# szcompressor/sz

Hardware: AMD Instinct MI355X
Metric: compression GB/s (input), 512^3 float32 ABS 1e-4 (higher is better)
Workload: dtype f32

## Files before the change

### sz_amd/csrc/szh_segenc.h

```cpp
#pragma once

namespace szh_se {
constexpr int NR = 4;
constexpr int INNER = 7;
constexpr int PF = 8;

struct col_t { int b0, b1, s0, s1, o0, o1, rows; };
struct seg_t {
    int bkbeg, bkend, kbeg, kend;
    int nE, E, L;
    int ka, nvec, pitch, kshift;
    int nblk, nruns;
    int lg_nvec;
};
SZH_HD int seg_pitch(int width) { int p = (width + 1) & ~1; if (((p >> 1) & 1) == 0) p += 2; return p; }
SZH_HD col_t make_col(const szh_geom3 &G, int col)
{
    col_t c;
    c.b0 = col / G.g1.num; c.b1 = col - c.b0 * G.g1.num;
    c.s0 = szh_blk_size(G.g0, c.b0); c.s1 = szh_blk_size(G.g1, c.b1); c.o0 = szh_blk_start(G.g0, c.b0); c.o1 = szh_blk_start(G.g1, c.b1);
    c.rows = c.s0 * c.s1;
    return c;
}
SZH_HD seg_t make_seg(const szh_geom3 &G, int rows, int segi, int segb, int VW)
{
    seg_t s;
    s.bkbeg = segi * segb; s.bkend = s.bkbeg + segb < G.g2.num ? s.bkbeg + segb : G.g2.num;
    s.kbeg = szh_blk_start(G.g2, s.bkbeg); s.kend = s.bkend < G.g2.num ? szh_blk_start(G.g2, s.bkend) : G.g2.count;
    s.E = G.g2.early; s.L = G.g2.late;
    int nE = G.g2.split - s.bkbeg; if (nE < 0) nE = 0; if (nE > s.bkend - s.bkbeg) nE = s.bkend - s.bkbeg;
    s.nE = nE;
    s.ka = s.kbeg / VW * VW;
    const int kb = (s.kend + VW - 1) / VW * VW;
    s.nvec = (kb - s.ka) / VW;
    s.pitch = seg_pitch(kb - s.ka); s.kshift = s.kbeg - s.ka;
    s.nblk = s.bkend - s.bkbeg; s.nruns = s.nblk * rows;
    s.lg_nvec = 0; while ((1 << s.lg_nvec) < s.nvec) ++s.lg_nvec;
    return s;
}
inline size_t seg_tile_bytes(const szh_geom3 &G, int segb, int VW)
{
    const size_t rows = (size_t)G.g0.early * G.g1.early;
    const int width = segb * G.g2.early + 2 * VW;
    return (rows * (size_t)seg_pitch(width) * 2 + 15) & ~(size_t)15;
}
inline size_t seg_pieces_per_thread(const szh_geom3 &G, int segb, int VW)
{
    const size_t rows = (size_t)G.g0.early * G.g1.early;
    const size_t nvec = ((size_t)segb * G.g2.early + 2 * VW) / VW + 1;
    size_t p2 = 1; while (p2 < nvec) p2 <<= 1;
    return (rows * p2 + 255) / 256;
}
inline size_t seg_window_words(const szh_geom3 &G, unsigned maxlen, int nrmax = NR) { return (size_t)256 * nrmax * (size_t)G.g2.early * maxlen / 32 + 8; }
}

#ifdef SZH_HIPSIM
static inline bool any_lane(bool p) { return __ballot(p ? 1 : 0) != 0ull; }
#else
__device__ __forceinline__ bool any_lane(bool p) { return __builtin_amdgcn_ballot_w64(p) != 0ull; }
#endif
__device__ __forceinline__ unsigned magic_of(unsigned d) { return d > 1u ? 0xffffffffu / d + 1u : 0u; }
__device__ __forceinline__ unsigned div_by(unsigned x, unsigned d, unsigned m) { return d > 1u ? (unsigned)(((u64)x * m) >> 32) : x; }

#define SZH_COL_HBINS 256
__global__ __launch_bounds__(256) void k_col_hist(szh_geom3 G, const uint16_t *__restrict__ codes, unsigned nbins, int rshift, int vw, unsigned *__restrict__ col_hist)
{
    SZH_DYN_SMEM(smem);
    unsigned *sh = reinterpret_cast<unsigned *>(smem);
    const unsigned R = 1u << rshift;
    for (unsigned i = threadIdx.x; i < (nbins << rshift); i += 256) sh[i] = 0;
    __syncthreads();
    const szh_se::col_t c = szh_se::make_col(G, (int)blockIdx.x);
    const int nvec = G.g2.count / vw;
    const int lane = (int)threadIdx.x & 63, wid = (int)threadIdx.x >> 6;
    const unsigned rep = threadIdx.x & (R - 1);
    const unsigned m_s1 = magic_of((unsigned)c.s1);
    for (int x = lane; x < nvec; x += 64) {
        for (int r0 = wid; r0 < c.rows; r0 += 16) {
            uint4 w[4];
#pragma unroll
            for (int q = 0; q < 4; ++q) {
                const int r = r0 + 4 * q;
                w[q] = uint4{0u, 0u, 0u, 0u};
                if (r < c.rows) {
                    const int i = (int)div_by((unsigned)r, (unsigned)c.s1, m_s1), j = r - i * c.s1;
                    const uint16_t *src = codes + (int64_t)(c.o0 + i) * G.d0 + (int64_t)(c.o1 + j) * G.d1 + x * vw;
                    if (vw == 8) w[q] = *reinterpret_cast<const uint4 *>(src);
                    else if (vw == 4) { const uint2 t = *reinterpret_cast<const uint2 *>(src); w[q].x = t.x; w[q].y = t.y; }
                    else w[q].x = src[0];
                }
            }
#pragma unroll
            for (int q = 0; q < 4; ++q) {
                if (r0 + 4 * q < c.rows) {
                    const unsigned wv[4] = {w[q].x, w[q].y, w[q].z, w[q].w};
#pragma unroll
                    for (int e = 0; e < 8; ++e) if (e < vw) { const unsigned cd = (e & 1) ? wv[e >> 1] >> 16 : wv[e >> 1] & 0xffffu; atomicAdd(&sh[(cd << rshift) + rep], 1u); }
                }
            }
        }
    }
    __syncthreads();
    for (unsigned b = threadIdx.x; b < nbins; b += 256) {
        unsigned t = 0;
        for (unsigned q = 0; q < R; ++q) t += sh[(b << rshift) + q];
        col_hist[(size_t)blockIdx.x * nbins + b] = t;
    }
}
__global__ __launch_bounds__(256) void k_hist_reduce(const unsigned *__restrict__ col_hist, unsigned nbins, int64_t ncols, unsigned *__restrict__ hist)
{
    __shared__ unsigned acc[SZH_COL_HBINS];
    for (unsigned b = threadIdx.x; b < nbins; b += 256) acc[b] = 0;
    __syncthreads();
    const unsigned tpb = 256u / nbins > 0u ? 256u / nbins : 1u;
    if (threadIdx.x < tpb * nbins) {
        const unsigned bin = threadIdx.x % nbins, lane_col = threadIdx.x / nbins;
        unsigned t = 0;
        for (int64_t col = (int64_t)blockIdx.x * tpb + lane_col; col < ncols; col += (int64_t)gridDim.x * tpb) t += col_hist[(size_t)col * nbins + bin];
        if (t) atomicAdd(&acc[bin], t);
    }
    __syncthreads();
    for (unsigned b = threadIdx.x; b < nbins; b += 256) if (acc[b]) atomicAdd(&hist[b], acc[b]);
}
__global__ __launch_bounds__(256) void k_col_bits_h(const unsigned *__restrict__ col_hist, const uint8_t *__restrict__ len, unsigned nbins, int64_t ncols, u64 *__restrict__ col_bits, u64 *__restrict__ col_zeros)
{
    __shared__ uint8_t llen[SZH_COL_HBINS];
    for (unsigned i = threadIdx.x; i < nbins; i += 256) llen[i] = len[i];
    __syncthreads();
    const int64_t e = (int64_t)blockIdx.x * 256 + threadIdx.x;
    if (e >= ncols) return;
    const unsigned *h = col_hist + (size_t)e * nbins;
    u64 bits = 0;
    for (unsigned b = 0; b < nbins; ++b) bits += (u64)h[b] * llen[b];
    col_bits[e] = bits; col_zeros[e] = h[0];
}

__global__ __launch_bounds__(256) void k_col_bits(szh_geom3 G, const uint16_t *__restrict__ codes, const uint8_t *__restrict__ len, unsigned nsym, int vw,
                                                  u64 *__restrict__ col_bits, u64 *__restrict__ col_zeros)
{
    SZH_DYN_SMEM(smem);
    __shared__ u64 red[8];
    uint8_t *llen = reinterpret_cast<uint8_t *>(smem);
    const bool tab_lds = nsym <= 16384;
    if (tab_lds) { for (unsigned i = threadIdx.x; i < nsym; i += 256) llen[i] = len[i]; __syncthreads(); }
    const szh_se::col_t c = szh_se::make_col(G, (int)blockIdx.x);
    const int nvec = G.g2.count / vw;
    const int lane = (int)threadIdx.x & 63, wid = (int)threadIdx.x >> 6;
    const unsigned m_s1 = magic_of((unsigned)c.s1);
    u64 bits = 0; unsigned zeros = 0;
    for (int x = lane; x < nvec; x += 64) {
        for (int r0 = wid; r0 < c.rows; r0 += 16) {
            uint4 w[4];
#pragma unroll
            for (int q = 0; q < 4; ++q) {
                const int r = r0 + 4 * q;
                w[q] = uint4{0u, 0u, 0u, 0u};
                if (r < c.rows) {
                    const int i = (int)div_by((unsigned)r, (unsigned)c.s1, m_s1), j = r - i * c.s1;
                    const uint16_t *src = codes + (int64_t)(c.o0 + i) * G.d0 + (int64_t)(c.o1 + j) * G.d1 + x * vw;
                    if (vw == 8) w[q] = *reinterpret_cast<const uint4 *>(src);
                    else if (vw == 4) { const uint2 t = *reinterpret_cast<const uint2 *>(src); w[q].x = t.x; w[q].y = t.y; }
                    else w[q].x = src[0];
                }
            }
#pragma unroll
            for (int q = 0; q < 4; ++q) {
                if (r0 + 4 * q < c.rows) {
                    const unsigned wv[4] = {w[q].x, w[q].y, w[q].z, w[q].w};
#pragma unroll
                    for (int e = 0; e < 8; ++e) if (e < vw) {
                        const unsigned cd = (e & 1) ? wv[e >> 1] >> 16 : wv[e >> 1] & 0xffffu;
                        bits += tab_lds ? llen[cd] : len[cd]; zeros += cd == 0u ? 1u : 0u;
                    }
                }
            }
        }
    }
    bits = wave_sum_u64(bits); const u64 z = wave_sum_u64((u64)zeros);
    if (lane == 0) { red[wid] = bits; red[4 + wid] = z; }
    __syncthreads();
    if (threadIdx.x == 0) { col_bits[blockIdx.x] = red[0] + red[1] + red[2] + red[3]; col_zeros[blockIdx.x] = red[4] + red[5] + red[6] + red[7]; }
}

__global__ __launch_bounds__(256) void k_col_bounds(const u64 *__restrict__ col_bitoff, int64_t nent, const u64 *__restrict__ total_bits, u64 bit0, unsigned *out32)
{
    const int64_t e = (int64_t)blockIdx.x * 256 + threadIdx.x;
    if (e > nent) return;
    const u64 at = bit0 + (e < nent ? col_bitoff[e] : *total_bits);
    out32[at >> 5] = 0u;
    if (e == nent) out32[(at >> 5) + 1] = 0u;
}
#define SZH_COL_SCAN_PER 8
__global__ __launch_bounds__(1024) void k_col_scan(const u64 *__restrict__ col_bits, const u64 *__restrict__ col_zeros, int nent, u64 *__restrict__ col_bitoff, u64 *__restrict__ col_zoff,
                                                   u64 *total_bits, u64 *total_zeros, u64 bit0, unsigned *out32, const u64 *__restrict__ plan = nullptr)
{
    __shared__ u64 shb[16], shz[16];
    if (plan) { if (plan[SZH_PLAN_STATUS] != 0) return; bit0 = plan[SZH_PLAN_BIT0]; }
    const int tid = (int)threadIdx.x, lane = tid & 63, wid = tid >> 6;
    const int lo = tid * SZH_COL_SCAN_PER;
    u64 vb[SZH_COL_SCAN_PER], vz[SZH_COL_SCAN_PER];
#pragma unroll
    for (int q = 0; q < SZH_COL_SCAN_PER; ++q) { const bool in = lo + q < nent; vb[q] = in ? col_bits[lo + q] : 0ull; vz[q] = in ? col_zeros[lo + q] : 0ull; }
    u64 b = 0, z = 0;
#pragma unroll
    for (int q = 0; q < SZH_COL_SCAN_PER; ++q) { b += vb[q]; z += vz[q]; }
    u64 ib = b, iz = z;
    for (int o = 1; o < 64; o <<= 1) { const u64 tb = __shfl_up(ib, o, 64), tz = __shfl_up(iz, o, 64); if (lane >= o) { ib += tb; iz += tz; } }
    if (lane == 63) { shb[wid] = ib; shz[wid] = iz; }
    __syncthreads();
    u64 baseb = 0, basez = 0, totb = 0, totz = 0;
    for (int w = 0; w < 16; ++w) { if (w < wid) { baseb += shb[w]; basez += shz[w]; } totb += shb[w]; totz += shz[w]; }
    u64 rb = baseb + ib - b, rz = basez + iz - z;
#pragma unroll
    for (int q = 0; q < SZH_COL_SCAN_PER; ++q) {
        if (lo + q < nent) { col_bitoff[lo + q] = rb; col_zoff[lo + q] = rz; out32[(bit0 + rb) >> 5] = 0u; }
        rb += vb[q]; rz += vz[q];
    }
    if (tid == 0) { *total_bits = totb; *total_zeros = totz; out32[(bit0 + totb) >> 5] = 0u; out32[((bit0 + totb) >> 5) + 1] = 0u; }
}

__global__ __launch_bounds__(1024) void k_col_zscan(const unsigned *__restrict__ col_zeros, int nent, u64 *__restrict__ col_zoff, u64 *total_zeros)
{
    __shared__ u64 shz[16];
    const int tid = (int)threadIdx.x, lane = tid & 63, wid = tid >> 6;
    const int lo = tid * SZH_COL_SCAN_PER;
    u64 vz[SZH_COL_SCAN_PER], z = 0;
#pragma unroll
    for (int q = 0; q < SZH_COL_SCAN_PER; ++q) { vz[q] = lo + q < nent ? (u64)col_zeros[lo + q] : 0ull; z += vz[q]; }
    u64 iz = z;
    for (int o = 1; o < 64; o <<= 1) { const u64 tz = __shfl_up(iz, o, 64); if (lane >= o) iz += tz; }
    if (lane == 63) shz[wid] = iz;
    __syncthreads();
    u64 basez = 0, totz = 0;
    for (int w = 0; w < 16; ++w) { if (w < wid) basez += shz[w]; totz += shz[w]; }
    u64 rz = basez + iz - z;
#pragma unroll
    for (int q = 0; q < SZH_COL_SCAN_PER; ++q) { if (lo + q < nent) col_zoff[lo + q] = rz; rz += vz[q]; }
    if (tid == 0) *total_zeros = totz;
}

template <class T, bool WIDE>
__global__ __launch_bounds__(256) void k_col_encode(szh_geom3 G, const uint16_t *__restrict__ codes, const u64 *__restrict__ table, unsigned nsym, const szh_se::seg_t *__restrict__ segs, int nseg, int vw, int nrmax,
                                                    size_t tile_bytes, unsigned win_words, const u64 *__restrict__ col_bitoff, const u64 *__restrict__ col_zoff, u64 bit0,
                                                    unsigned *out32, const T *__restrict__ data, T *__restrict__ unpred, const u64 *__restrict__ plan = nullptr)
{
    using namespace szh_se;
    if (plan) { if (plan[SZH_PLAN_STATUS] != 0) return; bit0 = plan[SZH_PLAN_BIT0]; }
    SZH_DYN_SMEM(smem);
    __shared__ u64 sh[2][4];
    __shared__ unsigned rowbase[128];
    u64 *ltab = reinterpret_cast<u64 *>(smem);
    uint16_t *tile = reinterpret_cast<uint16_t *>(smem + ((size_t)nsym + 1) * 8);
    uint16_t *nullrun = reinterpret_cast<uint16_t *>(smem + ((size_t)nsym + 1) * 8 + tile_bytes);
    unsigned *win = reinterpret_cast<unsigned *>(smem + ((size_t)nsym + 1) * 8 + tile_bytes + 16);
    const int tid = (int)threadIdx.x, lane = tid & 63, wid = tid >> 6;
    const col_t c = make_col(G, (int)blockIdx.x);
    for (unsigned i = tid; i < nsym; i += 256) ltab[i] = table[i];
    if (tid == 0) ltab[nsym] = 0;
    if (tid < 8) nullrun[tid] = (uint16_t)nsym;
    for (unsigned w = tid; w < win_words; w += 256) win[w] = 0u;
    const unsigned m_rows = magic_of((unsigned)c.rows);
    if (tid < c.rows) { const int i = tid / c.s1, j = tid - i * c.s1; rowbase[tid] = (unsigned)((int64_t)(c.o0 + i) * G.d0 + (int64_t)(c.o1 + j) * G.d1); }
    __syncthreads();
    uint4 pf[PF];
    auto fetch = [&](const seg_t &s) {
        const int lg = s.lg_nvec, mask = (1 << lg) - 1;
#pragma unroll
        for (int p = 0; p < PF; ++p) {
            const int x = p * 256 + tid, r = x >> lg, cv = x & mask;
            pf[p] = uint4{0u, 0u, 0u, 0u};
            if (r < c.rows && cv < s.nvec) {
                const uint16_t *src = codes + (size_t)rowbase[r] + (unsigned)(s.ka + cv * vw);
                if (vw == 8) pf[p] = *reinterpret_cast<const uint4 *>(src);
                else if (vw == 4) { const uint2 t = *reinterpret_cast<const uint2 *>(src); pf[p].x = t.x; pf[p].y = t.y; }
                else pf[p].x = src[0];
// ... 279 lines not shown
```

### sz_amd/csrc/szhip.hip

```cpp
#include <hip/hip_runtime.h>
#include <algorithm>
#include <array>
#include <cmath>
#include <cstdio>
#include <cstdlib>
#include <cstring>
#include <atomic>
#include <chrono>
#include <ctime>
#include <condition_variable>
#include <deque>
#include <functional>
#include <memory>
#include <mutex>
#include <thread>
#include <vector>
#include "../../include/szhip.h"
#include "szhost.h"
#include "szhip_kernels.h"
#include "szh_quality.h"
#include "szh_rangebatch.h"

namespace {

struct DevBuf { void *p = nullptr; size_t cap = 0; };

double now_ms()
{
    timespec ts; clock_gettime(CLOCK_MONOTONIC, &ts);
    return ts.tv_sec * 1e3 + ts.tv_nsec * 1e-6;
}

}

static std::atomic<int> g_compress_calls{0};
static std::atomic<int> g_fed_active{0};
static std::atomic<long long> g_last_meeting_us{-(1ll << 60)};
static long long mono_us() { timespec ts; clock_gettime(CLOCK_MONOTONIC, &ts); return (long long)ts.tv_sec * 1000000ll + ts.tv_nsec / 1000; }
struct compress_call_guard {
    compress_call_guard()
    {
        if (g_compress_calls.fetch_add(1) > 0) g_last_meeting_us.store(mono_us());
        const long long t0 = mono_us();
        while (g_fed_active.load() != 0 && mono_us() - t0 < 200000) std::this_thread::yield();
    }
    ~compress_call_guard() { g_compress_calls.fetch_sub(1); }
};
struct fed_call_guard {
    bool on = false;
    bool try_raise()
    {
        if (mono_us() - g_last_meeting_us.load() < 100000) return false;
        int expected = 0;
        if (!g_fed_active.compare_exchange_strong(expected, 1)) return false;
        if (g_compress_calls.load() > 1) { g_fed_active.store(0); return false; }
        on = true;
        return true;
    }
    ~fed_call_guard() { if (on) g_fed_active.store(0); }
};
struct szhip_chain_pool {
    std::thread th[4];
    std::mutex m; std::condition_variable cv;
    std::atomic<int> phase{0};
    std::atomic<uint64_t> seq{0};
    std::atomic<int> stage1{0}, stage2{0};
    int n = 0;
    std::function<void(int)> chain, section;
    static void pause() {
#if defined(__x86_64__)
        __builtin_ia32_pause();
#endif
    }
    void run(int e)
    {
        uint64_t seen = 0;
        for (;;) {
            { std::unique_lock<std::mutex> lk(m); cv.wait(lk, [&] { return phase.load() != 0; }); }
            if (phase.load() == 2) return;
            while (phase.load(std::memory_order_acquire) == 1 && seq.load(std::memory_order_acquire) == seen) pause();
            const uint64_t s = seq.load(std::memory_order_acquire);
            if (s != seen) {
                seen = s;
                if (e < n) { chain(e); stage1.fetch_add(1, std::memory_order_release); section(e); }
                stage2.fetch_add(1, std::memory_order_release);
            }
        }
    }
    void start() { for (int e = 0; e < 4; ++e) th[e] = std::thread([this, e] { run(e); }); }
    void arm() { { std::lock_guard<std::mutex> lk(m); if (phase.load() == 0) phase.store(1); } cv.notify_all(); }
    void disarm() { std::lock_guard<std::mutex> lk(m); if (phase.load() == 1) phase.store(0); }
    void submit(int ncoef, std::function<void(int)> c, std::function<void(int)> sec)
    {
        n = ncoef; chain = std::move(c); section = std::move(sec);
        stage1.store(0); stage2.store(0);
        arm();
        seq.fetch_add(1, std::memory_order_release);
    }
    void wait_chains() { while (stage1.load(std::memory_order_acquire) < n) pause(); }
    void wait_all() { while (stage2.load(std::memory_order_acquire) < 4) std::this_thread::yield(); }
    ~szhip_chain_pool()
    {
        { std::lock_guard<std::mutex> lk(m); phase.store(2); }
        cv.notify_all();
        for (auto &t : th) if (t.joinable()) t.join();
    }
};

constexpr int SZH_STAGE_T = 4;
struct szhip_ctx {
    int device = 0;
    int cus = 256;
    hipStream_t stream = nullptr;
    hipStream_t stream2 = nullptr;
    hipEvent_t ev_in = nullptr, ev_fit = nullptr, ev_feed = nullptr, ev_sec = nullptr;
    int settle_probes = 0, settle_rejected = 0;
    hipStream_t stream3 = nullptr;
    hipEvent_t ev_perm = nullptr;
    hipEvent_t ev[6] = {nullptr, nullptr, nullptr, nullptr, nullptr, nullptr};
    char err[512] = {0};
    unsigned epoch = 0;
    bool hdec_sync_rounds = false, hdec_unconverged = false;
    bool gate = false;
    unsigned long long *hdec_res = nullptr;
    DevBuf lor_bits, reg_flags, reg_rank, coef_compact, in, out, codes_nat, codes_blk, coef, blk_lor, faceI, faceJ, rb_down, rb_right, rb_vals, pt_flags, feed_word, progress, order, small, hist, col_zeros, col_zeros64,
        seg_bits, seg_zeros, seg_bitoff, seg_zoff, seg_hist, seg_tab, col_off, partial, samples, unpred, stream_buf, chunk_bits, chunk_off, code_tab, len_tab, dec_tab,
        starts, ends, counts, offs, dirty, zcnt, zpos, pwr_log, pwr_signs, pwr_small, coef_dec, msst_ptab, msst_cells, msst_rec, msst_pe, book_tree, book_rec, book_stage,
        batch_rec, batch_blob,
        in2, quality;
    void *pinned = nullptr; size_t pinned_cap = 0;
    void *pinned2 = nullptr; size_t pinned2_cap = 0;
    void *stage_buf[SZH_STAGE_T][2] = {};
    hipEvent_t stage_ev[SZH_STAGE_T][2] = {};
    void *pinned3 = nullptr; size_t pinned3_cap = 0;
    int streams_independent = -1;
    void *coh = nullptr; size_t coh_cap = 0;
    int order_nI = -1, order_nJ = -1;
    bool wave_timeout = false, ticket_atomic = false;
    bool coef_late = false, no_chain_overlap = false;
    bool book_declined = false, no_dev_book = false;
    unsigned long long *book_pin = nullptr;
    std::vector<int> chain_codes; std::vector<unsigned char> chain_unpred;
    unsigned char *sec_pin[4] = {nullptr, nullptr, nullptr, nullptr}; size_t sec_pin_cap[4] = {0, 0, 0, 0};
    szhip_chain_pool *chain_pool = nullptr;
};

namespace {

#include "szhip_rt.inc"
#include "szhip_steps.inc"
#include "szhip_sz21.inc"
#include "szhip_sz14.inc"
#include "szhip_pwr.inc"
#include "szhip_omp.inc"
#include "szhip_ompbatch.inc"
#include "szhip_rangebatch.inc"
#include "szhip_quality.inc"

}

static void drain(szhip_ctx *ctx)
{
    if (ctx->stream3) hipStreamSynchronize(ctx->stream3);
    hipStreamSynchronize(ctx->stream2);
    hipStreamSynchronize(ctx->stream);
}
static int drained_on_failure(szhip_ctx *ctx, int rc) { if (rc != SZHIP_OK) drain(ctx); return rc; }
static int synced_on_failure(szhip_ctx *ctx, int rc) { if (rc != SZHIP_OK) hipStreamSynchronize(ctx->stream); return rc; }

template <class F>
static int with_ticket_fallback(szhip_ctx *ctx, F &&run)
{
    ctx->wave_timeout = false; ctx->hdec_unconverged = false; ctx->coef_late = false; ctx->book_declined = false;
    auto again = [&]() { drain(ctx); return run(); };
    int rc = run();
    if (rc == SZHIP_ERR_INTERNAL && ctx->book_declined && !ctx->no_dev_book) {
        ctx->no_dev_book = true; ctx->wave_timeout = false; rc = again(); ctx->no_dev_book = false;
    }
    if (rc == SZHIP_OK && !ctx->no_chain_overlap && tune_int("SZ_HIP_TEST_CHAIN_FALLBACK", 0)) { ctx->coef_late = true; rc = SZHIP_ERR_INTERNAL; }
    if (rc == SZHIP_ERR_INTERNAL && ctx->coef_late && !ctx->no_chain_overlap) {
        ctx->no_chain_overlap = true; ctx->wave_timeout = false; rc = again();
    }
    if (rc == SZHIP_ERR_INTERNAL && ctx->hdec_unconverged && !ctx->hdec_sync_rounds) {
        ctx->hdec_sync_rounds = true; ctx->wave_timeout = false; rc = again(); ctx->hdec_sync_rounds = false;
    }
    if (rc == SZHIP_OK && !ctx->ticket_atomic && tune_int("SZ_HIP_TEST_TICKET_FALLBACK", 0)) { ctx->wave_timeout = true; rc = SZHIP_ERR_INTERNAL; }
    if (rc == SZHIP_ERR_INTERNAL && ctx->wave_timeout && !ctx->ticket_atomic) {
        ctx->ticket_atomic = true; rc = again();
    }
    return rc;
}

template <class F>
static int guarded_compress(szhip_ctx *ctx, unsigned char **out, size_t *out_size, F &&run)
{
    const compress_call_guard in_flight;
    unsigned char *const out0 = *out; const size_t cap0 = *out_size;
    return drained_on_failure(ctx, with_ticket_fallback(ctx, [&]() { *out = out0; *out_size = cap0; return run(); }));
}

static bool dims_3d_2d(size_t r0, size_t r1, size_t r2)
{
    return !((r0 != 0 && r0 < 2) || r1 < 2 || r2 < 2 || r0 > 0x7fffffff || r1 > 0x7fffffff || r2 > 0x7fffffff);
}
static bool dims_3d_2d_1d(size_t r0, size_t r1, size_t r2)
{
    return !((r0 != 0 && r0 < 2) || (r1 < 2 && !(r0 == 0 && r1 == 0)) || r2 < 2 || r0 > 0x7fffffff || r1 > 0x7fffffff || r2 > 0x7fffffff);
}

extern "C" {


static int create_ctx(szhip_ctx **out, int device)
{
    if (!out) return SZHIP_ERR_ARG;
    int count = 0;
    hipError_t e = hipGetDeviceCount(&count);
    if (e != hipSuccess || count <= 0) {
        fprintf(stderr, "szhip: no HIP device available (%s); this library has no CPU fallback\n", hipGetErrorString(e));
        return SZHIP_ERR_NODEVICE;
    }
    if (device < 0 || device >= count) return SZHIP_ERR_ARG;
    szhip_ctx *ctx = new szhip_ctx();
    ctx->device = device;
    { int c = 0; if (hipDeviceGetAttribute(&c, hipDeviceAttributeMultiprocessorCount, device) == hipSuccess && c > 0) ctx->cus = c; }
    if (hipSetDevice(device) != hipSuccess || hipStreamCreateWithFlags(&ctx->stream, hipStreamNonBlocking) != hipSuccess) {
        delete ctx; return SZHIP_ERR_NODEVICE;
    }
    for (int i = 0; i < 6; ++i) if (hipEventCreate(&ctx->ev[i]) != hipSuccess) { delete ctx; return SZHIP_ERR_NODEVICE; }
    if (hipStreamCreateWithFlags(&ctx->stream2, hipStreamNonBlocking) != hipSuccess || hipEventCreateWithFlags(&ctx->ev_in, hipEventDisableTiming) != hipSuccess ||
        hipEventCreateWithFlags(&ctx->ev_fit, hipEventDisableTiming) != hipSuccess ||
        hipEventCreateWithFlags(&ctx->ev_feed, hipEventDisableTiming) != hipSuccess ||
        hipEventCreateWithFlags(&ctx->ev_sec, hipEventDisableTiming) != hipSuccess) { delete ctx; return SZHIP_ERR_NODEVICE; }
    *out = ctx;
    return SZHIP_OK;
}

int szhip_create(szhip_ctx **out, int device)
{
    const int rc = create_ctx(out, device);
    if (rc == SZHIP_OK) settle_streams(*out, nullptr, 0);
    return rc;
}

void szhip_destroy(szhip_ctx *ctx)
{
    if (!ctx) return;
    hipSetDevice(ctx->device);
    hipStreamSynchronize(ctx->stream);
    delete ctx->chain_pool; ctx->chain_pool = nullptr;
    DevBuf *bufs[] = {&ctx->lor_bits, &ctx->reg_flags, &ctx->reg_rank, &ctx->coef_compact, &ctx->in, &ctx->out, &ctx->codes_nat, &ctx->codes_blk, &ctx->coef, &ctx->blk_lor, &ctx->faceI, &ctx->faceJ, &ctx->rb_down, &ctx->rb_right, &ctx->rb_vals, &ctx->pt_flags, &ctx->feed_word, &ctx->progress,
                      &ctx->order, &ctx->small, &ctx->hist, &ctx->col_zeros, &ctx->col_zeros64, &ctx->seg_bits, &ctx->seg_zeros, &ctx->seg_bitoff, &ctx->seg_zoff, &ctx->seg_hist, &ctx->seg_tab, &ctx->col_off, &ctx->partial,
                      &ctx->samples, &ctx->unpred, &ctx->stream_buf, &ctx->chunk_bits, &ctx->chunk_off, &ctx->code_tab,
                      &ctx->len_tab, &ctx->dec_tab, &ctx->starts, &ctx->ends, &ctx->counts, &ctx->offs, &ctx->dirty, &ctx->zcnt, &ctx->zpos,
                      &ctx->pwr_log, &ctx->pwr_signs, &ctx->pwr_small, &ctx->coef_dec, &ctx->msst_ptab, &ctx->msst_cells, &ctx->msst_rec, &ctx->msst_pe, &ctx->book_tree, &ctx->book_rec, &ctx->book_stage, &ctx->batch_rec, &ctx->batch_blob, &ctx->in2, &ctx->quality};
    for (DevBuf *b : bufs) if (b->p) hipFree(b->p);
    if (ctx->pinned) hipHostFree(ctx->pinned);
    if (ctx->pinned2) hipHostFree(ctx->pinned2);
    if (ctx->pinned3) hipHostFree(ctx->pinned3);
    if (ctx->coh) hipHostFree(ctx->coh);
    if (ctx->hdec_res) hipHostFree(ctx->hdec_res);
    if (ctx->book_pin) hipHostFree(ctx->book_pin);
    for (int w = 0; w < SZH_STAGE_T; ++w) for (int k = 0; k < 2; ++k) { if (ctx->stage_buf[w][k]) hipHostFree(ctx->stage_buf[w][k]); if (ctx->stage_ev[w][k]) hipEventDestroy(ctx->stage_ev[w][k]); }
    for (int i = 0; i < 6; ++i) if (ctx->ev[i]) hipEventDestroy(ctx->ev[i]);
    if (ctx->ev_in) hipEventDestroy(ctx->ev_in);
    if (ctx->ev_fit) hipEventDestroy(ctx->ev_fit);
    if (ctx->ev_feed) hipEventDestroy(ctx->ev_feed);
    if (ctx->ev_sec) hipEventDestroy(ctx->ev_sec);
    for (int e = 0; e < 4; ++e) if (ctx->sec_pin[e]) hipHostFree(ctx->sec_pin[e]);
    if (ctx->stream2) hipStreamDestroy(ctx->stream2);
    if (ctx->stream3) hipStreamDestroy(ctx->stream3);
    if (ctx->ev_perm) hipEventDestroy(ctx->ev_perm);
    if (ctx->stream) hipStreamDestroy(ctx->stream);
    delete ctx;
}

const char *szhip_last_error(szhip_ctx *ctx) { return ctx ? ctx->err : "no context"; }

struct szhip_pool_job {
    int dtype; const void *data; int on_dev; size_t r0, r1, r2; double eb; szhip_params prm; const unsigned char *meta; size_t meta_len;
    int out_on_device; unsigned char *out; size_t out_size; szhip_stats stats; int rc; bool done;
};
struct szhip_pool {
    std::vector<szhip_ctx *> ctx;
    std::vector<std::thread> workers;
    std::mutex mu;
    std::condition_variable cv_work, cv_done;
    std::deque<int> queue;
    std::vector<szhip_pool_job> jobs;
    std::vector<bool> used;
    bool stop = false;
};
static void szhip_pool_worker(szhip_pool *p, int lane)
{
    for (;;) {
        int t;
        {
            std::unique_lock<std::mutex> lk(p->mu);
            p->cv_work.wait(lk, [&] { return p->stop || !p->queue.empty(); });
            if (p->queue.empty()) return;
            t = p->queue.front(); p->queue.pop_front();
        }
        szhip_pool_job &j = p->jobs[t];
        j.rc = szhip_compress(p->ctx[lane], j.dtype, j.data, j.on_dev, j.r0, j.r1, j.r2, j.eb, &j.prm, j.meta, j.meta_len, j.out_on_device,
                              &j.out, &j.out_size, &j.stats);
        { std::lock_guard<std::mutex> lk(p->mu); j.done = true; }
        p->cv_done.notify_all();
    }
}
int szhip_pool_create(szhip_pool **out, int device, int lanes)
{
    if (!out || lanes < 1 || lanes > 16) return SZHIP_ERR_ARG;
    szhip_pool *p = new szhip_pool();
    for (int i = 0; i < lanes; ++i) {
        szhip_ctx *c = nullptr;
        const int rc = create_ctx(&c, device);
        if (rc != SZHIP_OK) { for (szhip_ctx *x : p->ctx) szhip_destroy(x); delete p; return rc; }
        c->gate = lanes > 1;
        { std::vector<hipStream_t> mains; for (szhip_ctx *x : p->ctx) { mains.push_back(x->stream); mains.push_back(x->stream2); } settle_streams(c, mains.data(), (int)mains.size(), lanes == 1); }
        p->ctx.push_back(c);
    }
    p->jobs.resize(64); p->used.assign(64, false);
    for (int i = 0; i < lanes; ++i) p->workers.emplace_back(szhip_pool_worker, p, i);
    *out = p;
    return SZHIP_OK;
}
void szhip_pool_destroy(szhip_pool *p)
{
    if (!p) return;
    { std::lock_guard<std::mutex> lk(p->mu); p->stop = true; }
    p->cv_work.notify_all();
    for (auto &w : p->workers) if (w.joinable()) w.join();
    for (szhip_ctx *c : p->ctx) szhip_destroy(c);
    delete p;
}
int szhip_pool_submit(szhip_pool *p, int dtype, const void *data, int data_on_device, size_t r0, size_t r1, size_t r2, double eb,
                      const szhip_params *params, const unsigned char *meta, size_t meta_len, int out_on_device,
                      unsigned char *out_buf, size_t out_cap, int *ticket)
{
    if (!p || !data || !params || !meta || !ticket) return SZHIP_ERR_ARG;
    std::lock_guard<std::mutex> lk(p->mu);
    int t = -1;
    for (size_t i = 0; i < p->used.size(); ++i) if (!p->used[i]) { t = (int)i; break; }
    if (t < 0) return SZHIP_ERR_ARG;
    szhip_pool_job &j = p->jobs[t];
    j = szhip_pool_job();
    j.dtype = dtype; j.data = data; j.on_dev = data_on_device; j.r0 = r0; j.r1 = r1; j.r2 = r2; j.eb = eb; j.prm = *params;
    j.meta = meta; j.meta_len = meta_len; j.out_on_device = out_on_device; j.out = out_on_device == 2 ? out_buf : nullptr;
    j.out_size = out_on_device == 2 ? out_cap : 0; j.rc = SZHIP_ERR_INTERNAL; j.done = false;
    p->used[t] = true;
    p->queue.push_back(t);
    *ticket = t;
    p->cv_work.notify_one();
    return SZHIP_OK;
}
int szhip_pool_wait(szhip_pool *p, int ticket, unsigned char **out, size_t *out_size, szhip_stats *stats)
{
    if (!p || ticket < 0 || ticket >= (int)p->jobs.size()) return SZHIP_ERR_ARG;
    std::unique_lock<std::mutex> lk(p->mu);
    if (!p->used[ticket]) return SZHIP_ERR_ARG;
    p->cv_done.wait(lk, [&] { return p->jobs[ticket].done; });
    szhip_pool_job &j = p->jobs[ticket];
    if (out) *out = j.out;
    if (out_size) *out_size = j.out_size;
    if (stats) *stats = j.stats;
    p->used[ticket] = false;
    return j.rc;
}


int szhip_stage_input(szhip_ctx *ctx, const void *host_data, size_t bytes, void **device_ptr)
{
    if (!ctx || !host_data || !device_ptr) return SZHIP_ERR_ARG;
    if (hipSetDevice(ctx->device) != hipSuccess) return SZHIP_ERR_NODEVICE;
    TRY(ensure(ctx, ctx->in, bytes));
    TRY(staged_copy(ctx, ctx->in.p, host_data, bytes, true));
    *device_ptr = ctx->in.p;
    return SZHIP_OK;
}

int szhip_stage_input_batch(szhip_ctx *ctx, const void *const *host_data, int count, size_t bytes, const void **device_ptrs)
{
    if (!ctx || !host_data || !device_ptrs || count < 1 || bytes == 0) return SZHIP_ERR_ARG;
    for (int i = 0; i < count; ++i) if (!host_data[i]) return SZHIP_ERR_ARG;
    if (hipSetDevice(ctx->device) != hipSuccess) return SZHIP_ERR_NODEVICE;
    std::vector<const void *> d;
    TRY(synced_on_failure(ctx, batch_stage(ctx, ctx->in, count, bytes, ctx->stream, [&](int i) { return host_data[i]; }, d)));
    if (hipStreamSynchronize(ctx->stream) != hipSuccess) return SZHIP_ERR_NODEVICE;
    for (int i = 0; i < count; ++i) device_ptrs[i] = d[i];
    return SZHIP_OK;
}
int szhip_stage_input_batch_lens(szhip_ctx *ctx, const void *const *host_data, int count, const size_t *bytes, const void **device_ptrs)
{
    if (!ctx || !host_data || !device_ptrs || !bytes || count < 1) return SZHIP_ERR_ARG;
    for (int i = 0; i < count; ++i) if (!host_data[i] || bytes[i] == 0) return SZHIP_ERR_ARG;
    if (hipSetDevice(ctx->device) != hipSuccess) return SZHIP_ERR_NODEVICE;
    std::vector<const void *> d;
    TRY(synced_on_failure(ctx, batch_stage(ctx, ctx->in, count, 0, ctx->stream, [&](int i) { return host_data[i]; }, d, nullptr, bytes)));
    if (hipStreamSynchronize(ctx->stream) != hipSuccess) return SZHIP_ERR_NODEVICE;
    for (int i = 0; i < count; ++i) device_ptrs[i] = d[i];
    return SZHIP_OK;
}

static int check_alignment_set_device(szhip_ctx *ctx, int dtype, const void *p)
{
    if (((uintptr_t)p & (dtype == SZHIP_F32 ? 3u : 7u)) != 0) {
        snprintf(ctx->err, sizeof(ctx->err), "pointer %p is not aligned to its %d-byte elements", p, dtype == SZHIP_F32 ? 4 : 8);
        return SZHIP_ERR_ARG;
    }
    return hipSetDevice(ctx->device) != hipSuccess ? SZHIP_ERR_NODEVICE : SZHIP_OK;
}
#define BY_DTYPE(dtype, fn, ...) ((dtype) == SZHIP_F32 ? fn<float>(__VA_ARGS__) : fn<double>(__VA_ARGS__))

int szhip_minmax(szhip_ctx *ctx, int dtype, const void *data, int on_dev, size_t n, double *vmin, double *vmax)
{
    if (!ctx || !data || !n || !vmin || !vmax) return SZHIP_ERR_ARG;
    TRY(check_alignment_set_device(ctx, dtype, data));
    return BY_DTYPE(dtype, minmax_impl, ctx, data, on_dev, n, vmin, vmax);
}

static int batch_pointers(szhip_ctx *ctx, int dtype, const void *const *p, int count, size_t n)
{
    if (!ctx || !p || count < 1 || n == 0 || (dtype != SZHIP_F32 && dtype != SZHIP_F64)) return SZHIP_ERR_ARG;
    for (int i = 0; i < count; ++i) {
        if (!p[i]) { snprintf(ctx->err, sizeof(ctx->err), "array %d of the batch: a null pointer", i); return SZHIP_ERR_ARG; }
        if (((uintptr_t)p[i] & (dtype == SZHIP_F32 ? 3u : 7u)) != 0) {
            snprintf(ctx->err, sizeof(ctx->err), "array %d of the batch: pointer %p is not aligned to its %d-byte elements", i, p[i], dtype == SZHIP_F32 ? 4 : 8);
            return SZHIP_ERR_ARG;
        }
    }
    return SZHIP_OK;
}

int szhip_minmax_batch(szhip_ctx *ctx, int dtype, const void *const *data, int count, int data_on_device, size_t n, double *vmin, double *vmax, szhip_stats *stats)
{
    if (!vmin || !vmax) return SZHIP_ERR_ARG;
    TRY(batch_pointers(ctx, dtype, data, count, n));
    if (hipSetDevice(ctx->device) != hipSuccess) return SZHIP_ERR_NODEVICE;
    return synced_on_failure(ctx, BY_DTYPE(dtype, minmax_batch_impl, ctx, data, count, data_on_device, 1, 1, n, n, n, nullptr, vmin, vmax, stats));
}
static int check_view(szhip_ctx *ctx, size_t r0, size_t r1, size_t r2, size_t pitch0, size_t pitch1);
int szhip_minmax_batch_view(szhip_ctx *ctx, int dtype, const void *const *data, int count, int data_on_device, size_t r0, size_t r1, size_t r2, size_t pitch0, size_t pitch1,
                            double *vmin, double *vmax, szhip_stats *stats)
{
    if (!vmin || !vmax) return SZHIP_ERR_ARG;
    if (r0 < 1 || r1 < 1 || r2 < 1 || r0 > 0x7fffffff || r1 > 0x7fffffff || r2 > 0x7fffffff) return SZHIP_ERR_ARG;
    TRY(batch_pointers(ctx, dtype, data, count, 1));
    TRY(check_view(ctx, r0, r1, r2, pitch0, pitch1));
    if ((double)r0 * (double)r1 * (double)r2 >= 4294967296.0) { snprintf(ctx->err, sizeof(ctx->err), "szhip_minmax_batch_view: sub-boxes of 2^32 values or more"); return SZHIP_ERR_UNSUP; }
    if (hipSetDevice(ctx->device) != hipSuccess) return SZHIP_ERR_NODEVICE;
    if (pitch1 == r2 && pitch0 == r1 * r2) { const size_t n = r0 * r1 * r2; r0 = r1 = 1; r2 = pitch0 = pitch1 = n; }
    return synced_on_failure(ctx, BY_DTYPE(dtype, minmax_batch_impl, ctx, data, count, data_on_device, r0, r1, r2, pitch0, pitch1, nullptr, vmin, vmax, stats));
}

int szhip_compress(szhip_ctx *ctx, int dtype, const void *data, int data_on_device, size_t r0, size_t r1, size_t r2, double eb,
                   const szhip_params *params, const unsigned char *meta, size_t meta_len, int out_on_device,
                   unsigned char **out, size_t *out_size, szhip_stats *stats)
{
    if (!ctx || !data || !params || !meta || !out || !out_size) return SZHIP_ERR_ARG;
    if (!dims_3d_2d(r0, r1, r2)) return SZHIP_ERR_ARG;
    if (!(eb > 0)) return SZHIP_ERR_ARG;
    TRY(check_alignment_set_device(ctx, dtype, data));
    return guarded_compress(ctx, out, out_size, [&]() {
               return BY_DTYPE(dtype, compress_impl, ctx, data, data_on_device, r0, r1, r2, eb, params, meta, meta_len, out_on_device, out, out_size, stats); });
}

int szhip_compress_sz14(szhip_ctx *ctx, int dtype, const void *data, int data_on_device, size_t r0, size_t r1, size_t r2, double eb,
                        double value_range, double median, const szhip_params *params, const unsigned char *meta, size_t meta_len,
                        int out_on_device, unsigned char **out, size_t *out_size, szhip_stats *stats)
{
    if (!ctx || !data || !params || !meta || !out || !out_size) return SZHIP_ERR_ARG;
    if (!dims_3d_2d_1d(r0, r1, r2)) return SZHIP_ERR_ARG;
    if (!(eb > 0)) return SZHIP_ERR_ARG;
    TRY(check_alignment_set_device(ctx, dtype, data));
    return guarded_compress(ctx, out, out_size, [&]() {
               return BY_DTYPE(dtype, compress14_impl, ctx, data, data_on_device, r0, r1, r2, eb, value_range, median, params, meta, meta_len, nullptr, out_on_device, out, out_size, stats); });
}

int szhip_decompress_sz14(szhip_ctx *ctx, int dtype, const unsigned char *stream, int stream_on_device, size_t stream_len, size_t body_off,
                          size_t r0, size_t r1, size_t r2, void *out, int out_on_device, szhip_stats *stats)
{
    if (!ctx || !stream || !out || body_off >= stream_len) return SZHIP_ERR_ARG;
    if (!dims_3d_2d_1d(r0, r1, r2)) return SZHIP_ERR_ARG;
    TRY(check_alignment_set_device(ctx, dtype, out));
    return drained_on_failure(ctx, with_ticket_fallback(ctx, [&]() {
               return BY_DTYPE(dtype, decompress14_impl, ctx, stream, stream_on_device, stream_len, body_off, 0, r0, r1, r2, out, out_on_device, stats); }));
}

int szhip_compress_omp(szhip_ctx *ctx, int dtype, const void *data, int data_on_device, size_t r0, size_t r1, size_t r2, double eb, int thread_num,
                       const szhip_params *params, const unsigned char *meta, size_t meta_len, int out_on_device, unsigned char **out, size_t *out_size,
                       szhip_stats *stats)
{
    if (!ctx || !data || !params || !meta || !out || !out_size) return SZHIP_ERR_ARG;
    if (r0 < 1 || r1 < 1 || r2 < 1 || r0 > 0x7fffffff || r1 > 0x7fffffff || r2 > 0x7fffffff || thread_num < 1) return SZHIP_ERR_ARG;
    if (!(eb > 0)) return SZHIP_ERR_ARG;
    TRY(check_alignment_set_device(ctx, dtype, data));
    return synced_on_failure(ctx,
               BY_DTYPE(dtype, compress_omp_impl, ctx, data, data_on_device, r0, r1, r2, r1 * r2, r2, eb, thread_num, params, meta, meta_len, out_on_device, out, out_size, stats));
}

int szhip_decompress_omp(szhip_ctx *ctx, int dtype, const unsigned char *stream, int stream_on_device, size_t stream_len, size_t body_off,
                         size_t r0, size_t r1, size_t r2, void *out, int out_on_device, szhip_stats *stats)
{
    if (!ctx || !stream || !out || body_off >= stream_len) return SZHIP_ERR_ARG;
    if (r0 < 1 || r1 < 1 || r2 < 1 || r0 > 0x7fffffff || r1 > 0x7fffffff || r2 > 0x7fffffff) return SZHIP_ERR_ARG;
    TRY(check_alignment_set_device(ctx, dtype, out));
    return synced_on_failure(ctx,
               BY_DTYPE(dtype, decompress_omp_impl, ctx, stream, stream_on_device, stream_len, body_off, r0, r1, r2, out, out_on_device, 0, 0, stats));
}

static int batch_args(szhip_ctx *ctx, int dtype, const szhip_batch_item *items, int count, size_t r0, size_t r1, size_t r2, bool compress)
// ... 462 lines not shown
```

### sz_amd/csrc/szhip_kernels.h

```cpp
#pragma once
#include <hip/hip_runtime.h>
#include "szh_core.h"
#include "szh_pencil.h"
#include "szh_bufio.h"

typedef unsigned long long u64;

#ifdef SZH_HIPSIM
#define SZH_DYN_SMEM(name) char *name = hipsim_dyn_smem()
#else
#define SZH_DYN_SMEM(name) extern __shared__ __attribute__((aligned(16))) char name[]
#endif

__device__ __forceinline__ u64 ord_enc(float v)
{
    unsigned u = __float_as_uint(v);
    u = (u & 0x80000000u) ? ~u : (u | 0x80000000u);
    return (u64)u;
}
__device__ __forceinline__ u64 ord_enc(double v)
{
    u64 u = (u64)__double_as_longlong(v);
    u = (u & 0x8000000000000000ull) ? ~u : (u | 0x8000000000000000ull);
    return u;
// ... 129 lines not shown
    __device__ static szh_u64 ld_sys_u64(const szh_u64 *p) { return __hip_atomic_load(const_cast<szh_u64 *>(p), __ATOMIC_RELAXED, __HIP_MEMORY_SCOPE_SYSTEM); }
    __device__ static float ld_coef(const float *p) { return __uint_as_float(__hip_atomic_load(reinterpret_cast<unsigned *>(const_cast<float *>(p)), __ATOMIC_RELAXED, __HIP_MEMORY_SCOPE_SYSTEM)); }
    __device__ static double ld_coef(const double *p) { return __longlong_as_double((long long)__hip_atomic_load(reinterpret_cast<szh_u64 *>(const_cast<double *>(p)), __ATOMIC_RELAXED, __HIP_MEMORY_SCOPE_SYSTEM)); }
    __device__ static void backoff(int n) { for (int i = 0; i < n; ++i) __builtin_amdgcn_s_sleep(2); }
    template <class E, int N> __device__ static void ld16(const E *p, E (&v)[N])
    {
        static_assert(sizeof(E) * N == 16, "16-byte vector");
        const uint4 w = *reinterpret_cast<const uint4 *>(p);
        __builtin_memcpy(v, &w, 16);
    }
    template <class E, int N> __device__ static void st16(E *p, const E (&v)[N])
    {
        static_assert(sizeof(E) * N == 16, "16-byte vector");
        uint4 w; __builtin_memcpy(&w, v, 16);
        *reinterpret_cast<uint4 *>(p) = w;
    }
    __device__ static void nap() { __builtin_amdgcn_s_sleep(40); }
};

template <class T> struct szh_tile_shape;
#ifndef SZH_TPI_F32
#define SZH_TPI_F32 2
#define SZH_TPJ_F32 2
#endif
template <> struct szh_tile_shape<float> { static constexpr int TPI = SZH_TPI_F32, TPJ = SZH_TPJ_F32, RL = 64; };
#ifndef SZH_TPI_F64
#define SZH_TPI_F64 3
#define SZH_TPJ_F64 3
#define SZH_RL_F64 32
#endif
template <> struct szh_tile_shape<double> { static constexpr int TPI = SZH_TPI_F64, TPJ = SZH_TPJ_F64, RL = SZH_RL_F64; };

template <class T, bool DEC, bool MS = false>
__global__ __launch_bounds__((szh_tile_shape<T>::TPI * szh_tile_shape<T>::TPJ + 2) * 64) void k_pencil(szh_qargs<T> a)
{
    using S = szh_tile_shape<T>;
    using B = GpuBackend<S::TPI, S::TPJ, S::RL>;
    constexpr int NP = S::TPI * S::TPJ, NV = S::TPI + S::TPJ, NT = (NP + 2) * 64;
    __shared__ uint16_t cring[NP * (SZH_XC + 1) * 64];
    __shared__ T faces[(NP + NV) * (S::RL + 2) * SZH_FROWS + SZH_FTRASH];
    __shared__ unsigned cstep[NP + NV];
    __shared__ unsigned spubJ[NP], spubI[NP];
    __shared__ int scratch[128];
#ifdef SZH_LDS_PAD
    __shared__ int lds_pad[SZH_LDS_PAD / 4];
    if (a.backoff == -12345) lds_pad[threadIdx.x] = 1;
#endif
    __shared__ unsigned tk_s;
    (void)NT;
#ifdef SZH_HIPSIM
    const int w = (int)(threadIdx.x >> 6);
#else
    const int w = __builtin_amdgcn_readfirstlane((int)(threadIdx.x >> 6));
    {
        const int d = w < NP ? (w / S::TPJ + w % S::TPJ) : -1;
        if (d < 0) __builtin_amdgcn_s_setprio(3);
        else if (d == 0) __builtin_amdgcn_s_setprio(3); else if (d == 1) __builtin_amdgcn_s_setprio(2);
        else if (d <= 3) __builtin_amdgcn_s_setprio(1); else __builtin_amdgcn_s_setprio(0);
    }
#endif
    const szh_tile_lds<T> L{cring, faces, (NP + NV) * (S::RL + 2) * SZH_FROWS, cstep, spubJ, spubI, scratch};
    const unsigned ntiles = (unsigned)(((a.nI + S::TPI - 1) / S::TPI) * ((a.nJ + S::TPJ - 1) / S::TPJ));
    for (unsigned it = 0;; ++it) {
        if (it) __syncthreads();
        if (threadIdx.x < NP + NV) cstep[threadIdx.x] = 0;
        if (threadIdx.x < NP) { spubJ[threadIdx.x] = 0; spubI[threadIdx.x] = 0; }
        if (threadIdx.x == 0) {
            const unsigned t = (a.ticket_mode && !a.persist) ? blockIdx.x : atomicAdd(a.ticket, 1u);
            tk_s = t >= ntiles ? 0xffffffffu
                 : (a.ticket_mode == 2 || a.persist) ? szh_pencil_order_at((a.nI + S::TPI - 1) / S::TPI, (a.nJ + S::TPJ - 1) / S::TPJ, t) : a.order[t];
        }
        __syncthreads();
#ifdef SZH_HIPSIM
        const unsigned ij = tk_s;
#else
        const unsigned ij = (unsigned)__builtin_amdgcn_readfirstlane((int)tk_s);
#endif
        if (ij == 0xffffffffu) break;
        const int TI = (int)(ij >> 16), TJ = (int)(ij & 0xffffu);
        if (w < NP) {
            const int I = TI * S::TPI + w / S::TPJ, J = TJ * S::TPJ + w % S::TPJ;
            if (I < a.nI && J < a.nJ) szh_pencil_run<T, DEC, B, MS>(a, I, J, L);
        } else if (w == NP) szh_tile_store<T, B>(a, TI, TJ, L);
        else szh_tile_fill<T, B>(a, TI, TJ, L);
        if (!a.persist) break;
    }
}

template <class T> struct GlobAcc {
    const T *p; int64_t d0, d1;
    __device__ T operator()(int i, int j, int k) const { return p[i * d0 + j * d1 + k]; }
    __device__ T operator()(int j, int k) const { return p[j * d1 + k]; }
};

template <class T>
__global__ __launch_bounds__(256) void k_fit_select(szh_geom3 G, const T *__restrict__ data, T *coef, uint8_t *blk_lor,
                                                    T noise, int use_mean, T mean, u64 *minmax)
{
    __shared__ u64 red[8];
    const int lane = threadIdx.x & 63, wid = threadIdx.x >> 6;
    const int64_t b = (int64_t)blockIdx.x * 256 + threadIdx.x;
    u64 lmin = ~0ull, lmax = 0ull;
    if (b < G.nblocks) {
        const int nb2 = G.g2.num, nb1 = G.g1.num;
        const int b2 = (int)(b % nb2);
        const int64_t c = b / nb2;
        const int b1 = (int)(c % nb1), b0 = (int)(c / nb1);
        const int s0 = szh_blk_size(G.g0, b0), s1 = szh_blk_size(G.g1, b1), s2 = szh_blk_size(G.g2, b2);
        const GlobAcc<T> A{data + (int64_t)szh_blk_start(G.g0, b0) * G.d0 + (int64_t)szh_blk_start(G.g1, b1) * G.d1 + szh_blk_start(G.g2, b2),
                           G.d0, G.d1};
        T c4[4];
        auto range = [&](T v) { const u64 oe = ord_enc(v); const bool num = v == v; lmin = num && oe < lmin ? oe : lmin; lmax = num && oe > lmax ? oe : lmax; };
        int reg;
        if (G.ndim == 2) {
            c4[0] = 0;
            szh_fit_block_2d<T>(A, s1, s2, c4 + 1, range);
            reg = szh_select_block_2d<T>(A, s1, s2, c4 + 1, noise);
        } else {
            szh_fit_block<T>(A, s0, s1, s2, c4, range);
            reg = szh_select_block<T>(A, s0, s1, s2, c4, noise, use_mean, mean);
        }
        for (int e = 0; e < 4; ++e) coef[(int64_t)e * G.nblocks + b] = c4[e];
        blk_lor[b] = reg ? 0 : 1;
    }
    lmin = wave_min_u64(lmin); lmax = wave_max_u64(lmax);
    if (lane == 0) { red[wid] = lmin; red[4 + wid] = lmax; }
    __syncthreads();
    if (threadIdx.x == 0) {
        u64 mn = red[0], mx = red[4];
        for (int w = 1; w < 4; ++w) { mn = red[w] < mn ? red[w] : mn; mx = red[4 + w] > mx ? red[4 + w] : mx; }
        atomicMin(&minmax[0], mn); atomicMax(&minmax[1], mx);
    }
}

template <class T>
__global__ __launch_bounds__(256) void k_minmax(const T *__restrict__ data, int64_t n, u64 *minmax)
{
    __shared__ u64 red[8];
    u64 lmin = ~0ull, lmax = 0ull;
    for (int64_t i = (int64_t)blockIdx.x * 256 + threadIdx.x; i < n; i += (int64_t)gridDim.x * 256) {
        const T v = data[i]; const u64 e = ord_enc(v); const bool num = v == v;
        lmin = num && e < lmin ? e : lmin; lmax = num && e > lmax ? e : lmax;
    }
    lmin = wave_min_u64(lmin); lmax = wave_max_u64(lmax);
    if ((threadIdx.x & 63) == 0) { red[threadIdx.x >> 6] = lmin; red[4 + (threadIdx.x >> 6)] = lmax; }
    __syncthreads();
    if (threadIdx.x == 0) {
        u64 mn = red[0], mx = red[4];
        for (int w = 1; w < 4; ++w) { mn = red[w] < mn ? red[w] : mn; mx = red[4 + w] > mx ? red[4 + w] : mx; }
        atomicMin(&minmax[0], mn); atomicMax(&minmax[1], mx);
    }
}

template <class T>
__global__ __launch_bounds__(256) void k_gather_mean(const T *__restrict__ data, szh_meanwalk w, int64_t count, T *out)
{
    const int64_t m = (int64_t)blockIdx.x * 256 + threadIdx.x;
    if (m < count) out[m] = data[szh_meanwalk_pos(w, m)];
}

#define SZH_LDS_RADIUS_BINS 4096
template <class T, bool FREQ>
__device__ __forceinline__ void sample_body(szh_geom3 G, const T *__restrict__ data, int64_t nrows, int sd, double ebD, T mean,
                                            unsigned max_radius, unsigned *radius_hist, unsigned *freq_hist, u64 *within)
{
    __shared__ unsigned sh_r[SZH_LDS_RADIUS_BINS];
    __shared__ unsigned sh_f[FREQ ? 8192 : 1];
    for (int i = threadIdx.x; i < SZH_LDS_RADIUS_BINS; i += 256) sh_r[i] = 0;
    if (FREQ) for (int i = threadIdx.x; i < 8192; i += 256) sh_f[i] = 0;
    __syncthreads();
    const int64_t rpp = G.g1.count - 1, r2 = G.g2.count;
    const bool two_d = G.ndim == 2;
    unsigned w = 0;
    for (int64_t ridx = (int64_t)blockIdx.x * 256 + threadIdx.x; ridx < nrows; ridx += (int64_t)gridDim.x * 256) {
        const int64_t n1 = two_d ? 0 : ridx / rpp + 1, n2 = two_d ? ridx + 1 : ridx - (n1 - 1) * rpp + 1;
        const int64_t c0 = two_d ? szh_sample_col0_2d(n2, sd) : sd - ((n1 + n2) % sd);
        const int64_t origin = n1 * G.d0 + n2 * r2;
        for (int64_t m = 0;; ++m) {
            const int64_t col = c0 + m * sd;
            if (m > 0 && col >= r2) break;
            const int64_t pos = origin + col;
            if (pos >= G.n) break;
            unsigned ri; int fi, we;
            szh_sample_point<T>(data, pos, r2, two_d ? 0 : G.d0, ebD, mean, max_radius, &ri, &fi, &we);
            if (ri < SZH_LDS_RADIUS_BINS) atomicAdd(&sh_r[ri], 1u); else atomicAdd(&radius_hist[ri], 1u);
            if (FREQ) atomicAdd(&sh_f[fi], 1u);
            w += (unsigned)we;
        }
    }
    w = wave_sum_u32(w);
    if ((threadIdx.x & 63) == 0 && w) atomicAdd(within, (u64)w);
    __syncthreads();
    for (int i = threadIdx.x; i < SZH_LDS_RADIUS_BINS; i += 256) if (sh_r[i]) atomicAdd(&radius_hist[i], sh_r[i]);
    if (FREQ) for (int i = threadIdx.x; i < 8192; i += 256) if (sh_f[i]) atomicAdd(&freq_hist[i], sh_f[i]);
}
template <class T, bool FREQ>
__global__ __launch_bounds__(256) void k_sample(szh_geom3 G, const T *__restrict__ data, int64_t nrows, int sd, double ebD, T mean,
                                                unsigned max_radius, unsigned *radius_hist, unsigned *freq_hist, u64 *within)
{
    sample_body<T, FREQ>(G, data, nrows, sd, ebD, mean, max_radius, radius_hist, freq_hist, within);
}
template <class T, bool FREQ>
__global__ void k_sample_walk(szh_geom3 G, const T *__restrict__ data, int sd, double ebD, T mean, unsigned max_radius, unsigned *radius_hist,
                              unsigned *freq_hist, u64 *within)
{
    if (threadIdx.x != 0 || blockIdx.x != 0) return;
    const int64_t r3 = G.g2.count, r2 = G.g1.count, r23 = r2 * r3, len = G.n;
    int64_t oc = sd - 2, n1 = 1, n2 = 1, pos = r23 + r3 + oc;
    u64 w = 0;
    while (pos < len) {
        unsigned ri; int fi, we;
        szh_sample_point<T>(data, pos, r3, r23, ebD, mean, max_radius, &ri, &fi, &we);
        atomicAdd(&radius_hist[ri], 1u);
        if (FREQ) atomicAdd(&freq_hist[fi], 1u);
        w += (unsigned)we;
        oc += sd;
        if (oc >= r3) {
            n2++;
            if (n2 == r2) { n1++; n2 = 1; pos += r3; }
            const int64_t oc2 = (n1 + n2) % sd;
            pos += (r3 + sd - oc) + (sd - oc2);
            oc = sd - oc2;
            if (oc == 0) oc++;
        } else pos += sd;
    }
    if (w) atomicAdd(within, w);
}

template <class T>
__device__ __forceinline__ void sample_view_body(const unsigned tid, szh_geom3 G, const T *data, int64_t p0, int64_t p1, int64_t nrows, int sd, double ebD,
                                                 unsigned max_radius, unsigned *radius_hist, u64 *within)
{
    __shared__ unsigned sh_r[SZH_LDS_RADIUS_BINS];
    for (int i = tid; i < SZH_LDS_RADIUS_BINS; i += 256) sh_r[i] = 0;
    __syncthreads();
    const int64_t rpp = G.g1.count - 1, r2 = G.g2.count;
    unsigned w = 0;
    for (int64_t ridx = (int64_t)blockIdx.x * 256 + tid; ridx < nrows; ridx += (int64_t)gridDim.x * 256) {
        const int64_t n1 = ridx / rpp + 1, n2 = ridx - (n1 - 1) * rpp + 1;
        const int64_t c0 = sd - ((n1 + n2) % sd);
        const int64_t origin = n1 * G.d0 + n2 * r2;
        for (int64_t m = 0;; ++m) {
            const int64_t col = c0 + m * sd;
            if (m > 0 && col >= r2) break;
            const int64_t pos = origin + col;
            if (pos >= G.n) break;
            unsigned ri; int fi, we;
            if (col < r2) szh_sample_point<T>(data, n1 * p0 + n2 * p1 + col, p1, p0, ebD, (T)0, max_radius, &ri, &fi, &we);
            else szh_sample_point_view<T>(data, pos, r2, G.d0, p0, p1, ebD, max_radius, &ri, &we);
            if (ri < SZH_LDS_RADIUS_BINS) atomicAdd(&sh_r[ri], 1u); else atomicAdd(&radius_hist[ri], 1u);
            w += (unsigned)we;
        }
    }
    w = wave_sum_u32(w);
    if ((tid & 63) == 0 && w) atomicAdd(within, (u64)w);
    __syncthreads();
    for (int i = tid; i < SZH_LDS_RADIUS_BINS; i += 256) if (sh_r[i]) atomicAdd(&radius_hist[i], sh_r[i]);
}
template <class T>
__global__ __launch_bounds__(256) void k_sample_view(szh_geom3 G, const T *__restrict__ data, int64_t p0, int64_t p1, int64_t nrows, int sd, double ebD,
                                                     unsigned max_radius, unsigned *radius_hist, u64 *within)
{
    __shared__ unsigned sh_r[SZH_LDS_RADIUS_BINS];
    for (int i = threadIdx.x; i < SZH_LDS_RADIUS_BINS; i += 256) sh_r[i] = 0;
    __syncthreads();
    const int64_t rpp = G.g1.count - 1, r2 = G.g2.count;
    unsigned w = 0;
    for (int64_t ridx = (int64_t)blockIdx.x * 256 + threadIdx.x; ridx < nrows; ridx += (int64_t)gridDim.x * 256) {
        const int64_t n1 = ridx / rpp + 1, n2 = ridx - (n1 - 1) * rpp + 1;
        const int64_t c0 = sd - ((n1 + n2) % sd);
        const int64_t origin = n1 * G.d0 + n2 * r2;
        for (int64_t m = 0;; ++m) {
            const int64_t col = c0 + m * sd;
            if (m > 0 && col >= r2) break;
            const int64_t pos = origin + col;
            if (pos >= G.n) break;
            unsigned ri; int fi, we;
            if (col < r2) szh_sample_point<T>(data, n1 * p0 + n2 * p1 + col, p1, p0, ebD, (T)0, max_radius, &ri, &fi, &we);
            else szh_sample_point_view<T>(data, pos, r2, G.d0, p0, p1, ebD, max_radius, &ri, &we);
            if (ri < SZH_LDS_RADIUS_BINS) atomicAdd(&sh_r[ri], 1u); else atomicAdd(&radius_hist[ri], 1u);
            w += (unsigned)we;
        }
    }
    w = wave_sum_u32(w);
    if ((threadIdx.x & 63) == 0 && w) atomicAdd(within, (u64)w);
    __syncthreads();
    for (int i = threadIdx.x; i < SZH_LDS_RADIUS_BINS; i += 256) if (sh_r[i]) atomicAdd(&radius_hist[i], sh_r[i]);
}
template <class T>
__global__ void k_sample_walk_view(szh_geom3 G, const T *__restrict__ data, int64_t p0, int64_t p1, int sd, double ebD, unsigned max_radius,
                                   unsigned *radius_hist, u64 *within)
{
    if (threadIdx.x != 0 || blockIdx.x != 0) return;
    const int64_t r3 = G.g2.count, r2 = G.g1.count, r23 = r2 * r3, len = G.n;
    int64_t oc = sd - 2, n1 = 1, n2 = 1, pos = r23 + r3 + oc;
    u64 w = 0;
    while (pos < len) {
        unsigned ri; int we;
        szh_sample_point_view<T>(data, pos, r3, r23, p0, p1, ebD, max_radius, &ri, &we);
        atomicAdd(&radius_hist[ri], 1u);
        w += (unsigned)we;
        oc += sd;
        if (oc >= r3) {
            n2++;
            if (n2 == r2) { n1++; n2 = 1; pos += r3; }
            const int64_t oc2 = (n1 + n2) % sd;
            pos += (r3 + sd - oc) + (sd - oc2);
            oc = sd - oc2;
            if (oc == 0) oc++;
        } else pos += sd;
    }
// ... 1123 lines not shown
```

### sz_amd/csrc/szhip_rt.inc

```

#define HIPCHK(call)                                                                                   \
    do {                                                                                               \
        hipError_t e_ = (call);                                                                        \
        if (e_ != hipSuccess) {                                                                        \
            snprintf(ctx->err, sizeof(ctx->err), "%s failed: %s (%s:%d)", #call, hipGetErrorString(e_), __FILE__, __LINE__); \
            fprintf(stderr, "szhip: %s\n", ctx->err);                                                  \
            return SZHIP_ERR_NODEVICE;                                                                 \
        }                                                                                              \
    } while (0)

#define FAIL(code, ...)                                                                                \
    do {                                                                                               \
        snprintf(ctx->err, sizeof(ctx->err), __VA_ARGS__);                                             \
        fprintf(stderr, "szhip: %s\n", ctx->err);                                                      \
        return (code);                                                                                 \
    } while (0)
#define FAIL_PUBLISHED(code, ...)                                                                      \
    do {                                                                                               \
        if (!out_on_device && out && *out) { free(*out); *out = nullptr; }                              \
        if (out_size) *out_size = 0;                                                                   \
        FAIL(code, __VA_ARGS__);                                                                       \
    } while (0)

int ensure(szhip_ctx *ctx, DevBuf &b, size_t bytes, bool zero_new = false)
{
    if (bytes == 0) bytes = 16;
    if (b.cap >= bytes) return SZHIP_OK;
    if (b.p) { HIPCHK(hipStreamSynchronize(ctx->stream)); HIPCHK(hipFree(b.p)); b.p = nullptr; b.cap = 0; }
    size_t cap = bytes + bytes / 8 + 256;
    HIPCHK(hipMalloc(&b.p, cap));
    b.cap = cap;
    if (zero_new) HIPCHK(hipMemsetAsync(b.p, 0, cap, ctx->stream));
    return SZHIP_OK;
}

#define TRY(x) do { int rc_ = (x); if (rc_ != SZHIP_OK) return rc_; } while (0)

int ensure_host(szhip_ctx *ctx, void *&p, size_t &have, size_t bytes, hipStream_t user, unsigned flags = hipHostMallocDefault)
{
    if (have >= bytes) return SZHIP_OK;
    if (p) { HIPCHK(hipStreamSynchronize(user)); HIPCHK(hipHostFree(p)); p = nullptr; have = 0; }
    size_t cap = bytes + bytes / 4 + 4096;
    HIPCHK(hipHostMalloc(&p, cap, flags));
    have = cap;
    return SZHIP_OK;
}
int ensure_pinned(szhip_ctx *ctx, size_t bytes) { return ensure_host(ctx, ctx->pinned, ctx->pinned_cap, bytes, ctx->stream); }
int ensure_pinned2(szhip_ctx *ctx, size_t bytes) { return ensure_host(ctx, ctx->pinned2, ctx->pinned2_cap, bytes, ctx->stream2); }
int ensure_pinned3(szhip_ctx *ctx, size_t bytes) { return ensure_host(ctx, ctx->pinned3, ctx->pinned3_cap, bytes, ctx->stream); }
int ensure_coherent(szhip_ctx *ctx, size_t bytes)
{
    const size_t had = ctx->coh_cap;
    TRY(ensure_host(ctx, ctx->coh, ctx->coh_cap, bytes, ctx->stream, hipHostMallocCoherent | hipHostMallocMapped));
    if (ctx->coh_cap != had) memset(ctx->coh, 0, ctx->coh_cap);
    return SZHIP_OK;
}

enum { SM_MINMAX = 0, SM_WITHIN = 2, SM_MEANCNT = 3, SM_TOTAL_UNPRED = 4, SM_TOTAL_BITS = 5, SM_TICKET = 6, SM_ERR = 7,
       SM_CHANGED = 8, SM_MEANSUM = 9, SM_TOTAL_SYM = 10, SM_NREG = 11, SM_SCRATCH = 12, SM_COUNT = 16 };

int probe_streams(szhip_ctx *ctx)
{
    if (ctx->streams_independent >= 0) return SZHIP_OK;
    TRY(ensure_coherent(ctx, 256));
    TRY(ensure(ctx, ctx->small, SM_COUNT * 8));
    volatile unsigned long long *flag = (volatile unsigned long long *)((char *)ctx->coh + 128);
    unsigned long long *src = (unsigned long long *)((char *)ctx->coh + 192);
    *flag = 0; *src = 1;
    HIPCHK(hipStreamSynchronize(ctx->stream)); HIPCHK(hipStreamSynchronize(ctx->stream2));
    u64 *sm = (u64 *)ctx->small.p;
    hipLaunchKernelGGL(k_probe_wait, dim3(1), dim3(1), 0, ctx->stream, (const unsigned long long *)flag, (unsigned long long *)(sm + SM_SCRATCH));
    HIPCHK(hipGetLastError());
    HIPCHK(hipMemcpyAsync(sm + SM_SCRATCH + 1, src, 8, hipMemcpyHostToDevice, ctx->stream2));
    const double t0 = now_ms();
    HIPCHK(hipStreamSynchronize(ctx->stream2));
    const double waited = now_ms() - t0;
    *flag = 1;
    HIPCHK(hipStreamSynchronize(ctx->stream));
    ctx->streams_independent = waited < 2.0 ? 1 : 0;
    return SZHIP_OK;
}

static int probe_pair(szhip_ctx *ctx, hipStream_t a, hipStream_t b, int *shared)
{
    TRY(ensure_coherent(ctx, 256));
    TRY(ensure(ctx, ctx->small, SM_COUNT * 8));
    volatile unsigned long long *flag = (volatile unsigned long long *)((char *)ctx->coh + 128);
    *flag = 0;
    HIPCHK(hipStreamSynchronize(a)); HIPCHK(hipStreamSynchronize(b));
    u64 *sm = (u64 *)ctx->small.p;
    hipLaunchKernelGGL(k_probe_wait, dim3(1), dim3(1), 0, a, (const unsigned long long *)flag, (unsigned long long *)(sm + SM_SCRATCH));
    HIPCHK(hipGetLastError());
    hipLaunchKernelGGL(k_probe_touch, dim3(1), dim3(1), 0, b, (unsigned long long *)(sm + SM_SCRATCH + 1));
    HIPCHK(hipGetLastError());
    const double t0 = now_ms();
    HIPCHK(hipStreamSynchronize(b));
    const double waited = now_ms() - t0;
    *flag = 1;
    HIPCHK(hipStreamSynchronize(a));
    *shared = waited < 2.0 ? 0 : 1;
    return SZHIP_OK;
}

static void settle_one(szhip_ctx *ctx, hipStream_t *victim, const std::vector<hipStream_t> &against, std::vector<hipStream_t> &rejected, int *probes)
{
    for (int attempt = 0; attempt < 6; ++attempt) {
        bool clash = false;
        for (hipStream_t a : against) {
            if (a == *victim) continue;
            int shared = 0;
            ++*probes;
            if (probe_pair(ctx, a, *victim, &shared) != SZHIP_OK) return;
            if (shared) { clash = true; break; }
        }
        if (!clash) return;
        hipStream_t fresh = nullptr;
        if (hipStreamCreateWithFlags(&fresh, hipStreamNonBlocking) != hipSuccess) return;
        rejected.push_back(*victim);
        *victim = fresh;
    }
}
static void settle_streams(szhip_ctx *ctx, const hipStream_t *mains, int n_mains, bool third = true)
{
#ifdef SZH_SYNC_LAUNCH
    (void)ctx; (void)mains; (void)n_mains; (void)third;
#else
    std::vector<hipStream_t> rejected, against(mains, mains + n_mains);
    int probes = 0;
    if (n_mains) settle_one(ctx, &ctx->stream, against, rejected, &probes);
    against.push_back(ctx->stream);
    settle_one(ctx, &ctx->stream2, against, rejected, &probes);
    if (third && !ctx->stream3 && hipStreamCreateWithFlags(&ctx->stream3, hipStreamNonBlocking) != hipSuccess) ctx->stream3 = nullptr;
    if (third && ctx->stream3) { against.push_back(ctx->stream2); settle_one(ctx, &ctx->stream3, against, rejected, &probes); }
    ctx->settle_probes = probes; ctx->settle_rejected = (int)rejected.size();
    for (hipStream_t r : rejected) hipStreamDestroy(r);
#endif
}

int tune_int(const char *name, int def);
constexpr size_t SZH_STAGE_CHUNK = 8u << 20;
struct host_view { size_t r1, row, pitch0, pitch1; };
static void host_view_move(const host_view &v, char *base, char *buf, size_t off, size_t len, bool gather)
{
    size_t rw = off / v.row, col = off - rw * v.row;
    while (len) {
        const size_t k = rw / v.r1, i = rw - k * v.r1, take = std::min(len, v.row - col);
        char *p = base + k * v.pitch0 + i * v.pitch1 + col;
        if (gather) memcpy(buf, p, take); else memcpy(p, buf, take);
        buf += take; len -= take; col = 0; ++rw;
    }
}
int staged_copy(szhip_ctx *ctx, void *dst, const void *src, size_t bytes, bool to_device, const host_view *hv = nullptr)
{
    hipStream_t st = ctx->stream;
    const size_t chunk = std::min(SZH_STAGE_CHUNK, (size_t)std::max(1, tune_int("SZ_HIP_STAGE_CHUNK_KB", (int)(SZH_STAGE_CHUNK >> 10))) << 10);
    if (bytes < 4 * chunk && hv) {
        TRY(ensure_pinned3(ctx, bytes));
        HIPCHK(hipStreamSynchronize(st));
        if (to_device) host_view_move(*hv, (char *)const_cast<void *>(src), (char *)ctx->pinned3, 0, bytes, true);
        HIPCHK(hipMemcpyAsync(to_device ? dst : ctx->pinned3, to_device ? ctx->pinned3 : src, bytes, to_device ? hipMemcpyHostToDevice : hipMemcpyDeviceToHost, st));
        HIPCHK(hipStreamSynchronize(st));
        if (!to_device) host_view_move(*hv, (char *)dst, (char *)ctx->pinned3, 0, bytes, false);
        return SZHIP_OK;
    }
    if (bytes < 4 * chunk) {
        HIPCHK(hipMemcpyAsync(dst, src, bytes, to_device ? hipMemcpyHostToDevice : hipMemcpyDeviceToHost, st));
        HIPCHK(hipStreamSynchronize(st));
        return SZHIP_OK;
    }
    constexpr int nthr = SZH_STAGE_T;
    for (int w = 0; w < nthr; ++w)
        for (int k = 0; k < 2; ++k)
            if (!ctx->stage_buf[w][k]) {
                HIPCHK(hipHostMalloc(&ctx->stage_buf[w][k], SZH_STAGE_CHUNK, hipHostMallocDefault));
                HIPCHK(hipEventCreateWithFlags(&ctx->stage_ev[w][k], hipEventDisableTiming));
            }
    HIPCHK(hipStreamSynchronize(st));
    const size_t nchunks = (bytes + chunk - 1) / chunk;
    std::atomic<int> failed(0);
    const int device = ctx->device;
    auto host_in = [&](void *buf, size_t off, size_t len) {
        if (hv) host_view_move(*hv, (char *)const_cast<void *>(src), (char *)buf, off, len, true); else memcpy(buf, (const char *)src + off, len);
    };
    auto host_out = [&](const void *buf, size_t off, size_t len) {
        if (hv) host_view_move(*hv, (char *)dst, (char *)const_cast<void *>(buf), off, len, false); else memcpy((char *)dst + off, buf, len);
    };
    auto worker = [&](int w) {
        if (hipSetDevice(device) != hipSuccess) { failed = 1; return; }
        size_t pend_off[2] = {0, 0}, pend_len[2] = {0, 0};
        bool pend[2] = {false, false};
        int k = 0;
        for (size_t c = (size_t)w; c < nchunks && !failed; c += (size_t)nthr, k ^= 1) {
            const size_t off = c * chunk, len = std::min(chunk, bytes - off);
            if (to_device) {
                if (pend[k] && hipEventSynchronize(ctx->stage_ev[w][k]) != hipSuccess) { failed = 1; return; }
                host_in(ctx->stage_buf[w][k], off, len);
                if (hipMemcpyAsync((char *)dst + off, ctx->stage_buf[w][k], len, hipMemcpyHostToDevice, st) != hipSuccess ||
                    hipEventRecord(ctx->stage_ev[w][k], st) != hipSuccess) { failed = 1; return; }
                pend[k] = true;
            } else {
                if (pend[k]) {
                    if (hipEventSynchronize(ctx->stage_ev[w][k]) != hipSuccess) { failed = 1; return; }
                    host_out(ctx->stage_buf[w][k], pend_off[k], pend_len[k]);
                }
                if (hipMemcpyAsync(ctx->stage_buf[w][k], (const char *)src + off, len, hipMemcpyDeviceToHost, st) != hipSuccess ||
                    hipEventRecord(ctx->stage_ev[w][k], st) != hipSuccess) { failed = 1; return; }
                pend[k] = true; pend_off[k] = off; pend_len[k] = len;
            }
        }
        for (int q = 0; q < 2; ++q, k ^= 1) {
            if (!pend[k]) continue;
            if (hipEventSynchronize(ctx->stage_ev[w][k]) != hipSuccess) { failed = 1; return; }
// ... 204 lines not shown
```

### sz_amd/csrc/szhip_sz21.inc

```
static bool book_declines(unsigned rec_status, unsigned long long plan_status, int test_switch) { return rec_status != 0 || plan_status != 0 || test_switch != 0; }

struct sz21_plan {
    bool use_beam = false;
    bool segenc = false;
    bool seghist = false;
    bool dev_book = false;
    bool sliced = false;
    int slices_req = 1;
    int se_vw = 1, se_segb = 0, se_nseg = 0, se_nrmax = szh_se::NR; size_t se_tile = 0;
    int sh_rshift = 0;
    bool revise(unsigned enc_maxlen) { if (!segenc || enc_maxlen <= 32) return false; segenc = false; seghist = false; return true; }
};
template <class T>
sz21_plan sz21_make_plan(const szhip_ctx *ctx, const szh_geom3 &G, unsigned intervals, size_t reg_count, bool beam_ok, bool overlap, bool feed, size_t meta_len)
{
    sz21_plan P;
    const int64_t n = G.n;
    P.use_beam = !overlap && beam_ok;
    const int segenc_sw = tune_int("SZ_HIP_SEGENC", 1);
    P.segenc = G.ndim == 3 && segenc_sw != 0 && (!feed || segenc_sw == 2);
    P.se_vw = (G.g2.count % 8) == 0 ? 8 : ((G.g2.count % 4) == 0 ? 4 : 1);
    if (P.segenc) {
        bool ok = intervals < 65536 && (double)n < 4.0e9;
        if ((int64_t)G.g0.late * G.g1.late * G.g2.late < 32) ok = false;
        const size_t fixed = ((size_t)intervals + 1) * 8 + 16 + szh_se::seg_window_words(G, 32) * 4 + 64;
        const size_t lds_cap = (size_t)63 * 1024, want = (size_t)std::max(4, tune_int("SZ_HIP_SEG_TILE_KB", 14)) * 1024;
        if (ok && fixed + szh_se::seg_tile_bytes(G, 1, P.se_vw) > lds_cap) ok = false;
        if (ok) {
            const size_t budget = std::min(lds_cap - fixed, std::max(want, szh_se::seg_tile_bytes(G, 1, P.se_vw)));
            int sb = 1;
            while (sb < G.g2.num && szh_se::seg_tile_bytes(G, sb + 1, P.se_vw) <= budget && szh_se::seg_pieces_per_thread(G, sb + 1, P.se_vw) <= (size_t)szh_se::PF) ++sb;
            sb = (G.g2.num + (G.g2.num + sb - 1) / sb - 1) / ((G.g2.num + sb - 1) / sb);
            if (const int f = tune_int("SZ_HIP_SEG_SEGB", 0)) sb = std::max(1, std::min(f, sb));
            P.se_segb = sb;
            P.se_nseg = (G.g2.num + sb - 1) / sb;
            P.se_tile = szh_se::seg_tile_bytes(G, sb, P.se_vw);
            const int rows_typ = (2 * G.g0.split > G.g0.num ? G.g0.early : G.g0.late) * (2 * G.g1.split > G.g1.num ? G.g1.early : G.g1.late);
            const int runs_typ = std::max(1, sb * rows_typ), rounds_typ = (runs_typ + 256 * szh_se::NR - 1) / (256 * szh_se::NR);
            P.se_nrmax = std::max(1, std::min(szh_se::NR, (runs_typ + 256 * rounds_typ - 1) / (256 * rounds_typ)));
            if ((double)G.g0.num * G.g1.num >= 2.0e9) ok = false;
        }
        P.segenc = ok;
    }
    P.seghist = P.segenc && intervals <= SZH_COL_HBINS && tune_int("SZ_HIP_SEGHIST", 1) != 0;
    if (P.seghist) P.sh_rshift = hist_rshift(intervals, 4096);
    P.dev_book = P.segenc && reg_count == 0 && !ctx->no_dev_book && tune_int("SZ_HIP_DEV_BOOK", 0) != 0 && G.g0.num * G.g1.num <= 1024 * SZH_COL_SCAN_PER &&
                 tune_int("SZ_HIP_SEG_SCAN1", 1) != 0 && meta_len + 8 + 4 + sizeof(T) + 1 + sizeof(T) <= 3072;
    P.slices_req = tune_int("SZ_HIP_SLICES", ctx->gate ? tune_int("SZ_HIP_SLICES_POOL", 2) : 4);
    P.sliced = P.use_beam && P.slices_req > 1 && !P.seghist;
    return P;
}

template <class T>
struct sz21_call : call_base {
    static constexpr int is_double = sizeof(T) == 8;
    static constexpr int64_t LINE = 128 / (int64_t)sizeof(T);
    const szhip_params *const prm; const unsigned char *meta; const size_t meta_len; const int out_on_device; unsigned char **const out; size_t *const out_size;
    const double eb_in; const T eb;
    const bool two_d;
    const szh_geom3 G; const int ncoef, ncols; const int64_t n, nb;
    const int tp_on = tune_int("SZ_HIP_TIMING", 0); double tp_t[32]; const char *tp_n[32]; int tp_k = 0;
    const T *d_in = nullptr; u64 *sm = nullptr; T *d_coef = nullptr; uint8_t *d_lor = nullptr; uint16_t *d_nat = nullptr, *d_blk = nullptr; unsigned *d_hist = nullptr, *h_hist = nullptr;
    T noise = 0; bool fit_tile = false; int ft_nseg = 0;
    size_t ind_bytes = 0; unsigned char *ind_bits = nullptr; u64 *nreg_h = nullptr, *minmax_h = nullptr;
    unsigned intervals = 0; int use_mean = 0; T mean = 0; size_t reg_count = 0;
    std::vector<unsigned char> meta_own;
    sz21_plan P;
    unsigned *tile_done = nullptr; size_t beam_words = 0;
    int perm_segb = 1, perm_nseg = 1; size_t perm_lds = 0;
    std::vector<szh_se::seg_t> se_segs; std::vector<u64> tab_code; std::vector<uint8_t> tab_len;
    unsigned enc_maxlen = 0; bool enc32 = false; size_t lds_e32 = 0;
    unsigned char *hdr = nullptr; size_t pre_len = 0, sections_total = 0, hdr_len = 0, unpred_bytes = 0, total_len = 0; u64 total_bits = 0, total_unpred = 0;
    u64 h_small[SM_COUNT];
    szhost_coeffs cf;
    size_t sec_len[4] = {0, 0, 0, 0};
    std::vector<std::thread> section_threads;
    std::atomic<int> section_failed{0};
    std::vector<unsigned char> all_reg_keep;
    std::vector<uint32_t> blk_of_rank;
    size_t chain_done[4] = {0, 0, 0, 0};
    size_t chain_avail = 0;
    double chain_t0[4] = {0, 0, 0, 0}, chain_t1[4] = {0, 0, 0, 0};
    bool overlap = false, feed = false, two_pieces = false;
    fed_call_guard fed_guard;
    T *hcoef = nullptr;
    bool pool_busy = false;
    bool cf_own = false;
    sz21_call(szhip_ctx *c, size_t r0, size_t r1, size_t r2, double eb_, const szhip_params *p, const unsigned char *m, size_t ml, int ood, unsigned char **o, size_t *os)
        : call_base(c), prm(p), meta(m), meta_len(ml), out_on_device(ood), out(o), out_size(os), eb_in(eb_), eb((T)eb_), two_d(r0 == 0),
          G(r0 == 0 ? szh_make_geom2((int)r1, (int)r2) : szh_make_geom3((int)r0, (int)r1, (int)r2)), ncoef(r0 == 0 ? 3 : 4), ncols(G.g0.num * G.g1.num), n(G.n), nb(G.nblocks)
    {
        memset(&cf, 0, sizeof(cf));
        S.n_elements = (uint64_t)n; S.n_blocks = (uint64_t)nb;
    }
    ~sz21_call() {
        join_sections();
        if (ctx->chain_pool) ctx->chain_pool->disarm();
        if (cf_own) for (int e = 0; e < 4; ++e) { cf.codes[e] = nullptr; cf.unpred[e] = nullptr; }
        szhost_coeffs_free(&cf);
    }
    void join_sections() {
        for (auto &x : section_threads) if (x.joinable()) x.join();
        if (pool_busy && ctx->chain_pool) { ctx->chain_pool->wait_all(); pool_busy = false; }
    }
    void TP(const char *nm) { if (tp_on && tp_k < 32) { tp_t[tp_k] = now_ms() - t_begin; tp_n[tp_k++] = nm; } }
    void print_trace() const { if (tp_on) { for (int i = 0; i < tp_k; ++i) fprintf(stderr, "%s %.2f | ", tp_n[i], tp_t[i]); fprintf(stderr, "\n"); } }
    bool is_lorenzo(int64_t bb) const { return (ind_bits[bb >> 3] >> (7 - (bb & 7))) & 1; }
    size_t count_lorenzo(int64_t bb, int64_t b_end) const {
        size_t ones = 0;
        for (; bb < b_end && (bb & 7); ++bb) ones += is_lorenzo(bb);
        for (; bb + 64 <= b_end; bb += 64) { uint64_t w8; memcpy(&w8, ind_bits + (bb >> 3), 8); ones += (size_t)__builtin_popcountll(w8); }
        for (; bb < b_end; ++bb) ones += is_lorenzo(bb);
        return ones;
    }
    size_t chains_done() const {
        size_t p = reg_count;
        for (int e = 0; e < ncoef; ++e) { const size_t d = __atomic_load_n(&chain_done[e], __ATOMIC_ACQUIRE); if (d < p) p = d; }
        return p;
    }
    int launch_fit(hipStream_t s_, int um, T mn) {
        if (fit_tile) hipLaunchKernelGGL((k_fit_tile<T>), dim3((unsigned)((int64_t)ncols * ft_nseg)), dim3(64), 0, s_, G, d_in, d_coef, d_lor, noise, um, mn, sm + SM_MINMAX, ft_nseg);
        else hipLaunchKernelGGL((k_fit_select<T>), dim3((unsigned)((nb + 255) / 256)), dim3(256), 0, s_, G, d_in, d_coef, d_lor, noise, um, mn, sm + SM_MINMAX);
        HIPCHK(hipGetLastError());
        return SZHIP_OK;
    }
    int launch_pack_lor(hipStream_t s_) {
        hipLaunchKernelGGL(k_pack_lor, dim3((unsigned)((ind_bytes + 255) / 256)), dim3(256), 0, s_, (const uint8_t *)d_lor, nb, (uint8_t *)ctx->lor_bits.p, sm + SM_NREG);
        HIPCHK(hipGetLastError());
        HIPCHK(hipMemcpyAsync(ind_bits, ctx->lor_bits.p, ind_bytes, hipMemcpyDeviceToHost, s_));
        HIPCHK(hipMemcpyAsync(nreg_h, sm + SM_NREG, 8, hipMemcpyDeviceToHost, s_));
        return SZHIP_OK;
    }
    int stage_and_fit(const void *data, int data_on_device) {
        TRY(stage_input(ctx, data, data_on_device, (size_t)n, &d_in));
        TRY(clear_small(ctx, &sm));
        static const u64 minmax_init[2] = {~0ull, 0ull};
        HIPCHK(hipMemcpyAsync(sm + SM_MINMAX, minmax_init, 16, hipMemcpyHostToDevice, st));
        TRY(ensure(ctx, ctx->coef, (size_t)nb * 4 * sizeof(T)));
        TRY(ensure(ctx, ctx->blk_lor, (size_t)nb));
        d_coef = (T *)ctx->coef.p;
        d_lor = (uint8_t *)ctx->blk_lor.p;
        HIPCHK(hipEventRecord(ctx->ev[0], st));
        TP("ev0");
        HIPCHK(hipEventRecord(ctx->ev_in, st));
        HIPCHK(hipStreamWaitEvent(ctx->stream2, ctx->ev_in, 0));
        noise = (T)((double)eb * (two_d ? 0.81 : 1.22));
        fit_tile = !two_d && szh_ft::applies<T>(G, d_in) && tune_int("SZ_HIP_FIT_TILE", 0) != 0;
        ft_nseg = (G.g2.num + szh_ft::shape<T>::SEGB - 1) / szh_ft::shape<T>::SEGB;
        TRY(launch_fit(ctx->stream2, 0, (T)0));
        ind_bytes = ((size_t)nb + 7) / 8;
        TRY(ensure(ctx, ctx->lor_bits, ind_bytes + 8));
        TRY(ensure_pinned2(ctx, ind_bytes + 32));
        ind_bits = (unsigned char *)ctx->pinned2 + 32;
        nreg_h = (u64 *)ctx->pinned2;
        minmax_h = (u64 *)ctx->pinned2 + 2;
        TRY(launch_pack_lor(ctx->stream2));
        HIPCHK(hipMemcpyAsync(minmax_h, sm + SM_MINMAX, 16, hipMemcpyDeviceToHost, ctx->stream2));
        HIPCHK(hipEventRecord(ctx->ev_fit, ctx->stream2));
        return SZHIP_OK;
    }
    int choose_intervals() {
        intervals = prm->quantization_intervals;
        const unsigned max_radius = prm->max_quant_intervals / 2;
        if (intervals == 0) {
            const int64_t md = (int64_t)(int)std::sqrt((double)n);
            const szh_meanwalk w = two_d ? szh_make_meanwalk(n, INT64_MAX / 2, INT64_MAX / 2, md) : szh_make_meanwalk(n, G.d0, G.g2.count, md);
            int64_t M = 0, M_hi = n / std::max<int64_t>(md - 2, 1) + 2;
            while (szh_meanwalk_pos(w, M_hi) < n) M_hi *= 2;
            while (M < M_hi) { int64_t mid = (M + M_hi) / 2; if (szh_meanwalk_pos(w, mid) >= n) M_hi = mid; else M = mid + 1; }
            TRY(ensure(ctx, ctx->samples, (size_t)M * sizeof(T)));
            TRY(ensure_pinned(ctx, std::max<size_t>((size_t)M * sizeof(T), (size_t)(max_radius + 8192) * 4 + 64)));
            hipLaunchKernelGGL((k_gather_mean<T>), dim3((unsigned)((M + 255) / 256)), dim3(256), 0, st, d_in, w, M, (T *)ctx->samples.p);
            HIPCHK(hipGetLastError());
            HIPCHK(hipMemcpyAsync(ctx->pinned, ctx->samples.p, (size_t)M * sizeof(T), hipMemcpyDeviceToHost, st));
            TP("mean enqueued");
            HIPCHK(hipStreamSynchronize(st));
            TP("mean on host");
            double h0 = now_ms();
            const double smean = szhost_seq_mean(is_double, ctx->pinned, (size_t)M);
            host_ms += now_ms() - h0;
            TRY(ensure(ctx, ctx->hist, (size_t)(max_radius + 8192) * 4 + 64));
            unsigned *d_rh = (unsigned *)ctx->hist.p, *d_fh = d_rh + max_radius;
            HIPCHK(hipMemsetAsync(d_rh, 0, (size_t)(max_radius + 8192) * 4, st));
            const int64_t nrows = szh_sample_row_limit(G, prm->sample_distance);
            if (!two_d && (G.g0.count <= 1 || G.g1.count <= 1)) {
                hipLaunchKernelGGL((k_sample_walk<T, true>), dim3(1), dim3(64), 0, st, G, d_in, prm->sample_distance, (double)eb, (T)smean, max_radius, d_rh, d_fh, sm + SM_WITHIN);
                HIPCHK(hipGetLastError());
            } else if (nrows > 0) {
                int grid = (int)std::min<int64_t>((nrows + 255) / 256, 1024);
                hipLaunchKernelGGL((k_sample<T, true>), dim3(grid), dim3(256), 0, st, G, d_in, nrows, prm->sample_distance, (double)eb, (T)smean, max_radius, d_rh, d_fh, sm + SM_WITHIN);
                HIPCHK(hipGetLastError());
            }
            unsigned *s_hist = (unsigned *)ctx->pinned;
            u64 within = 0;
            HIPCHK(hipMemcpyAsync(s_hist, d_rh, (size_t)(max_radius + 8192) * 4, hipMemcpyDeviceToHost, st));
            HIPCHK(hipMemcpyAsync(&within, sm + SM_WITHIN, 8, hipMemcpyDeviceToHost, st));
            TP("sample enqueued");
            HIPCHK(hipStreamSynchronize(st));
            TP("sample on host");
            h0 = now_ms();
            u64 sample_count = 0;
            for (unsigned i = 0; i < max_radius; ++i) sample_count += s_hist[i];
            szhost_decision dec;
            szhost_decide(is_double, s_hist, max_radius, s_hist + max_radius, sample_count, within, prm->pred_threshold, (double)eb, smean, &dec);
            host_ms += now_ms() - h0;
            intervals = dec.intervals; use_mean = two_d ? 0 : dec.use_mean;
            if (use_mean) {
                T *d_sum = (T *)(sm + SM_MEANSUM);
                hipLaunchKernelGGL((k_mean_seq<T>), dim3(1), dim3(64), 0, st, d_in, n, (T)dec.dense_pos, eb, d_sum, sm + SM_MEANCNT);
                HIPCHK(hipGetLastError());
                T hsum = 0; u64 hcnt = 0;
                HIPCHK(hipMemcpyAsync(&hsum, d_sum, sizeof(T), hipMemcpyDeviceToHost, st));
                HIPCHK(hipMemcpyAsync(&hcnt, sm + SM_MEANCNT, 8, hipMemcpyDeviceToHost, st));
                HIPCHK(hipStreamSynchronize(st));
                if (hcnt > 0) mean = hsum / (T)hcnt;
            }
        }
        if (intervals > 65536 || intervals < 4) FAIL(SZHIP_ERR_UNSUP, "quantization interval count %u outside [4,65536]", intervals);
        S.intervals = intervals; S.use_mean = use_mean;
        return SZHIP_OK;
    }
    int join_fit() {
        HIPCHK(hipStreamWaitEvent(st, ctx->ev_fit, 0));
        if (use_mean) {
            TRY(launch_fit(st, use_mean, mean));
            HIPCHK(hipMemsetAsync(sm + SM_NREG, 0, 8, st));
            TRY(launch_pack_lor(st));
            HIPCHK(hipStreamSynchronize(st));
        } else HIPCHK(hipEventSynchronize(ctx->ev_fit));
        TP("fit joined");
        reg_count = (size_t)*nreg_h;
        S.n_reg_blocks = reg_count;
        if (reg_count == 0 && ctx->chain_pool) ctx->chain_pool->disarm();
        meta_own.assign(meta, meta + meta_len);
        if (prm->flags & SZHIP_RANGE_FROM_DATA) {
            if (meta_len < 4 + 20 + 2 * sizeof(T)) FAIL(SZHIP_ERR_ARG, "parameter bytes too short for a range field");
            const T lo = (T)ord_dec<T>(minmax_h[0]), hi = (T)ord_dec<T>(minmax_h[1]);
            const T range = hi - lo, top = lo + range;
            unsigned char *q = meta_own.data() + 4 + 20;
            if (is_double) { szhost_put_f64be(q, (double)lo); szhost_put_f64be(q + 8, (double)top); }
            else { szhost_put_f32be(q, (float)lo); szhost_put_f32be(q + 4, (float)top); }
            S.vmin = (double)lo; S.vmax = (double)hi;
            if ((double)range <= eb_in) {
                HIPCHK(hipStreamSynchronize(ctx->stream2)); HIPCHK(hipStreamSynchronize(st));
                *out = nullptr; *out_size = 0;
                S.ms_total = now_ms() - t_begin;
                return SZHIP_CONSTANT;
            }
        }
        meta = meta_own.data();
        return SZHIP_OK;
    }
    void make_section(int e) {
        std::vector<uint32_t> h32(65536, 0);
        for (size_t i = 0; i < reg_count; ++i) h32[(size_t)cf.codes[e][i]]++;
        const huff_ptr ch(szhost_huff_build(131072, h32.data(), nullptr, 65536));
        if (!ch) { section_failed = 1; return; }
        const size_t tb = szhost_huff_tree_size(ch.get());
        const size_t enc_cap = (size_t)((ch->total_bits + 7) / 8) + 16;
        if (sizeof(T) + 12 + tb + 8 + enc_cap + 4 + cf.unpred_count[e] * sizeof(T) > ctx->sec_pin_cap[e]) { section_failed = 1; return; }
        unsigned char *const sec0 = ctx->sec_pin[e];
        unsigned char *q = sec0;
        if (is_double) szhost_put_f64be(q, cf.prec[e]); else szhost_put_f32be(q, (float)cf.prec[e]);
        q += sizeof(T);
        szhost_put_u32be(q, 32768); q += 4;
        szhost_put_u32be(q, (uint32_t)tb); q += 4;
        szhost_put_u32be(q, (uint32_t)ch->n_nodes); q += 4;
        szhost_huff_tree_write(ch.get(), q); q += tb;
        const size_t enc = szhost_huff_encode_i32(ch.get(), cf.codes[e], reg_count, q + 8);
        szhost_put_u64be(q, enc); q += 8 + enc;
        szhost_put_u32be(q, (uint32_t)cf.unpred_count[e]); q += 4;
        memcpy(q, cf.unpred[e], cf.unpred_count[e] * sizeof(T)); q += cf.unpred_count[e] * sizeof(T);
        sec_len[e] = (size_t)(q - sec0);
    }
    int prepare_chains() {
        for (int e = 0; e < ncoef; ++e) {
            const size_t bound = sizeof(T) + 12 + (13 * 2 * std::min<size_t>(reg_count, 65536) + 16) + 8 + (8 * reg_count + 16) + 4 + reg_count * sizeof(T) + 64;
            if (ctx->sec_pin_cap[e] < bound) {
                HIPCHK(hipStreamSynchronize(ctx->stream2)); HIPCHK(hipStreamSynchronize(st));
                if (ctx->sec_pin[e]) { HIPCHK(hipHostFree(ctx->sec_pin[e])); ctx->sec_pin[e] = nullptr; ctx->sec_pin_cap[e] = 0; }
                HIPCHK(hipHostMalloc((void **)&ctx->sec_pin[e], bound + bound / 8, hipHostMallocDefault));
                ctx->sec_pin_cap[e] = bound + bound / 8;
            }
        }
        TRY(ensure(ctx, ctx->reg_flags, (size_t)nb * 8));
        TRY(ensure(ctx, ctx->reg_rank, (size_t)nb * 8));
        TRY(ensure(ctx, ctx->coef_compact, reg_count * 4 * sizeof(T)));
        hipLaunchKernelGGL(k_reg_flags, dim3((unsigned)((nb + 255) / 256)), dim3(256), 0, st, (const uint8_t *)d_lor, nb, (u64 *)ctx->reg_flags.p);
        TRY(scan_u64(ctx, (const u64 *)ctx->reg_flags.p, nb, (u64 *)ctx->reg_rank.p, sm + SM_SCRATCH));
        hipLaunchKernelGGL((k_move_coef<T, 0>), dim3((unsigned)((nb + 255) / 256)), dim3(256), 0, st, (const uint8_t *)d_lor, (const u64 *)ctx->reg_rank.p, nb, (int64_t)reg_count, d_coef, (T *)ctx->coef_compact.p);
        HIPCHK(hipGetLastError());
#ifndef SZH_SYNC_LAUNCH
        overlap = !beam_applies<T>(G, d_in, reg_count) && !two_d && !ctx->gate && !ctx->no_chain_overlap && g_compress_calls.load() <= 1;
        if (overlap) { TRY(probe_streams(ctx)); overlap = ctx->streams_independent == 1; }
#endif
        feed = beam_applies<T>(G, d_in, reg_count) && !ctx->gate && !ctx->no_chain_overlap && g_compress_calls.load() <= 1 && tune_int("SZ_HIP_BEAM_FEED", 1) &&
               G.g0.num >= 2 && reg_count >= (size_t)tune_int("SZ_HIP_FEED_MIN_REG", 65536);
#ifndef SZH_SYNC_LAUNCH
        feed = feed && (G.d0 % 128) == 0;
        if (feed) { TRY(probe_streams(ctx)); feed = ctx->streams_independent == 1; }
#endif
        if (feed) feed = fed_guard.try_raise();
        TRY(ensure_pinned3(ctx, reg_count * 4 * sizeof(T) + (overlap ? ((size_t)nb + 64) * 4 * sizeof(T) + 256 : 0)));
        hcoef = (T *)ctx->pinned3;
        return SZHIP_OK;
    }
    int run_chains() {
        chain_avail = reg_count;
        struct AvailAll {
            size_t *p; size_t v;
            ~AvailAll() { __atomic_store_n(p, v, __ATOMIC_RELEASE); }
        } avail_all{&chain_avail, reg_count};
        const size_t first_piece = (size_t)std::max(1, tune_int("SZ_HIP_CHAIN_EARLY_PIECE", 32768));
        two_pieces = feed && reg_count >= 4 * first_piece;
        if (two_pieces) {
            for (int e = 0; e < 4; ++e)
                HIPCHK(hipMemcpyAsync(hcoef + (size_t)e * reg_count, (const T *)ctx->coef_compact.p + (size_t)e * reg_count, first_piece * sizeof(T), hipMemcpyDeviceToHost, st));
            HIPCHK(hipEventRecord(ctx->ev_sec, st));
            for (int e = 0; e < 4; ++e)
                HIPCHK(hipMemcpyAsync(hcoef + (size_t)e * reg_count + first_piece, (const T *)ctx->coef_compact.p + (size_t)e * reg_count + first_piece, (reg_count - first_piece) * sizeof(T), hipMemcpyDeviceToHost, st));
            chain_avail = 0;
            HIPCHK(hipEventSynchronize(ctx->ev_sec));
            __atomic_store_n(&chain_avail, first_piece, __ATOMIC_RELEASE);
        } else {
            HIPCHK(hipMemcpyAsync(hcoef, ctx->coef_compact.p, reg_count * 4 * sizeof(T), hipMemcpyDeviceToHost, st));
            HIPCHK(hipStreamSynchronize(st));
        }
        TP("coef on host");
        double h0 = now_ms();
        all_reg_keep.assign(reg_count, 0);
        TP("chain begin");
        const unsigned char *const ind = all_reg_keep.data();
        T *const chain_in = hcoef + (two_d ? reg_count : 0);
        szhost_coeff_chain_begin(is_double, ind, reg_count, (double)eb, G.g0.late, G.g1.late, G.g2.late, ncoef, &cf);
        if (ctx->chain_codes.size() < reg_count * 4) ctx->chain_codes.resize(reg_count * 4 + reg_count / 4);
        if (ctx->chain_unpred.size() < reg_count * 4 * sizeof(T)) ctx->chain_unpred.resize((reg_count * 4 + reg_count / 4) * sizeof(T));
        for (int e = 0; e < 4; ++e) {
            free(cf.codes[e]); free(cf.unpred[e]);
            cf.codes[e] = ctx->chain_codes.data() + (size_t)e * reg_count;
            cf.unpred[e] = ctx->chain_unpred.data() + (size_t)e * reg_count * sizeof(T);
        }
        cf_own = true;
        if (overlap) {
            blk_of_rank.resize(reg_count);
            size_t r = 0;
            for (int64_t bb = 0; bb < nb && r < reg_count; ++bb) if (!is_lorenzo(bb)) blk_of_rank[r++] = (uint32_t)bb;
            if (r != reg_count) FAIL(SZHIP_ERR_INTERNAL, "indicator bits and regression-block count disagree");
            for (int e = 0; e < 4; ++e) chain_done[e] = 0;
            for (int e = 0; e < ncoef; ++e)
                section_threads.emplace_back([this, e, chain_in, ind] {
                    szhost_coeff_chain_one_p(is_double, chain_in, ind, reg_count, use_mean, e, &cf, &chain_done[e]);
                    make_section(e);
                });
        } else {
            if (!ctx->chain_pool) { ctx->chain_pool = new szhip_chain_pool(); ctx->chain_pool->start(); }
            pool_busy = true;
            for (int e = 0; e < 4; ++e) chain_done[e] = feed && e >= ncoef ? reg_count : 0;
            const size_t *const avail_ptr = two_pieces ? &chain_avail : nullptr;
            ctx->chain_pool->submit(ncoef, [this, chain_in, ind, avail_ptr](int e) {
                    chain_t0[e] = now_ms() - t_begin;
                    szhost_coeff_chain_one_pa(is_double, chain_in, ind, reg_count, use_mean, e, &cf, feed ? &chain_done[e] : nullptr, avail_ptr);
                    chain_t1[e] = now_ms() - t_begin;
                }, [this](int e) { make_section(e); });
            if (two_pieces) {
                HIPCHK(hipStreamSynchronize(st));
                __atomic_store_n(&chain_avail, reg_count, __ATOMIC_RELEASE);
            }
            if (!feed) ctx->chain_pool->wait_chains();
        }
        if (!feed) host_ms += now_ms() - h0;
        TP("chain done");
        if (tp_on) fprintf(stderr, "chain threads: %.2f-%.2f %.2f-%.2f %.2f-%.2f %.2f-%.2f | ", chain_t0[0], chain_t1[0], chain_t0[1], chain_t1[1], chain_t0[2], chain_t1[2], chain_t0[3], chain_t1[3]);
        if (!overlap && !feed) {
            HIPCHK(hipMemcpyAsync(ctx->coef_compact.p, hcoef, reg_count * 4 * sizeof(T), hipMemcpyHostToDevice, st));
            hipLaunchKernelGGL((k_move_coef<T, 1>), dim3((unsigned)((nb + 255) / 256)), dim3(256), 0, st, (const uint8_t *)d_lor, (const u64 *)ctx->reg_rank.p, nb, (int64_t)reg_count, d_coef, (T *)ctx->coef_compact.p);
            HIPCHK(hipGetLastError());
        }
        return SZHIP_OK;
    }
    int feed_slices(const szh_qargs<T> &a) {
        const double h1 = now_ms();
        const int NF = std::max(2, std::min(G.g0.num, 12));
        const int64_t per_row = (int64_t)G.g1.num * G.g2.num;
        size_t r_lo = 0; int b0_lo = 0;
        for (int sl = 0; sl < NF; ++sl) {
            const int b0_hi = sl == NF - 1 ? G.g0.num : std::max(b0_lo, (int)((int64_t)G.g0.num * (sl + 1) / NF));
            if (b0_hi == b0_lo && sl != NF - 1) continue;
            size_t r_hi = reg_count;
            if (b0_hi < G.g0.num) r_hi = r_lo + ((size_t)(b0_hi - b0_lo) * per_row - count_lorenzo(b0_lo * per_row, b0_hi * per_row));
            unsigned idle = 0;
            while (chains_done() < r_hi) {
                szhip_chain_pool::pause();
                if (++idle > (1u << 28)) FAIL(SZHIP_ERR_INTERNAL, "coefficient chain made no progress");
            }
            const int planes_end = b0_hi >= G.g0.num ? G.g0.count : szh_blk_start(G.g0, b0_hi);
            TRY((feed_beam_slice<T>(ctx, G, a, ctx->stream2, hcoef, reg_count, r_lo, r_hi, b0_lo, b0_hi, planes_end, (const u64 *)ctx->reg_rank.p, nb)));
            r_lo = r_hi; b0_lo = b0_hi;
        }
        host_ms += now_ms() - h1;
        S.chain_overlapped = 2;
        return SZHIP_OK;
    }
    int ship_coefs(unsigned epoch, szh_u64 *coh_prog, T *dec, int64_t nbp) {
        const double h1 = now_ms();
        const szh_u64 tag = (szh_u64)(epoch & 0xffffffu) << 40;
        T *const full = (T *)(((uintptr_t)(hcoef + reg_count * 4) + 127) & ~(uintptr_t)127);
        const size_t chunk = std::max<size_t>(2048, reg_count / 32);
        size_t shipped = 0; int64_t sent = 0;
        int idle = 0;
        while (sent < nb) {
            const size_t p = chains_done();
            if (p > shipped && (p - shipped >= chunk || p == reg_count)) {
                for (int e = 0; e < ncoef; ++e)
                    for (size_t r = shipped; r < p; ++r) full[(size_t)e * nbp + blk_of_rank[r]] = hcoef[(size_t)e * reg_count + r];
                shipped = p;
                const int64_t fin = p == reg_count ? nb : (int64_t)blk_of_rank[p];
                const int64_t upto = fin == nb ? nb : fin / LINE * LINE;
                if (upto > sent) {
                    for (int e = 0; e < ncoef; ++e)
                        HIPCHK(hipMemcpyAsync(dec + (size_t)e * nbp + sent, full + (size_t)e * nbp + sent, (size_t)(upto - sent) * sizeof(T), hipMemcpyHostToDevice, ctx->stream2));
                    HIPCHK(hipStreamSynchronize(ctx->stream2));
                    __atomic_store_n(coh_prog, tag | (szh_u64)upto, __ATOMIC_RELEASE);
                    sent = upto;
                }
                idle = 0;
            } else if (++idle > 200000) FAIL(SZHIP_ERR_INTERNAL, "coefficient chain made no progress");
            else std::this_thread::sleep_for(std::chrono::microseconds(10));
        }
        host_ms += now_ms() - h1;
        S.chain_overlapped = 1;
        TP("coefficients shipped");
        return SZHIP_OK;
    }
    int launch_sweep() {
        TRY(ensure(ctx, ctx->codes_nat, (size_t)n * 2 + 64));
        TRY(ensure(ctx, ctx->codes_blk, (size_t)n * 2 + 64));
        d_nat = (uint16_t *)ctx->codes_nat.p; d_blk = (uint16_t *)ctx->codes_blk.p;
        int nI, nJ, ntiles;
        using TS = szh_tile_shape<T>;
        TRY(prepare_pencil(ctx, G, szh_gran<T>::NW, TS::TPI, TS::TPJ, &nI, &nJ, &ntiles));
        const szh_bm::grid_t bgrid = szh_bm::make_grid(G);
        beam_words = (size_t)bgrid.nKB * bgrid.nJG * szh_bm::WPG;
        if (P.sliced) {
            TRY(ensure_coherent(ctx, 512 + beam_words * 4));
            tile_done = (unsigned *)((char *)ctx->coh + 512);
            if (!ctx->stream3) HIPCHK(hipStreamCreateWithFlags(&ctx->stream3, hipStreamNonBlocking));
            if (!ctx->ev_perm) HIPCHK(hipEventCreateWithFlags(&ctx->ev_perm, hipEventDisableTiming));
        }
        szh_qargs<T> a; memset(&a, 0, sizeof(a));
        a.tile_done = tile_done; a.pub_lines = 32;
        a.G = G; a.data = d_in; a.out = nullptr; a.codes = d_nat; a.blk_lor = d_lor; a.coef = d_coef; a.coef_stride = nb;
        a.eb = eb; a.recip = 1 / eb; a.mean = mean; a.cap = (int)intervals; a.radius = (int)intervals / 2; a.use_mean = use_mean;
        a.faceI = (szh_u64 *)ctx->faceI.p; a.faceJ = (szh_u64 *)ctx->faceJ.p; a.epoch = ++ctx->epoch;
        a.nI = nI; a.nJ = nJ; a.order = (const unsigned *)ctx->order.p; a.no_reg = reg_count == 0;
        a.ticket = (unsigned *)(sm + SM_TICKET); a.err = (unsigned *)(sm + SM_ERR); a.ticket_mode = ctx->ticket_atomic ? 0 : tune_int("SZ_HIP_TICKET_MODE", 2);
        a.progress = (szh_u64 *)ctx->progress.p; a.backoff = SZH_FILL_BACKOFF; a.wide = pencil_wide<T>(G, nJ);
        a.coef_progress = nullptr;
        szh_u64 *coh_prog = nullptr;
        T *dec = nullptr;
        const int64_t nbp = (nb + LINE - 1) / LINE * LINE;
        if (overlap) {
            TRY(ensure_coherent(ctx, 256));
            TRY(ensure(ctx, ctx->coef_dec, (size_t)nbp * 4 * sizeof(T)));
            coh_prog = (szh_u64 *)ctx->coh;
            dec = (T *)ctx->coef_dec.p;
            a.coef_progress = coh_prog;
            a.coef = dec; a.coef_stride = nbp;
        }
        HIPCHK(hipEventRecord(ctx->ev[2], st));
        if (P.use_beam) {
#ifdef SZH_SYNC_LAUNCH
            if (feed) {
                TRY(ensure(ctx, ctx->pt_flags, (size_t)G.n + 64)); TRY(ensure(ctx, ctx->rb_vals, (size_t)G.n * sizeof(T) + 64)); TRY(ensure(ctx, ctx->feed_word, 256));
                HIPCHK(hipMemsetAsync(ctx->pt_flags.p, 0, (size_t)G.n, st));
                TRY(feed_slices(a));
                TRY((launch_beam<T, false>(ctx, G, a, st, reg_count, true)));
            } else
#endif
            TRY((launch_beam<T, false>(ctx, G, a, st, reg_count, feed)));
            S.quant_kernel = 2;
#ifndef SZH_SYNC_LAUNCH
            if (feed) TRY(feed_slices(a));
#endif
        } else {
            const unsigned pgrid = pencil_grid(ctx, a, ntiles);
            hipLaunchKernelGGL((k_pencil<T, false>), dim3(pgrid), dim3((TS::TPI * TS::TPJ + 2) * 64), 0, st, a);
            HIPCHK(hipGetLastError());
        }
        HIPCHK(hipEventRecord(ctx->ev[3], st));
        TP("pencil launched");
        S.quant_kernel_launches = 1;
        if (overlap) TRY(ship_coefs(a.epoch, coh_prog, dec, nbp));
        return SZHIP_OK;
    }
    int launch_hist() {
        HIPCHK(hipEventRecord(ctx->ev_in, st));
        HIPCHK(hipStreamWaitEvent(ctx->stream2, ctx->ev_in, 0));
        HIPCHK(hipMemsetAsync(d_hist, 0, (size_t)intervals * 4, ctx->stream2));
        TRY(launch_hist_u16(ctx, ctx->stream2, d_nat, 0, n, intervals, d_hist));
        HIPCHK(hipMemcpyAsync(h_hist, d_hist, (size_t)intervals * 4, hipMemcpyDeviceToHost, ctx->stream2));
        HIPCHK(hipEventRecord(ctx->ev_fit, ctx->stream2));
        return SZHIP_OK;
    }
    int prepare_permute() {
        perm_segb = choose_segb(G, 2, SZH_PERM_TILE_BYTES);
        perm_nseg = (G.g2.num + perm_segb - 1) / perm_segb;
        TRY(ensure(ctx, ctx->zcnt, (size_t)ncols * perm_nseg * 4));
        TRY(ensure(ctx, ctx->zpos, (size_t)ncols * perm_nseg * SZH_ZCAP * 4));
        const size_t tile_el = (tile_bytes(G, perm_segb, 2) + 1) / 2;
        perm_lds = ((tile_el + 1) & ~(size_t)1) * 2 + 16;
        return SZHIP_OK;
    }
    void launch_permute(hipStream_t s_, int col0, int cols) {
        hipLaunchKernelGGL((k_permute<0>), dim3((unsigned)cols, std::min(perm_nseg, std::max(1, tune_int("SZ_HIP_PERM_Y", 1)))), dim3(256), perm_lds, s_, G, (const uint16_t *)d_nat, d_blk,
                           (unsigned *)ctx->col_zeros.p, perm_segb, (unsigned *)ctx->zcnt.p, (unsigned *)ctx->zpos.p, col0);
    }
    int scan_col_zeros(hipStream_t s_) {
        hipLaunchKernelGGL(k_u32_to_u64, dim3((ncols + 255) / 256), dim3(256), 0, s_, (const unsigned *)ctx->col_zeros.p, (int64_t)ncols, (u64 *)ctx->col_zeros64.p);
        return scan_u64(ctx, (const u64 *)ctx->col_zeros64.p, ncols, (u64 *)ctx->col_off.p, sm + SM_TOTAL_UNPRED, s_);
    }
    int permute_all() {
        HIPCHK(hipMemsetAsync(ctx->col_zeros.p, 0, (size_t)ncols * 4, st));
        TRY(prepare_permute());
        launch_permute(st, 0, ncols);
        HIPCHK(hipGetLastError());
        return scan_col_zeros(st);
    }
    int hist_and_order_sliced() {
        const int NS = std::min(P.slices_req, G.g0.num);
        TRY(prepare_permute());
        HIPCHK(hipMemsetAsync(d_hist, 0, (size_t)intervals * 4, ctx->stream2));
        HIPCHK(hipMemsetAsync(ctx->col_zeros.p, 0, (size_t)ncols * 4, ctx->stream3));
        const unsigned tag = (ctx->epoch & 0xfffu) << 20;
        bool sweep_over = false;
        int b0_done = 0;
        int64_t hist_first = 0;
        for (int sl = 0; sl < NS; ++sl) {
            const int b0_hi = sl == NS - 1 ? G.g0.num : std::max(b0_done, (int)((int64_t)G.g0.num * (sl + 1) / NS));
            const int rows_need = b0_hi >= G.g0.num ? G.g0.count : szh_blk_start(G.g0, b0_hi);
            size_t first_late = 0;
            unsigned spins = 0;
            while (!sweep_over && first_late < beam_words) {
                const unsigned wv = __atomic_load_n(&tile_done[first_late], __ATOMIC_ACQUIRE);
                if ((wv & 0xfff00000u) == tag && (int)(wv & 0xfffffu) >= rows_need) { ++first_late; continue; }
                szhip_chain_pool::pause();
                if ((++spins & 127u) == 0) {
                    const hipError_t q = hipEventQuery(ctx->ev[3]);
                    if (q == hipSuccess) { sweep_over = true; break; }
                    if (q != hipErrorNotReady) HIPCHK(q);
                }
            }
            if (b0_hi > b0_done) {
                const int64_t h_lo = hist_first, h_hi = b0_hi >= G.g0.num ? (int64_t)n : ((int64_t)rows_need * G.d0) / 8 * 8;
                hist_first = h_hi;
                if (h_hi > h_lo) TRY(launch_hist_u16(ctx, ctx->stream2, d_nat, h_lo, h_hi, intervals, d_hist));
                if (!P.segenc) launch_permute(ctx->stream3, b0_done * G.g1.num, (b0_hi - b0_done) * G.g1.num);
                HIPCHK(hipGetLastError());
                b0_done = b0_hi;
            }
        }
        HIPCHK(hipMemcpyAsync(h_hist, d_hist, (size_t)intervals * 4, hipMemcpyDeviceToHost, ctx->stream2));
        HIPCHK(hipEventRecord(ctx->ev_fit, ctx->stream2));
        if (!P.segenc) TRY(scan_col_zeros(ctx->stream3));
        HIPCHK(hipEventRecord(ctx->ev_perm, ctx->stream3));
        return SZHIP_OK;
    }
    int hist_and_order() {
        TRY(ensure(ctx, ctx->hist, (size_t)(65536 + 8192) * 4 + 64));
        d_hist = (unsigned *)ctx->hist.p;
        TRY(ensure_pinned(ctx, (size_t)intervals * 4 + 64));
        h_hist = (unsigned *)ctx->pinned;
        if (P.seghist) {
            TRY(ensure(ctx, ctx->seg_hist, (size_t)ncols * intervals * 4));
            HIPCHK(hipMemsetAsync(d_hist, 0, (size_t)intervals * 4, st));
            hipLaunchKernelGGL(k_col_hist, dim3((unsigned)ncols), dim3(256), ((size_t)intervals * 4) << P.sh_rshift, st, G, (const uint16_t *)d_nat, intervals, P.sh_rshift, P.se_vw, (unsigned *)ctx->seg_hist.p);
            hipLaunchKernelGGL(k_hist_reduce, dim3((unsigned)std::min<int64_t>(64, ncols)), dim3(256), 0, st, (const unsigned *)ctx->seg_hist.p, intervals, (int64_t)ncols, d_hist);
            HIPCHK(hipGetLastError());
            if (!P.dev_book) {
                HIPCHK(hipMemcpyAsync(h_hist, d_hist, (size_t)intervals * 4, hipMemcpyDeviceToHost, st));
                HIPCHK(hipEventRecord(ctx->ev_fit, st));
            }
        } else if (!P.sliced) TRY(launch_hist());
        TRY(ensure(ctx, ctx->col_zeros, (size_t)ncols * 4));
        TRY(ensure(ctx, ctx->col_zeros64, (size_t)ncols * 8));
        TRY(ensure(ctx, ctx->col_off, (size_t)ncols * 8));
        if (P.sliced) TRY(hist_and_order_sliced());
        else if (!P.segenc) TRY(permute_all());
        return SZHIP_OK;
    }
    unsigned char *put_front(unsigned char *q) const {
        memcpy(q, meta, meta_len); q += meta_len;
        szhost_put_u64be(q, (uint64_t)n); q += 8;
        szhost_put_u32be(q, (uint32_t)G.block_size); q += 4;
        if (is_double) szhost_put_f64be(q, (double)eb); else szhost_put_f32be(q, (float)eb);
        return q + sizeof(T);
    }
    int upload_segments() {
        se_segs.resize((size_t)P.se_nseg);
        for (int q = 0; q < P.se_nseg; ++q) se_segs[(size_t)q] = szh_se::make_seg(G, 1, q, P.se_segb, P.se_vw);
        TRY(ensure(ctx, ctx->seg_tab, se_segs.size() * sizeof(szh_se::seg_t)));
        HIPCHK(hipMemcpyAsync(ctx->seg_tab.p, se_segs.data(), se_segs.size() * sizeof(szh_se::seg_t), hipMemcpyHostToDevice, st));
        return SZHIP_OK;
    }
    template <class F>
    int pack_columns(unsigned char *d_stream, u64 base_bits, const u64 *d_plan, unsigned maxlen, F &&between) {
        const int64_t nent = (int64_t)ncols;
        TRY(ensure(ctx, ctx->seg_bits, (size_t)nent * 8)); TRY(ensure(ctx, ctx->seg_zeros, (size_t)nent * 8));
        TRY(ensure(ctx, ctx->seg_bitoff, (size_t)nent * 8)); TRY(ensure(ctx, ctx->seg_zoff, (size_t)nent * 8));
        u64 *const bits = (u64 *)ctx->seg_bits.p, *const zeros = (u64 *)ctx->seg_zeros.p, *const bitoff = (u64 *)ctx->seg_bitoff.p, *const zoff = (u64 *)ctx->seg_zoff.p;
        const size_t lb = intervals <= 16384 ? (size_t)intervals : 16;
        if (P.seghist) hipLaunchKernelGGL(k_col_bits_h, dim3((unsigned)((nent + 255) / 256)), dim3(256), 0, st, (const unsigned *)ctx->seg_hist.p, (const uint8_t *)ctx->len_tab.p, intervals, nent, bits, zeros);
        else hipLaunchKernelGGL(k_col_bits, dim3((unsigned)nent), dim3(256), lb, st, G, (const uint16_t *)d_nat, (const uint8_t *)ctx->len_tab.p, intervals, P.se_vw, bits, zeros);
        if (nent <= 1024 * SZH_COL_SCAN_PER && tune_int("SZ_HIP_SEG_SCAN1", 1))
            hipLaunchKernelGGL(k_col_scan, dim3(1), dim3(1024), 0, st, (const u64 *)bits, (const u64 *)zeros, (int)nent, bitoff, zoff, sm + SM_TOTAL_BITS, sm + SM_TOTAL_UNPRED, base_bits, (unsigned *)d_stream, d_plan);
        else {
            TRY(scan_u64(ctx, (const u64 *)bits, nent, bitoff, sm + SM_TOTAL_BITS));
            TRY(scan_u64(ctx, (const u64 *)zeros, nent, zoff, sm + SM_TOTAL_UNPRED));
            hipLaunchKernelGGL(k_col_bounds, dim3((unsigned)((nent + 1 + 255) / 256)), dim3(256), 0, st, (const u64 *)bitoff, nent, (const u64 *)(sm + SM_TOTAL_BITS), base_bits, (unsigned *)d_stream);
        }
        HIPCHK(hipGetLastError());
        TRY(between());
        const unsigned win = (unsigned)szh_se::seg_window_words(G, std::max(1u, maxlen), P.se_nrmax);
        const size_t lds = ((size_t)intervals + 1) * 8 + P.se_tile + 16 + (size_t)win * 4;
        auto encode = [&](auto kernel) {
            hipLaunchKernelGGL(kernel, dim3((unsigned)nent), dim3(256), lds, st, G, (const uint16_t *)d_nat, (const u64 *)ctx->code_tab.p, intervals, (const szh_se::seg_t *)ctx->seg_tab.p, P.se_nseg, P.se_vw,
                               P.se_nrmax, P.se_tile, win, (const u64 *)bitoff, (const u64 *)zoff, base_bits, (unsigned *)d_stream, d_in, (T *)ctx->unpred.p, d_plan);
        };
        if (G.g2.num >= 2 && G.g2.early <= szh_se::INNER && G.g2.late >= szh_se::INNER - 1) encode(k_col_encode<T, true>);
        else encode(k_col_encode<T, false>);
        HIPCHK(hipGetLastError());
        return SZHIP_OK;
    }
    int enqueue_readback() {
        HIPCHK(hipEventRecord(ctx->ev[4], st));
        TP("encode launched");
        HIPCHK(hipMemcpyAsync(h_small, sm, SM_COUNT * 8, hipMemcpyDeviceToHost, st));
        return SZHIP_OK;
    }
    int check_final(bool declined, unsigned book_status, u64 bits, u64 unpred) {
        if ((unsigned)h_small[SM_ERR] == 2) { ctx->coef_late = true; FAIL(SZHIP_ERR_INTERNAL, "wavefront kernel: the regression coefficients did not arrive"); }
        if ((unsigned)h_small[SM_ERR] != 0) { ctx->wave_timeout = true; FAIL(SZHIP_ERR_INTERNAL, "wavefront kernel: halo wait timed out"); }
        if (declined) {
            ctx->book_declined = true;
            snprintf(ctx->err, sizeof(ctx->err), "device code book declined (status %u)", book_status);
            return SZHIP_ERR_INTERNAL;
        }
        if ((bits > 0 && h_small[SM_TOTAL_BITS] != bits) || h_small[SM_TOTAL_UNPRED] != unpred)
            FAIL(SZHIP_ERR_INTERNAL, "entropy stage mismatch (bits %llu vs %llu, unpredictable %llu vs %llu)", (unsigned long long)h_small[SM_TOTAL_BITS],
                 (unsigned long long)bits, (unsigned long long)h_small[SM_TOTAL_UNPRED], (unsigned long long)unpred);
        return SZHIP_OK;
    }
    void finish_stats(size_t len, u64 unpred, int packing, int book_on_device) {
        compress_times(ctx, S, host_ms, t_begin, len);
        S.n_unpred = unpred; S.packing = packing; S.book_on_device = book_on_device;
    }
    int encode_with_device_book() {
        const size_t bk_front = meta_len + 8 + 4 + sizeof(T), bk_mid = 1 + sizeof(T);
        if (!P.seghist) HIPCHK(hipStreamWaitEvent(st, ctx->ev_fit, 0));
        if (!ctx->book_pin) HIPCHK(hipHostMalloc((void **)&ctx->book_pin, 4096, hipHostMallocDefault));
        unsigned char *const blob = (unsigned char *)ctx->book_pin + 256;
        unsigned char *const mid = put_front(blob);
        mid[0] = (unsigned char)use_mean; memcpy(mid + 1, &mean, sizeof(T));
        const size_t plan_fixed = bk_front + 12 + bk_mid + ind_bytes + 8;
        const size_t tree_cap = 1 + (size_t)9 * (2 * SZH_BOOK_CAP - 1);
        const size_t unpred_cap = std::min((size_t)n * sizeof(T), (size_t)n * sizeof(T) / 4 + 65536);
        const bool in_place = out_on_device == 2 && *out && *out_size >= plan_fixed + tree_cap + 64 && ((uintptr_t)*out & 15) == 0 && tune_int("SZ_HIP_OUT_IN_PLACE", 1);
        const size_t stream_cap = in_place ? *out_size : plan_fixed + tree_cap + (size_t)n * sizeof(T) + 65536;
        if (!in_place) TRY(ensure(ctx, ctx->stream_buf, stream_cap));
        unsigned char *d_stream = in_place ? (unsigned char *)*out : (unsigned char *)ctx->stream_buf.p;
        TRY(ensure(ctx, ctx->book_stage, bk_front + bk_mid)); TRY(ensure(ctx, ctx->book_tree, tree_cap)); TRY(ensure(ctx, ctx->book_rec, 32 + SZH_PLAN_COUNT * 8));
        TRY(ensure(ctx, ctx->code_tab, (size_t)intervals * 8)); TRY(ensure(ctx, ctx->len_tab, (size_t)intervals));
        TRY(ensure(ctx, ctx->unpred, unpred_cap + 64));
        szh_book_rec *const d_rec = (szh_book_rec *)ctx->book_rec.p;
        u64 *const d_plan = (u64 *)((char *)ctx->book_rec.p + 32);
        HIPCHK(hipMemcpyAsync(ctx->book_stage.p, blob, bk_front + bk_mid, hipMemcpyHostToDevice, st));
        hipLaunchKernelGGL(k_huff_book, dim3(1), dim3(256), 0, st, (const unsigned *)d_hist, intervals, SZH_BOOK_TAB_SEG, (unsigned char *)ctx->book_tree.p, (unsigned)tree_cap,
                           (u64 *)ctx->code_tab.p, (uint8_t *)ctx->len_tab.p, d_rec, d_plan, (u64)plan_fixed, (unsigned)sizeof(T), (u64)stream_cap, (u64)unpred_cap);
        HIPCHK(hipGetLastError());
        TRY(upload_segments());
        TRY(pack_columns(d_stream, 0, (const u64 *)d_plan, 32u, [&]() -> int {
            hipLaunchKernelGGL(k_book_tail, dim3((unsigned)std::min<size_t>(64, (plan_fixed + tree_cap + 255) / 256)), dim3(256), 0, st, d_stream, (const unsigned char *)ctx->book_stage.p, (unsigned)bk_front,
                               (unsigned)bk_mid, intervals, (const unsigned char *)ctx->lor_bits.p, ind_bytes, (const unsigned char *)ctx->book_tree.p, (const szh_book_rec *)d_rec, (const u64 *)d_plan);
            return SZHIP_OK;
        }));
        hipLaunchKernelGGL((k_book_unpred<T>), dim3((unsigned)std::min<size_t>(256, (unpred_cap / sizeof(T) + 255) / 256)), dim3(256), 0, st, d_stream, (const T *)ctx->unpred.p, (const szh_book_rec *)d_rec, (const u64 *)d_plan);
        HIPCHK(hipGetLastError());
        TRY(enqueue_readback());
        HIPCHK(hipMemcpyAsync(ctx->book_pin, ctx->book_rec.p, 32 + SZH_PLAN_COUNT * 8, hipMemcpyDeviceToHost, st));
        HIPCHK(hipStreamSynchronize(st));
        TP("final sync");
        szh_book_rec rec; memcpy(&rec, ctx->book_pin, sizeof(rec));
        const u64 *const plan = (const u64 *)ctx->book_pin + 4;
        print_trace();
        TRY(check_final(book_declines(rec.status, plan[SZH_PLAN_STATUS], tune_int("SZ_HIP_TEST_BOOK_FALLBACK", 0)), rec.status ? rec.status : (unsigned)plan[SZH_PLAN_STATUS],
                        rec.total_bits, rec.total_unpred));
        const size_t len = (size_t)plan[SZH_PLAN_TOTAL_LEN];
        TRY(deliver_stream(ctx, d_stream, len, out_on_device, out, out_size, in_place, true));
        finish_stats(len, rec.total_unpred, 1, 1);
        return SZHIP_OK;
    }
    int build_host_book() {
        TP("permute launched");
        HIPCHK(hipEventSynchronize(ctx->ev_fit));
        TP("hist on host");
        double h0 = now_ms();
        const huff_ptr hf = host_book(h_hist, intervals, tab_code, tab_len, &enc_maxlen);
        host_ms += now_ms() - h0;
        total_unpred = h_hist[0];
        if (!hf) FAIL(SZHIP_ERR_INTERNAL, "Huffman build failed");
        TP("tree built");
        join_sections();
        TP("sections joined");
        if (section_failed) FAIL(SZHIP_ERR_INTERNAL, "coefficient Huffman build failed");
        for (int e = 0; e < ncoef; ++e) sections_total += sec_len[e];
        h0 = now_ms();
        const size_t tree_bytes = szhost_huff_tree_size(hf.get());
        pre_len = meta_len + 8 + 4 + sizeof(T) + 4 + 4 + 4 + tree_bytes + 1 + sizeof(T) + ind_bytes;
        hdr_len = pre_len + sections_total + 8;
        unpred_bytes = (size_t)total_unpred * sizeof(T);
        total_len = hdr_len + unpred_bytes + (size_t)((hf->total_bits + 7) / 8);
        TRY(ensure_pinned(ctx, pre_len + 8 + 64));
        hdr = (unsigned char *)ctx->pinned;
        memset(hdr, 0, pre_len + 8);
        unsigned char *q = put_front(hdr);
        szhost_put_u32be(q, intervals); q += 4;
        szhost_put_u32be(q, (uint32_t)tree_bytes); q += 4;
        szhost_put_u32be(q, (uint32_t)hf->n_nodes); q += 4;
        szhost_huff_tree_write(hf.get(), q); q += tree_bytes;
        *q++ = (unsigned char)use_mean;
        memcpy(q, &mean, sizeof(T)); q += sizeof(T);
        memcpy(q, ind_bits, ind_bytes); q += ind_bytes;
        const uint64_t tu = total_unpred; memcpy(q, &tu, 8);
        total_bits = hf->total_bits;
        lds_e32 = (size_t)intervals * 8 + ((size_t)SZH_E32_ROUND * enc_maxlen / 32 + 4) * 4 + 16;
        enc32 = enc_maxlen >= 1 && enc_maxlen <= 32 && lds_e32 <= 60 * 1024 && tune_int("SZ_HIP_ENC32", 1);
        if (P.revise(enc_maxlen)) {
            if (P.sliced) HIPCHK(hipStreamWaitEvent(st, ctx->ev_perm, 0));
            TRY(permute_all());
        }
        if (P.segenc) TRY(upload_segments());
        if (P.segenc) for (unsigned s = 0; s < intervals; ++s) tab_code[s] = (tab_code[s] << 32) | tab_len[s] | (s == 0 ? 0x10000u : 0u);
        else if (enc32) for (unsigned s = 0; s < intervals; ++s) tab_code[s] = (tab_code[s] << 8) | tab_len[s];
        host_ms += now_ms() - h0;
        return upload_code_tables(ctx, tab_code, tab_len);
    }
    int copy_header(unsigned char *d_stream) {
        HIPCHK(hipMemcpyAsync(d_stream, hdr, pre_len, hipMemcpyHostToDevice, st));
        HIPCHK(hipMemcpyAsync(d_stream + pre_len + sections_total, hdr + pre_len, 8, hipMemcpyHostToDevice, st));
        if (sections_total) {
            const hipStream_t ssec = ctx->stream3 ? ctx->stream3 : ctx->stream2;
            HIPCHK(hipEventRecord(ctx->ev_feed, st));
            HIPCHK(hipStreamWaitEvent(ssec, ctx->ev_feed, 0));
            size_t off = pre_len;
            for (int e = 0; e < ncoef; ++e) { HIPCHK(hipMemcpyAsync(d_stream + off, ctx->sec_pin[e], sec_len[e], hipMemcpyHostToDevice, ssec)); off += sec_len[e]; }
            HIPCHK(hipEventRecord(ctx->ev_sec, ssec));
        }
        return SZHIP_OK;
    }
    int pack_block_ordered(unsigned char *d_stream) {
        const u64 base_bits = (u64)(hdr_len + unpred_bytes) * 8;
        if (P.sliced) HIPCHK(hipStreamWaitEvent(st, ctx->ev_perm, 0));
        if (total_unpred > 0) {
            TRY(ensure(ctx, ctx->unpred, unpred_bytes));
            HIPCHK(hipEventRecord(ctx->ev_in, st));
            HIPCHK(hipStreamWaitEvent(ctx->stream2, ctx->ev_in, 0));
            hipLaunchKernelGGL((k_unpred<T, 0>), dim3(ncols), dim3(256), 0, ctx->stream2, G, (const uint16_t *)d_blk, (const unsigned *)ctx->col_zeros.p,
                               (const u64 *)ctx->col_off.p, d_in, (T *)ctx->unpred.p, (T *)nullptr, (const unsigned *)ctx->zcnt.p, (const unsigned *)ctx->zpos.p, perm_segb, perm_nseg);
            HIPCHK(hipGetLastError());
            HIPCHK(hipEventRecord(ctx->ev_fit, ctx->stream2));
        }
        if (total_bits > 0) {
            TRY(chunk_bit_offsets(ctx, d_blk, n, intervals, sm, 64));
            if (enc32) {
                const int64_t nrounds = (n + SZH_E32_ROUND - 1) / SZH_E32_ROUND;
                hipLaunchKernelGGL(k_encode32, dim3((unsigned)((nrounds + SZH_E32_PER - 1) / SZH_E32_PER)), dim3(256), lds_e32, st, (const uint16_t *)d_blk, n, (const u64 *)ctx->code_tab.p,
                                   intervals, (const u64 *)ctx->chunk_off.p, base_bits, (unsigned *)d_stream);
                HIPCHK(hipGetLastError());
            } else
                TRY(launch_encode(ctx, d_blk, n, intervals, base_bits, d_stream));
        }
        if (total_unpred > 0) HIPCHK(hipStreamWaitEvent(st, ctx->ev_fit, 0));
        return SZHIP_OK;
    }
    int encode_with_host_book() {
        TRY(build_host_book());
        const bool in_place = out_on_device == 2 && *out && *out_size >= total_len + 64 && ((uintptr_t)*out & 15) == 0 && tune_int("SZ_HIP_OUT_IN_PLACE", 1);
        if (!in_place) TRY(ensure(ctx, ctx->stream_buf, total_len + 64));
        unsigned char *d_stream = in_place ? (unsigned char *)*out : (unsigned char *)ctx->stream_buf.p;
        if (P.segenc) {
            TRY(pack_columns(d_stream, (u64)(hdr_len + unpred_bytes) * 8, (const u64 *)nullptr, enc_maxlen, [&]() -> int {
                TRY(copy_header(d_stream));
                return ensure(ctx, ctx->unpred, unpred_bytes + 64);
            }));
        } else {
            HIPCHK(hipMemsetAsync(d_stream, 0, total_len + 64, st));
            TRY(copy_header(d_stream));
            TRY(pack_block_ordered(d_stream));
        }
        if (total_unpred > 0) HIPCHK(hipMemcpyAsync(d_stream + hdr_len, ctx->unpred.p, unpred_bytes, hipMemcpyDeviceToDevice, st));
        if (sections_total) HIPCHK(hipStreamWaitEvent(st, ctx->ev_sec, 0));
        TRY(enqueue_readback());
        TRY(deliver_stream(ctx, d_stream, total_len, out_on_device, out, out_size, in_place, false));
        TP("final sync");
        print_trace();
        const int rc = check_final(false, 0, total_bits, total_unpred);
        if (rc != SZHIP_OK) {
            if (!out_on_device && *out) { free(*out); *out = nullptr; }
            *out_size = 0;
            return rc;
        }
        finish_stats(total_len, total_unpred, P.segenc ? 1 : 0, 0);
        return SZHIP_OK;
    }
};

template <class T>
int compress_impl(szhip_ctx *ctx, const void *data, int data_on_device, size_t r0, size_t r1, size_t r2, double eb_in, const szhip_params *prm, const unsigned char *meta, size_t meta_len, int out_on_device,
                  unsigned char **out, size_t *out_size, szhip_stats *stats)
{
    sz21_call<T> c(ctx, r0, r1, r2, eb_in, prm, meta, meta_len, out_on_device, out, out_size);
    int rc = c.stage_and_fit(data, data_on_device);
    if (rc == SZHIP_OK) rc = c.choose_intervals();
    if (rc == SZHIP_OK) rc = c.join_fit();
    if (rc == SZHIP_CONSTANT && stats) *stats = c.S;
    if (rc != SZHIP_OK) return rc;
    if (ctx->chain_pool) ctx->chain_pool->arm();
    if (c.reg_count > 0) { TRY(c.prepare_chains()); TRY(c.run_chains()); }
    HIPCHK(hipEventRecord(ctx->ev[1], c.st));
    c.TP("ev1");
    c.P = sz21_make_plan<T>(ctx, c.G, c.intervals, c.reg_count, beam_applies<T>(c.G, c.d_in, c.reg_count), c.overlap, c.feed, meta_len);
    TRY(c.launch_sweep());
    TRY(c.hist_and_order());
    TRY(c.P.dev_book ? c.encode_with_device_book() : c.encode_with_host_book());
    return c.done(stats);
}

#define HDEC_CHECK(ctx) do { if ((ctx)->hdec_res[1] != 0 || (tune_int("SZ_HIP_TEST_HDEC_FALLBACK", 0) && !(ctx)->hdec_sync_rounds)) { (ctx)->hdec_unconverged = true; \
         \
        snprintf((ctx)->err, sizeof((ctx)->err), "Huffman decode: %llu start guesses still moving after two rounds", (ctx)->hdec_res[1]); return SZHIP_ERR_INTERNAL; } } while (0)
int huff_decode_device(szhip_ctx *ctx, u64 *sm, const unsigned char *d_bits, unsigned bytes_before, u64 total_bits, const std::vector<uint32_t> &dtab, int n_nodes,
                       int single_symbol, int64_t n, uint16_t *d_out_codes)
{
    if (!ctx->hdec_res) HIPCHK(hipHostMalloc((void **)&ctx->hdec_res, 64, hipHostMallocDefault));
    ctx->hdec_res[0] = (u64)n; ctx->hdec_res[1] = 0;
    hipStream_t st = ctx->stream;
    if (single_symbol >= 0) {
        hipLaunchKernelGGL(k_fill_u16, dim3((unsigned)((n + 255) / 256)), dim3(256), 0, st, d_out_codes, n, (uint16_t)single_symbol);
        HIPCHK(hipGetLastError());
    } else {
        const int64_t nsub = (int64_t)((total_bits + SZH_SUBSEQ_BITS - 1) / SZH_SUBSEQ_BITS);
        if (nsub == 0) FAIL(SZHIP_ERR_STREAM, "empty Huffman payload");
        const size_t lut_off = (dtab.size() * 4 + 63) / 64 * 64;
        TRY(ensure(ctx, ctx->dec_tab, lut_off + SZH_LUT_BYTES));
        HIPCHK(hipMemcpyAsync(ctx->dec_tab.p, dtab.data(), dtab.size() * 4, hipMemcpyHostToDevice, st));
        hipLaunchKernelGGL(k_hdec_build_lut, dim3(SZH_LUT_SIZE / 256), dim3(256), 0, st, (const unsigned *)ctx->dec_tab.p, (uint4 *)((char *)ctx->dec_tab.p + lut_off));
        TRY(ensure(ctx, ctx->starts, (size_t)nsub * 8)); TRY(ensure(ctx, ctx->ends, (size_t)nsub * 8));
        TRY(ensure(ctx, ctx->counts, (size_t)nsub * 8)); TRY(ensure(ctx, ctx->offs, (size_t)nsub * 8));
        TRY(ensure(ctx, ctx->dirty, (size_t)nsub));
        szh_hdec_args a;
        a.bits = d_bits; a.total_bits = total_bits; a.bytes_before = bytes_before; a.table = (const unsigned *)ctx->dec_tab.p; a.n_nodes = n_nodes;
        a.table_in_lds = (size_t)n_nodes * 8 <= 13 * 1024; a.nsub = nsub;
        a.lut = (const uint4 *)((char *)ctx->dec_tab.p + lut_off);
        a.starts = (u64 *)ctx->starts.p; a.ends = (u64 *)ctx->ends.p; a.counts = (u64 *)ctx->counts.p;
        a.dirty = (unsigned char *)ctx->dirty.p; a.changed = (unsigned *)(sm + SM_CHANGED);
        const size_t lds_tab = a.table_in_lds ? (size_t)n_nodes * 8 : 16;
        const size_t lds_pass = SZH_HDEC_LDS + SZH_LUT_SIZE * 4 + lds_tab, lds_write = SZH_HDEC_LDS + SZH_LUT_SIZE * 16 + lds_tab;
        const unsigned gsub = (unsigned)((nsub + 255) / 256);
        hipLaunchKernelGGL(k_hdec_init, dim3(gsub), dim3(256), 0, st, a);
        const bool optimistic = !ctx->hdec_sync_rounds;
        constexpr int64_t opt_rounds = 3;
        int64_t iter = 0;
        for (;;) {
            a.warmup = iter == 0;
            hipLaunchKernelGGL(k_hdec_pass, dim3(gsub), dim3(256), lds_pass, st, a);
            HIPCHK(hipMemsetAsync(sm + SM_CHANGED, 0, 8, st));
            hipLaunchKernelGGL(k_hdec_update, dim3(gsub), dim3(256), 0, st, a);
            HIPCHK(hipGetLastError());
            if (optimistic) {
                if (iter + 1 < opt_rounds && nsub > 1) { ++iter; continue; }
                HIPCHK(hipMemcpyAsync(&ctx->hdec_res[1], sm + SM_CHANGED, 8, hipMemcpyDeviceToHost, st));
                break;
            }
            unsigned changed = 0;
            HIPCHK(hipMemcpyAsync(&changed, sm + SM_CHANGED, 4, hipMemcpyDeviceToHost, st));
            HIPCHK(hipStreamSynchronize(st));
            if (!changed) break;
            if (++iter > nsub + 2) FAIL(SZHIP_ERR_INTERNAL, "Huffman decode did not converge");
        }
        TRY(scan_u64(ctx, (const u64 *)ctx->counts.p, nsub, (u64 *)ctx->offs.p, sm + SM_TOTAL_SYM));
        HIPCHK(hipMemcpyAsync(&ctx->hdec_res[0], sm + SM_TOTAL_SYM, 8, hipMemcpyDeviceToHost, st));
        hipLaunchKernelGGL(k_hdec_write, dim3(gsub), dim3(256), lds_write, st, a, (const u64 *)ctx->offs.p, d_out_codes, n);
        HIPCHK(hipGetLastError());
    }

    return SZHIP_OK;
}

int check_decoded(szhip_ctx *ctx, int64_t n, u64 listed, u64 zeros_found, const char *what)
{
    HDEC_CHECK(ctx);
    if ((int64_t)ctx->hdec_res[0] < n) FAIL(SZHIP_ERR_STREAM, "Huffman payload holds %llu symbols, need %lld", ctx->hdec_res[0], (long long)n);
    if (zeros_found != listed) FAIL(SZHIP_ERR_STREAM, "stream lists %llu %s values, codes need %llu", (unsigned long long)listed, what, (unsigned long long)zeros_found);
    return SZHIP_OK;
}

template <class T> struct dec_header {
    T eb = 0, mean = 0;
    unsigned intervals = 0; int use_mean = 0;
    dec_table D;
    size_t reg_count = 0, ind_off = 0, unpred_off = 0, pay_off = 0; uint64_t total_unpred = 0;
    std::vector<T> coef;
    bool defer = false;
    std::function<int()> finish; char finish_err[200] = {0};
};

template <class T>
int parse_header(const unsigned char *hs, size_t avail, size_t stream_len, size_t body_off, size_t nb, int want_block_size,
                 dec_header<T> &H, size_t *need, char *err, size_t errlen)
{
    const int ncoef = want_block_size == SZH_BLOCK_SIZE_2D ? 3 : 4;
    const int is_double = sizeof(T) == 8;
#define PFAIL(code, ...) do { snprintf(err, errlen, __VA_ARGS__); return (code); } while (0)
#define NEED(k) do { const size_t end_ = (size_t)(q - hs) + (size_t)(k); if (end_ > stream_len) PFAIL(SZHIP_ERR_STREAM, "truncated stream"); \
                     if (end_ > avail) { *need = std::min(stream_len, end_ + need_more); return 1; } } while (0)
    size_t need_more = 0;
    const unsigned char *q = hs + body_off;
    const int tp_on = tune_int("SZ_HIP_TIMING", 0); const double tp0 = now_ms();
    auto mark = [&](const char *nm) { if (tp_on) fprintf(stderr, "[header %s %.3f] ", nm, now_ms() - tp0); };
    NEED(4 + sizeof(T) + 12);
    const unsigned block_size = szhost_get_u32be(q); q += 4;
    if ((int)block_size != want_block_size) PFAIL(SZHIP_ERR_UNSUP, "block size %u", block_size);
    H.eb = is_double ? (T)szhost_get_f64be(q) : (T)szhost_get_f32be(q); q += sizeof(T);
    H.intervals = szhost_get_u32be(q); q += 4;
    const unsigned tree_size = szhost_get_u32be(q); q += 4;
    const int node_count = (int)szhost_get_u32be(q); q += 4;
    if (H.intervals < 4 || H.intervals > 65536) PFAIL(SZHIP_ERR_STREAM, "bad interval count %u", H.intervals);
    NEED(tree_size);
    if (node_count <= 0 || szhost_huff_serial_size(node_count) > tree_size) PFAIL(SZHIP_ERR_STREAM, "bad Huffman tree size");
    if (!read_tree(q, node_count, H.intervals, H.D)) PFAIL(SZHIP_ERR_STREAM, "bad Huffman tree");
    q += tree_size;
    NEED(1 + sizeof(T));
    H.use_mean = *q++;
    memcpy(&H.mean, q, sizeof(T)); q += sizeof(T);
    const size_t ind_bytes = (nb - 1) / 8 + 1;
    NEED(ind_bytes);
    {
        size_t ones = 0, full = nb / 8;
        for (size_t i = 0; i < full; ++i) ones += (size_t)__builtin_popcount(q[i]);
        for (size_t b = full * 8; b < nb; ++b) ones += (q[b >> 3] >> (7 - (b & 7))) & 1;
// ... 40 lines not shown
            int sec_rc[4] = {0, 0, 0, 0};
            size_t sec_zeros[4] = {0, 0, 0, 0};
            const std::vector<unsigned char> all_reg(reg_count, 0);
            auto decode_section = [&](int e) {
                const huff_ptr ch(szhost_huff_from_bytes(4 * sd[e].crad, sd[e].tree_at, sd[e].cnc));
                if (!ch) { sec_rc[e] = 1; return; }
                std::vector<int> codes(reg_count);
                if (!szhost_huff_decode_i32(ch.get(), sd[e].pay_at, sd[e].enc, reg_count, codes.data())) { sec_rc[e] = 2; return; }
                size_t zeros = 0;
                for (size_t i = 0; i < reg_count; ++i) zeros += codes[i] == 0;
                sec_zeros[e] = zeros;
                if (zeros > sd[e].cu) { sec_rc[e] = 3; return; }
                int *const c1[4] = {codes.data(), nullptr, nullptr, nullptr};
                const int r1[4] = {sd[e].crad, 0, 0, 0}; const double p1[4] = {sd[e].prec, 0, 0, 0}; const unsigned char *const u1[4] = {sd[e].cun, nullptr, nullptr, nullptr};
                szhost_coeff_unchain(is_double, coef_out + (size_t)(e + (ncoef == 3 ? 1 : 0)) * reg_count, all_reg.data(), reg_count, c1, r1, p1, u1, 1);
            };
            if (reg_count >= 16384) {
                std::vector<std::thread> th;
                for (int e = 1; e < ncoef; ++e) th.emplace_back(decode_section, e);
                decode_section(0);
                for (auto &t : th) t.join();
            } else {
                for (int e = 0; e < ncoef; ++e) decode_section(e);
            }
            for (int e = 0; e < ncoef; ++e) {
                if (sec_rc[e] == 1) { snprintf(ferr, 200, "bad coefficient tree"); return SZHIP_ERR_STREAM; }
                if (sec_rc[e] == 2) { snprintf(ferr, 200, "coefficient payload too short"); return SZHIP_ERR_STREAM; }
                if (sec_rc[e] == 3) { snprintf(ferr, 200, "coefficient section lists %u verbatim values, codes need %zu", sd[e].cu, sec_zeros[e]); return SZHIP_ERR_STREAM; }
            }
            return 0;
        };
        if (H.defer && H.reg_count >= (size_t)tune_int("SZ_HIP_DEC_DEFER_MIN", 16384)) H.finish = run_sections;
        else { const int src = run_sections(); if (src) PFAIL(src, "%s", H.finish_err); }
        mark("unchained");
    }
    NEED(8);
    memcpy(&H.total_unpred, q, 8); q += 8;
    H.unpred_off = (size_t)(q - hs);
    if (H.total_unpred > (stream_len - H.unpred_off) / sizeof(T)) PFAIL(SZHIP_ERR_STREAM, "truncated stream");
    H.pay_off = H.unpred_off + (size_t)H.total_unpred * sizeof(T);
    mark("done");
    return 0;
#undef NEED
#undef PFAIL
}

template <class T>
int decompress_impl(szhip_ctx *ctx, const unsigned char *stream_in, int stream_on_device, size_t stream_len, size_t body_off,
                    size_t r0, size_t r1, size_t r2, void *out, int out_on_device, szhip_stats *stats)
{
    const szh_geom3 G = r0 == 0 ? szh_make_geom2((int)r1, (int)r2) : szh_make_geom3((int)r0, (int)r1, (int)r2);
    const int64_t n = G.n, nb = G.nblocks;
    const double t_begin = now_ms();
    double host_ms = 0;
    hipStream_t st = ctx->stream;
    szhip_stats S; memset(&S, 0, sizeof(S));
    S.n_elements = (uint64_t)n; S.n_blocks = (uint64_t)nb;

    std::vector<unsigned char> hcopy;
    const unsigned char *hs = stream_in;
    size_t avail = stream_len;
    TRY(ensure(ctx, ctx->stream_buf, stream_len + 64));
    unsigned char *d_stream = (unsigned char *)ctx->stream_buf.p;
    HIPCHK(hipEventRecord(ctx->ev[0], st));
    bool on_device_copied = false;
    auto copy_on_device = [&]() -> int {
        if (on_device_copied) return SZHIP_OK;
        on_device_copied = true;
        if (stream_in != d_stream) HIPCHK(hipMemcpyAsync(d_stream, stream_in, stream_len, hipMemcpyDeviceToDevice, st));
        HIPCHK(hipMemsetAsync(d_stream + stream_len, 0, 64, st));
        return SZHIP_OK;
    };
    if (stream_on_device) avail = 0;
    else {
        TRY(staged_copy(ctx, d_stream, stream_in, stream_len, true));
        HIPCHK(hipMemsetAsync(d_stream + stream_len, 0, 64, st));
    }

    double h0 = now_ms();
    dec_header<T> H;
    H.defer = true;
    struct Finisher {
        std::thread th; int rc = 0;
        void join() { if (th.joinable()) th.join(); }
        ~Finisher() { join(); }
    } finisher;
    for (size_t want = std::min<size_t>(stream_len, (size_t)256 << 10);;) {
        if (stream_on_device && want > avail) {
            TRY(ensure_pinned(ctx, want));
            HIPCHK(hipMemcpyAsync(ctx->pinned, stream_in, want, hipMemcpyDeviceToHost, st));
            HIPCHK(hipEventRecord(ctx->ev_in, st));
            TRY(copy_on_device());
            HIPCHK(hipEventSynchronize(ctx->ev_in));
            hs = (const unsigned char *)ctx->pinned; avail = want;
        }
        size_t need = 0;
        const int rc = parse_header<T>(hs, avail, stream_len, body_off, (size_t)nb, G.block_size, H, &need, ctx->err, sizeof(ctx->err));
        if (rc == 0) break;
        if (rc < 0) {
            if (on_device_copied) hipStreamSynchronize(st);
            fprintf(stderr, "szhip: %s\n", ctx->err); return rc;
        }
        want = std::min<size_t>(stream_len, std::max<size_t>(need, avail * 2));
    }
    if (stream_on_device) TRY(copy_on_device());
    if (H.finish) finisher.th = std::thread([&] { finisher.rc = H.finish(); });
    if (tune_int("SZ_HIP_TIMING", 0)) fprintf(stderr, "[header on host %.3f ms after the call began]\n", now_ms() - t_begin);
    const T eb = H.eb, mean = H.mean;
    const unsigned intervals = H.intervals;
    const int use_mean = H.use_mean, n_nodes = H.D.n_nodes, single_symbol = H.D.single_symbol;
    const size_t reg_count = H.reg_count, unpred_off = H.unpred_off, pay_off = H.pay_off;
    const uint64_t total_unpred = H.total_unpred;
    std::vector<T> &hcoef = H.coef;
    std::vector<uint32_t> &dtab = H.D.dtab;
    const u64 total_bits = (u64)(stream_len - pay_off) * 8;
    S.intervals = intervals; S.use_mean = use_mean; S.n_reg_blocks = reg_count; S.n_unpred = total_unpred;
    host_ms += now_ms() - h0;

    u64 *sm = nullptr;
    TRY(clear_small(ctx, &sm));
    const size_t nat_elems = (size_t)n;
    const bool dec_beam = beam_applies<T>(G, out_on_device ? (const void *)out : (const void *)nullptr, reg_count);
    TRY(ensure(ctx, ctx->codes_nat, nat_elems * 2 + 64));
    TRY(ensure(ctx, ctx->codes_blk, (size_t)n * 2 + 64));
    uint16_t *d_nat = (uint16_t *)ctx->codes_nat.p, *d_blk = (uint16_t *)ctx->codes_blk.p;

    TRY(huff_decode_device(ctx, sm, d_stream + pay_off, (unsigned)std::min<size_t>(pay_off, 4096), total_bits, dtab, n_nodes, single_symbol, n, d_blk));

    const int ncols = G.g0.num * G.g1.num;
    TRY(ensure(ctx, ctx->col_zeros, (size_t)ncols * 4));
    TRY(ensure(ctx, ctx->col_zeros64, (size_t)ncols * 8));
    TRY(ensure(ctx, ctx->col_off, (size_t)ncols * 8));
    int perm_segb = 1, perm_nseg = 1;
    T *d_out = nullptr;
    TRY(device_out(ctx, out, out_on_device, (size_t)n, &d_out));
    T *d_sweep = d_out;
    const int up_vw = (G.g2.count % 8) == 0 ? 8 : ((G.g2.count % 4) == 0 ? 4 : 1);
    int up_segb = 0, up_nseg = 0; size_t up_lds = 0;
    bool col_unpack = dec_beam && tune_int("SZ_HIP_COL_UNPACK", 1) != 0 && ((uintptr_t)d_blk & 15) == 0 && (double)n < 4.0e9;
    if (col_unpack) {
        const size_t rows_max = (size_t)G.g0.early * G.g1.early, want = (size_t)std::max(4, tune_int("SZ_HIP_UNPACK_TILE_KB", 24)) * 1024;
        int sb = 1;
        while (sb < G.g2.num && (rows_max * (size_t)(sb + 1) * G.g2.early + 16) * 2 <= want) ++sb;
        up_segb = sb; up_nseg = (G.g2.num + sb - 1) / sb;
        up_lds = ((rows_max * (size_t)sb * G.g2.early + 16) * 2 + 15) & ~(size_t)15;
        if (up_lds > 63 * 1024 || rows_max > 128) col_unpack = false;
    }
    std::vector<szh_se::seg_t> up_segs;
    if (col_unpack) {
        hipLaunchKernelGGL(k_col_zeros, dim3((unsigned)ncols), dim3(256), 0, st, G, (const uint16_t *)d_blk, (unsigned *)ctx->col_zeros.p);
        HIPCHK(hipGetLastError());
        up_segs.resize((size_t)up_nseg);
        for (int q = 0; q < up_nseg; ++q) up_segs[(size_t)q] = szh_se::make_seg(G, 1, q, up_segb, up_vw);
        TRY(ensure(ctx, ctx->seg_tab, up_segs.size() * sizeof(szh_se::seg_t)));
        HIPCHK(hipMemcpyAsync(ctx->seg_tab.p, up_segs.data(), up_segs.size() * sizeof(szh_se::seg_t), hipMemcpyHostToDevice, st));
    } else
    {
        HIPCHK(hipMemsetAsync(ctx->col_zeros.p, 0, (size_t)ncols * 4, st));
        const int segb = choose_segb(G, 2, SZH_PERM_TILE_BYTES);
        const int nseg = (G.g2.num + segb - 1) / segb;
        TRY(ensure(ctx, ctx->zcnt, (size_t)ncols * nseg * 4));
        TRY(ensure(ctx, ctx->zpos, (size_t)ncols * nseg * SZH_ZCAP * 4));
        hipLaunchKernelGGL((k_permute<1>), dim3(ncols, std::min(nseg, std::max(1, tune_int("SZ_HIP_PERM_Y", nseg)))), dim3(256), tile_bytes(G, segb, 2), st, G, (const uint16_t *)d_blk, d_nat,
                           (unsigned *)ctx->col_zeros.p, segb, (unsigned *)ctx->zcnt.p, (unsigned *)ctx->zpos.p, 0);
        perm_segb = segb; perm_nseg = nseg;
        HIPCHK(hipGetLastError());
    }
    if (col_unpack && ncols <= 1024 * SZH_COL_SCAN_PER && tune_int("SZ_HIP_SEG_SCAN1", 1)) {
        hipLaunchKernelGGL(k_col_zscan, dim3(1), dim3(1024), 0, st, (const unsigned *)ctx->col_zeros.p, (int)ncols, (u64 *)ctx->col_off.p, sm + SM_TOTAL_UNPRED);
        HIPCHK(hipGetLastError());
    } else {
        hipLaunchKernelGGL(k_u32_to_u64, dim3((ncols + 255) / 256), dim3(256), 0, st, (const unsigned *)ctx->col_zeros.p, (int64_t)ncols,
                           (u64 *)ctx->col_zeros64.p);
        TRY(scan_u64(ctx, (const u64 *)ctx->col_zeros64.p, ncols, (u64 *)ctx->col_off.p, sm + SM_TOTAL_UNPRED));
    }
    ctx->hdec_res[2] = 0;
    HIPCHK(hipMemcpyAsync(&ctx->hdec_res[2], sm + SM_TOTAL_UNPRED, 8, hipMemcpyDeviceToHost, st));
    auto decoder_checks = [&]() { return check_decoded(ctx, n, total_unpred, ctx->hdec_res[2], "unpredictable"); };
    const bool checks_last = col_unpack && tune_int("SZ_HIP_DEC_CHECKS_LAST", 1) != 0;
    if (!checks_last) {
        HIPCHK(hipStreamSynchronize(st));
        TRY(decoder_checks());
    }
    if (col_unpack) {
        TRY(ensure(ctx, ctx->unpred, (size_t)total_unpred * sizeof(T) + 64));
        if (total_unpred > 0) HIPCHK(hipMemcpyAsync(ctx->unpred.p, d_stream + unpred_off, (size_t)total_unpred * sizeof(T), hipMemcpyDeviceToDevice, st));
        hipLaunchKernelGGL((k_col_unpack<T>), dim3((unsigned)ncols), dim3(256), up_lds, st, G, (const uint16_t *)d_blk, d_nat, (const szh_se::seg_t *)ctx->seg_tab.p, up_nseg, up_vw,
                           (const u64 *)ctx->col_off.p, (const T *)ctx->unpred.p, (u64)total_unpred, d_sweep);
        HIPCHK(hipGetLastError());
    } else
    if (total_unpred > 0) {
        TRY(ensure(ctx, ctx->unpred, (size_t)total_unpred * sizeof(T)));
        HIPCHK(hipMemcpyAsync(ctx->unpred.p, d_stream + unpred_off, (size_t)total_unpred * sizeof(T), hipMemcpyDeviceToDevice, st));
        hipLaunchKernelGGL((k_unpred<T, 1>), dim3(ncols), dim3(256), 0, st, G, (const uint16_t *)d_blk, (const unsigned *)ctx->col_zeros.p,
                           (const u64 *)ctx->col_off.p, (const T *)nullptr, (T *)ctx->unpred.p, d_sweep, (const unsigned *)ctx->zcnt.p,
                           (const unsigned *)ctx->zpos.p, perm_segb, perm_nseg);
        HIPCHK(hipGetLastError());
    }
    TRY(ensure(ctx, ctx->coef, (size_t)nb * 4 * sizeof(T)));
    TRY(ensure(ctx, ctx->blk_lor, (size_t)nb));

    hipLaunchKernelGGL(k_unpack_lor, dim3((unsigned)((nb + 255) / 256)), dim3(256), 0, st, (const uint8_t *)(d_stream + H.ind_off), nb,
                       (uint8_t *)ctx->blk_lor.p);
    HIPCHK(hipGetLastError());
    if (reg_count > 0) {
        TRY(ensure(ctx, ctx->reg_flags, (size_t)nb * 8));
        TRY(ensure(ctx, ctx->reg_rank, (size_t)nb * 8));
        TRY(ensure(ctx, ctx->coef_compact, reg_count * 4 * sizeof(T)));
        {
            const double hj = now_ms();
            finisher.join();
            host_ms += now_ms() - hj;
            if (tune_int("SZ_HIP_TIMING", 0)) fprintf(stderr, "[sections joined %.3f ms after the call began, waited %.3f]\n", now_ms() - t_begin, now_ms() - hj);
            if (finisher.rc) { snprintf(ctx->err, sizeof(ctx->err), "%s", H.finish_err); fprintf(stderr, "szhip: %s\n", ctx->err); return finisher.rc; }
        }
        TRY(ensure_pinned3(ctx, hcoef.size() * sizeof(T)));
        memcpy(ctx->pinned3, hcoef.data(), hcoef.size() * sizeof(T));
        HIPCHK(hipMemcpyAsync(ctx->coef_compact.p, ctx->pinned3, hcoef.size() * sizeof(T), hipMemcpyHostToDevice, st));
        hipLaunchKernelGGL(k_reg_flags, dim3((unsigned)((nb + 255) / 256)), dim3(256), 0, st, (const uint8_t *)ctx->blk_lor.p, nb, (u64 *)ctx->reg_flags.p);
        TRY(scan_u64(ctx, (const u64 *)ctx->reg_flags.p, nb, (u64 *)ctx->reg_rank.p, sm + SM_SCRATCH));
        hipLaunchKernelGGL((k_move_coef<T, 1>), dim3((unsigned)((nb + 255) / 256)), dim3(256), 0, st, (const uint8_t *)ctx->blk_lor.p,
                           (const u64 *)ctx->reg_rank.p, nb, (int64_t)reg_count, (T *)ctx->coef.p, (T *)ctx->coef_compact.p);
        HIPCHK(hipGetLastError());
    }
    HIPCHK(hipEventRecord(ctx->ev[1], st));

    int nI, nJ, ntiles;
    using TS = szh_tile_shape<T>;
    TRY(prepare_pencil(ctx, G, szh_gran<T>::NW, TS::TPI, TS::TPJ, &nI, &nJ, &ntiles));
    {
        szh_qargs<T> a; memset(&a, 0, sizeof(a));
        a.G = G; a.data = nullptr; a.out = d_out; a.codes = d_nat; a.blk_lor = (const uint8_t *)ctx->blk_lor.p; a.coef = (const T *)ctx->coef.p; a.coef_stride = nb;
        a.eb = eb; a.recip = 1 / eb; a.mean = mean; a.cap = (int)intervals; a.radius = (int)intervals / 2; a.use_mean = use_mean;
        a.faceI = (szh_u64 *)ctx->faceI.p; a.faceJ = (szh_u64 *)ctx->faceJ.p; a.epoch = ++ctx->epoch;
        a.nI = nI; a.nJ = nJ; a.order = (const unsigned *)ctx->order.p; a.no_reg = reg_count == 0;
        a.ticket = (unsigned *)(sm + SM_TICKET); a.err = (unsigned *)(sm + SM_ERR); a.ticket_mode = ctx->ticket_atomic ? 0 : tune_int("SZ_HIP_TICKET_MODE", 2);
        a.progress = (szh_u64 *)ctx->progress.p; a.backoff = SZH_FILL_BACKOFF; a.wide = pencil_wide<T>(G, nJ);
        HIPCHK(hipEventRecord(ctx->ev[2], st));
        if (dec_beam) {
            TRY((launch_beam<T, true>(ctx, G, a, st, reg_count))); S.quant_kernel = 2;
        }
        else {
        const unsigned pgrid = pencil_grid(ctx, a, ntiles);
        hipLaunchKernelGGL((k_pencil<T, true>), dim3(pgrid), dim3((TS::TPI * TS::TPJ + 2) * 64), 0, st, a);
        HIPCHK(hipGetLastError());
        }
        HIPCHK(hipEventRecord(ctx->ev[3], st));
        S.quant_kernel_launches = 1;
    }
    unsigned kerr = 0;
    HIPCHK(hipMemcpyAsync(&kerr, sm + SM_ERR, 4, hipMemcpyDeviceToHost, st));
    TRY(return_out(ctx, out, out_on_device, d_out, (size_t)n));
    HIPCHK(hipEventRecord(ctx->ev[4], st));
    HIPCHK(hipStreamSynchronize(st));
    if (checks_last) TRY(decoder_checks());
    if (kerr) { ctx->wave_timeout = true; FAIL(SZHIP_ERR_INTERNAL, "wavefront kernel: halo wait timed out"); }
    decompress_times(ctx, S, host_ms, t_begin, (size_t)n * sizeof(T));
    if (stats) *stats = S;
    return SZHIP_OK;
}
```

Measured before the change: 383.8.

## Publish device results to coherent host memory and poll instead of stream syncs

Kernels such as mean gather, sample histogram and code histogram now write their results straight into coherent mapped host memory. A last-block arrival counter then publishes a sequence word with a system-scope release store, and the host spins on that word in place of hipStreamSynchronize plus D2H memcpys. Header assembly is moved later, code and length tables go up in a single pinned copy, and the thread-pool workers spin briefly before falling back to the condition variable. This targets the host-device round-trip latency on the compression critical path, at the cost of CPU spinning, system fences and more complex correctness logic.

```diff
diff --git a/sz_amd/csrc/szh_segenc.h b/sz_amd/csrc/szh_segenc.h
--- a/sz_amd/csrc/szh_segenc.h
+++ b/sz_amd/csrc/szh_segenc.h
@@ -107,7 +107,8 @@
         col_hist[(size_t)blockIdx.x * nbins + b] = t;
     }
 }
-__global__ __launch_bounds__(256) void k_hist_reduce(const unsigned *__restrict__ col_hist, unsigned nbins, int64_t ncols, unsigned *__restrict__ hist)
+__global__ __launch_bounds__(256) void k_hist_reduce(const unsigned *__restrict__ col_hist, unsigned nbins, int64_t ncols, unsigned *hist,
+                                                     unsigned *arrive = nullptr, unsigned *host_hist = nullptr, u64 *word = nullptr, u64 seq = 0)
 {
     __shared__ unsigned acc[SZH_COL_HBINS];
     for (unsigned b = threadIdx.x; b < nbins; b += 256) acc[b] = 0;
@@ -121,6 +122,10 @@
     }
     __syncthreads();
     for (unsigned b = threadIdx.x; b < nbins; b += 256) if (acc[b]) atomicAdd(&hist[b], acc[b]);
+    if (word && szh_publish_last(arrive)) {
+        for (unsigned b = threadIdx.x; b < nbins; b += 256) host_hist[b] = __hip_atomic_load(&hist[b], __ATOMIC_RELAXED, __HIP_MEMORY_SCOPE_AGENT);
+        szh_publish_word(word, seq);
+    }
 }
 __global__ __launch_bounds__(256) void k_col_bits_h(const unsigned *__restrict__ col_hist, const uint8_t *__restrict__ len, unsigned nbins, int64_t ncols, u64 *__restrict__ col_bits, u64 *__restrict__ col_zeros)
 {
diff --git a/sz_amd/csrc/szhip.hip b/sz_amd/csrc/szhip.hip
--- a/sz_amd/csrc/szhip.hip
+++ b/sz_amd/csrc/szhip.hip
@@ -136,6 +136,11 @@
     int streams_independent = -1;
     void *coh = nullptr; size_t coh_cap = 0;
     int order_nI = -1, order_nJ = -1;
+    void *pub = nullptr; size_t pub_cap = 0; unsigned long long pub_seq = 0; unsigned pub_radius = 0; size_t pub_hi_r = 0, pub_hi_f = 0;
+    hipEvent_t ev_pub = nullptr;
+    unsigned long long *pin_words = nullptr;
+    void *tab_pin = nullptr; size_t tab_pin_cap = 0;
+    struct seg_key_t { int d[3], segb, vw; bool operator==(const seg_key_t &o) const { return d[0] == o.d[0] && d[1] == o.d[1] && d[2] == o.d[2] && segb == o.segb && vw == o.vw; } } seg_key = {{0, 0, 0}, 0, 0};
     bool wave_timeout = false, ticket_atomic = false;
     bool coef_late = false, no_chain_overlap = false;
     bool book_declined = false, no_dev_book = false;
@@ -290,21 +295,35 @@
     std::vector<szhip_pool_job> jobs;
     std::vector<bool> used;
     bool stop = false;
+    std::atomic<int> pending{0};
+    std::array<std::atomic<int>, 64> done_word{};
 };
+static void szhip_pool_spin(const std::atomic<int> &word)
+{
+    const int bound_us = tune_int("SZ_HIP_POOL_SPIN_US", 50);
+    if (bound_us <= 0) return;
+    const long long t0 = mono_us();
+    for (unsigned k = 1; word.load(std::memory_order_acquire) == 0; ++k) {
+        szhip_chain_pool::pause();
+        if ((k & 63u) == 0 && mono_us() - t0 >= bound_us) return;
+    }
+}
 static void szhip_pool_worker(szhip_pool *p, int lane)
 {
     for (;;) {
         int t;
+        szhip_pool_spin(p->pending);
         {
             std::unique_lock<std::mutex> lk(p->mu);
             p->cv_work.wait(lk, [&] { return p->stop || !p->queue.empty(); });
             if (p->queue.empty()) return;
             t = p->queue.front(); p->queue.pop_front();
+            p->pending.fetch_sub(1, std::memory_order_relaxed);
         }
         szhip_pool_job &j = p->jobs[t];
         j.rc = szhip_compress(p->ctx[lane], j.dtype, j.data, j.on_dev, j.r0, j.r1, j.r2, j.eb, &j.prm, j.meta, j.meta_len, j.out_on_device,
                               &j.out, &j.out_size, &j.stats);
-        { std::lock_guard<std::mutex> lk(p->mu); j.done = true; }
+        { std::lock_guard<std::mutex> lk(p->mu); j.done = true; p->done_word[(size_t)t].store(1, std::memory_order_release); }
         p->cv_done.notify_all();
     }
 }
@@ -349,7 +368,9 @@
     j.meta = meta; j.meta_len = meta_len; j.out_on_device = out_on_device; j.out = out_on_device == 2 ? out_buf : nullptr;
     j.out_size = out_on_device == 2 ? out_cap : 0; j.rc = SZHIP_ERR_INTERNAL; j.done = false;
     p->used[t] = true;
+    p->done_word[(size_t)t].store(0, std::memory_order_relaxed);
     p->queue.push_back(t);
+    p->pending.fetch_add(1, std::memory_order_release);
     *ticket = t;
     p->cv_work.notify_one();
     return SZHIP_OK;
@@ -357,6 +378,7 @@
 int szhip_pool_wait(szhip_pool *p, int ticket, unsigned char **out, size_t *out_size, szhip_stats *stats)
 {
     if (!p || ticket < 0 || ticket >= (int)p->jobs.size()) return SZHIP_ERR_ARG;
+    szhip_pool_spin(p->done_word[(size_t)ticket]);
     std::unique_lock<std::mutex> lk(p->mu);
     if (!p->used[ticket]) return SZHIP_ERR_ARG;
     p->cv_done.wait(lk, [&] { return p->jobs[ticket].done; });
diff --git a/sz_amd/csrc/szhip_kernels.h b/sz_amd/csrc/szhip_kernels.h
--- a/sz_amd/csrc/szhip_kernels.h
+++ b/sz_amd/csrc/szhip_kernels.h
@@ -305,11 +305,61 @@
     }
 }
 
+__device__ __forceinline__ void szh_fence_system()
+{
+#ifndef SZH_HIPSIM
+    __threadfence_system();
+#endif
+}
+__device__ __forceinline__ bool szh_publish_last(unsigned *arrive)
+{
+    __shared__ unsigned last;
+    szh_fence_system();
+    __syncthreads();
+    if (threadIdx.x == 0) {
+        const unsigned before = atomicAdd(arrive, 1u);
+        last = before + 1u == gridDim.x * gridDim.y ? 1u : 0u;
+        if (last) szh_fence_system();
+    }
+    __syncthreads();
+    return last != 0u;
+}
+__device__ __forceinline__ void szh_publish_word(u64 *word, u64 seq)
+{
+    szh_fence_system();
+    __syncthreads();
+    if (threadIdx.x == 0) __hip_atomic_store(word, seq, __ATOMIC_RELEASE, __HIP_MEMORY_SCOPE_SYSTEM);
+}
+__global__ void k_arm_small(u64 *sm, int count, int minmax_at)
+{
+    const int i = (int)threadIdx.x;
+    if (i < count) sm[i] = i == minmax_at ? ~0ull : 0ull;
+}
+
 template <class T>
-__global__ __launch_bounds__(256) void k_gather_mean(const T *__restrict__ data, szh_meanwalk w, int64_t count, T *out)
+__global__ __launch_bounds__(256) void k_gather_mean(const T *__restrict__ data, szh_meanwalk w, int64_t count, T *out, unsigned *arrive = nullptr, u64 *word = nullptr, u64 seq = 0)
 {
     const int64_t m = (int64_t)blockIdx.x * 256 + threadIdx.x;
     if (m < count) out[m] = data[szh_meanwalk_pos(w, m)];
+    if (word && szh_publish_last(arrive)) szh_publish_word(word, seq);
+}
+__global__ __launch_bounds__(1024) void k_publish_sample(const unsigned *__restrict__ radius_hist, unsigned max_radius, const unsigned *__restrict__ freq_hist, unsigned freq_bins,
+                                                         const u64 *__restrict__ within, unsigned *host_radius, unsigned *host_freq, u64 *hdr, u64 *word, u64 seq)
+{
+    __shared__ u64 sh_sum[16], sh_hr[16], sh_hf[16];
+    const int lane = (int)threadIdx.x & 63, wid = (int)threadIdx.x >> 6;
+    u64 sum = 0, hr = 0, hf = 0;
+    for (unsigned i = threadIdx.x; i < max_radius; i += 1024) { const unsigned v = radius_hist[i]; sum += v; if (v) hr = (u64)i + 1; }
+    for (unsigned i = threadIdx.x; i < freq_bins; i += 1024) if (freq_hist[i]) hf = (u64)i + 1;
+    sum = wave_sum_u64(sum); hr = wave_max_u64(hr); hf = wave_max_u64(hf);
+    if (lane == 0) { sh_sum[wid] = sum; sh_hr[wid] = hr; sh_hf[wid] = hf; }
+    __syncthreads();
+    sum = 0; hr = 0; hf = 0;
+    for (int q = 0; q < 16; ++q) { sum += sh_sum[q]; hr = sh_hr[q] > hr ? sh_hr[q] : hr; hf = sh_hf[q] > hf ? sh_hf[q] : hf; }
+    for (unsigned i = threadIdx.x; i < (unsigned)hr; i += 1024) host_radius[i] = radius_hist[i];
+    for (unsigned i = threadIdx.x; i < (unsigned)hf; i += 1024) host_freq[i] = freq_hist[i];
+    if (threadIdx.x == 0) { hdr[0] = hr; hdr[1] = hf; hdr[2] = sum; hdr[3] = *within; }
+    szh_publish_word(word, seq);
 }
 
 #define SZH_LDS_RADIUS_BINS 4096
diff --git a/sz_amd/csrc/szhip_rt.inc b/sz_amd/csrc/szhip_rt.inc
--- a/sz_amd/csrc/szhip_rt.inc
+++ b/sz_amd/csrc/szhip_rt.inc
@@ -55,9 +55,40 @@
     if (ctx->coh_cap != had) memset(ctx->coh, 0, ctx->coh_cap);
     return SZHIP_OK;
 }
+int tune_int(const char *name, int def);
 
 enum { SM_MINMAX = 0, SM_WITHIN = 2, SM_MEANCNT = 3, SM_TOTAL_UNPRED = 4, SM_TOTAL_BITS = 5, SM_TICKET = 6, SM_ERR = 7,
-       SM_CHANGED = 8, SM_MEANSUM = 9, SM_TOTAL_SYM = 10, SM_NREG = 11, SM_SCRATCH = 12, SM_COUNT = 16 };
+       SM_CHANGED = 8, SM_MEANSUM = 9, SM_TOTAL_SYM = 10, SM_NREG = 11, SM_SCRATCH = 12, SM_ARRIVE = 15, SM_COUNT = 16 };
+
+enum { PUB_MEAN = 0, PUB_SAMPLE = 8, PUB_HIST = 16, PUB_SAMPLE_HDR = 24, PUB_AREAS = 32 };
+int ensure_pub(szhip_ctx *ctx, size_t bytes)
+{
+    if (!ctx->ev_pub) HIPCHK(hipEventCreateWithFlags(&ctx->ev_pub, hipEventDisableTiming));
+    if (!ctx->pin_words) { HIPCHK(hipHostMalloc((void **)&ctx->pin_words, 4096, hipHostMallocDefault)); memset(ctx->pin_words, 0, 4096); }
+    const size_t had = ctx->pub_cap;
+    TRY(ensure_host(ctx, ctx->pub, ctx->pub_cap, PUB_AREAS * 8 + bytes, ctx->stream, hipHostMallocCoherent | hipHostMallocMapped));
+    if (ctx->pub_cap != had) { memset(ctx->pub, 0, ctx->pub_cap); ctx->pub_radius = 0; ctx->pub_hi_r = ctx->pub_hi_f = 0; }
+    return SZHIP_OK;
+}
+int wait_published(szhip_ctx *ctx, const unsigned long long *word, unsigned long long seq, hipEvent_t behind, const char *what)
+{
+    if (tune_int("SZ_HIP_TEST_PUB_LOST", 0)) seq += 1ull << 40;
+    for (unsigned looks = 1;; ++looks) {
+        if (__atomic_load_n(word, __ATOMIC_ACQUIRE) == seq) return SZHIP_OK;
+#ifdef SZH_SYNC_LAUNCH
+        const hipError_t q = hipSuccess;
+        (void)behind;
+#else
+        szhip_chain_pool::pause();
+        if ((looks & 255u) != 0) continue;
+        const hipError_t q = hipEventQuery(behind);
+        if (q == hipErrorNotReady) continue;
+#endif
+        HIPCHK(q);
+        if (__atomic_load_n(word, __ATOMIC_ACQUIRE) == seq) return SZHIP_OK;
+        FAIL(SZHIP_ERR_INTERNAL, "%s: the kernel has ended and its result never came", what);
+    }
+}
 
 int probe_streams(szhip_ctx *ctx)
 {
diff --git a/sz_amd/csrc/szhip_sz21.inc b/sz_amd/csrc/szhip_sz21.inc
--- a/sz_amd/csrc/szhip_sz21.inc
+++ b/sz_amd/csrc/szhip_sz21.inc
@@ -71,7 +71,13 @@
     std::vector<szh_se::seg_t> se_segs; std::vector<u64> tab_code; std::vector<uint8_t> tab_len;
     unsigned enc_maxlen = 0; bool enc32 = false; size_t lds_e32 = 0;
     unsigned char *hdr = nullptr; size_t pre_len = 0, sections_total = 0, hdr_len = 0, unpred_bytes = 0, total_len = 0; u64 total_bits = 0, total_unpred = 0;
-    u64 h_small[SM_COUNT];
+    u64 *h_small = nullptr;
+    enum { PW_MEANSUM = 32, PW_MEANCNT = 33 };
+    huff_ptr hf;
+    const uint8_t *d_len = nullptr;
+    bool sweep_ready = false; szh_qargs<T> qa; int q_ntiles = 0;
+    bool hist_cleared = false;
+    u64 seq_hist = 0;
     szhost_coeffs cf;
     size_t sec_len[4] = {0, 0, 0, 0};
     std::vector<std::thread> section_threads;
@@ -133,13 +139,16 @@
     }
     int stage_and_fit(const void *data, int data_on_device) {
         TRY(stage_input(ctx, data, data_on_device, (size_t)n, &d_in));
-        TRY(clear_small(ctx, &sm));
-        static const u64 minmax_init[2] = {~0ull, 0ull};
-        HIPCHK(hipMemcpyAsync(sm + SM_MINMAX, minmax_init, 16, hipMemcpyHostToDevice, st));
+        TRY(ensure(ctx, ctx->small, SM_COUNT * 8));
+        TRY(ensure_pub(ctx, 0));
+        sm = (u64 *)ctx->small.p;
+        h_small = ctx->pin_words;
         TRY(ensure(ctx, ctx->coef, (size_t)nb * 4 * sizeof(T)));
         TRY(ensure(ctx, ctx->blk_lor, (size_t)nb));
         d_coef = (T *)ctx->coef.p;
         d_lor = (uint8_t *)ctx->blk_lor.p;
+        hipLaunchKernelGGL(k_arm_small, dim3(1), dim3(64), 0, st, sm, (int)SM_COUNT, (int)SM_MINMAX);
+        HIPCHK(hipGetLastError());
         HIPCHK(hipEventRecord(ctx->ev[0], st));
         TP("ev0");
         HIPCHK(hipEventRecord(ctx->ev_in, st));
@@ -168,20 +177,27 @@
             int64_t M = 0, M_hi = n / std::max<int64_t>(md - 2, 1) + 2;
             while (szh_meanwalk_pos(w, M_hi) < n) M_hi *= 2;
             while (M < M_hi) { int64_t mid = (M + M_hi) / 2; if (szh_meanwalk_pos(w, mid) >= n) M_hi = mid; else M = mid + 1; }
-            TRY(ensure(ctx, ctx->samples, (size_t)M * sizeof(T)));
-            TRY(ensure_pinned(ctx, std::max<size_t>((size_t)M * sizeof(T), (size_t)(max_radius + 8192) * 4 + 64)));
-            hipLaunchKernelGGL((k_gather_mean<T>), dim3((unsigned)((M + 255) / 256)), dim3(256), 0, st, d_in, w, M, (T *)ctx->samples.p);
+            TRY(ensure(ctx, ctx->hist, (size_t)(65536 + 8192) * 4 + 64));
+            TRY(ensure_pub(ctx, pub_bytes(max_radius, (size_t)M)));
+            u64 *const pw = (u64 *)ctx->pub;
+            unsigned *const s_hist = (unsigned *)((char *)ctx->pub + pub_sample_off());
+            T *const h_samples = (T *)((char *)ctx->pub + pub_mean_off(max_radius));
+            if (ctx->pub_radius != max_radius) {
+                memset(s_hist, 0, (size_t)(max_radius + 8192) * 4);
+                ctx->pub_radius = max_radius; ctx->pub_hi_r = ctx->pub_hi_f = 0;
+            }
+            const u64 seq_mean = ++ctx->pub_seq;
+            hipLaunchKernelGGL((k_gather_mean<T>), dim3((unsigned)((M + 255) / 256)), dim3(256), 0, st, d_in, w, M, h_samples, (unsigned *)(sm + SM_ARRIVE), pw + PUB_MEAN, seq_mean);
             HIPCHK(hipGetLastError());
-            HIPCHK(hipMemcpyAsync(ctx->pinned, ctx->samples.p, (size_t)M * sizeof(T), hipMemcpyDeviceToHost, st));
+            HIPCHK(hipEventRecord(ctx->ev_pub, st));
+            unsigned *d_rh = (unsigned *)ctx->hist.p, *d_fh = d_rh + max_radius;
+            HIPCHK(hipMemsetAsync(d_rh, 0, (size_t)(max_radius + 8192) * 4, st));
             TP("mean enqueued");
-            HIPCHK(hipStreamSynchronize(st));
+            TRY(wait_published(ctx, pw + PUB_MEAN, seq_mean, ctx->ev_pub, "mean samples"));
             TP("mean on host");
             double h0 = now_ms();
-            const double smean = szhost_seq_mean(is_double, ctx->pinned, (size_t)M);
+            const double smean = szhost_seq_mean(is_double, h_samples, (size_t)M);
             host_ms += now_ms() - h0;
-            TRY(ensure(ctx, ctx->hist, (size_t)(max_radius + 8192) * 4 + 64));
-            unsigned *d_rh = (unsigned *)ctx->hist.p, *d_fh = d_rh + max_radius;
-            HIPCHK(hipMemsetAsync(d_rh, 0, (size_t)(max_radius + 8192) * 4, st));
             const int64_t nrows = szh_sample_row_limit(G, prm->sample_distance);
             if (!two_d && (G.g0.count <= 1 || G.g1.count <= 1)) {
                 hipLaunchKernelGGL((k_sample_walk<T, true>), dim3(1), dim3(64), 0, st, G, d_in, prm->sample_distance, (double)eb, (T)smean, max_radius, d_rh, d_fh, sm + SM_WITHIN);
@@ -191,16 +207,25 @@
                 hipLaunchKernelGGL((k_sample<T, true>), dim3(grid), dim3(256), 0, st, G, d_in, nrows, prm->sample_distance, (double)eb, (T)smean, max_radius, d_rh, d_fh, sm + SM_WITHIN);
                 HIPCHK(hipGetLastError());
             }
-            unsigned *s_hist = (unsigned *)ctx->pinned;
-            u64 within = 0;
-            HIPCHK(hipMemcpyAsync(s_hist, d_rh, (size_t)(max_radius + 8192) * 4, hipMemcpyDeviceToHost, st));
-            HIPCHK(hipMemcpyAsync(&within, sm + SM_WITHIN, 8, hipMemcpyDeviceToHost, st));
+            const u64 seq_sample = ++ctx->pub_seq;
+            ctx->pub_radius = 0;
+            hipLaunchKernelGGL(k_publish_sample, dim3(1), dim3(1024), 0, st, (const unsigned *)d_rh, max_radius, (const unsigned *)d_fh, 8192u, (const u64 *)(sm + SM_WITHIN),
+                               s_hist, s_hist + max_radius, pw + PUB_SAMPLE_HDR, pw + PUB_SAMPLE, seq_sample);
+            HIPCHK(hipGetLastError());
+            HIPCHK(hipEventRecord(ctx->ev_pub, st));
+            HIPCHK(hipMemsetAsync(d_rh, 0, (size_t)SZH_COL_HBINS * 4, st));
+            hist_cleared = true;
             TP("sample enqueued");
-            HIPCHK(hipStreamSynchronize(st));
+            TRY(prepare_sweep());
+            TRY(wait_published(ctx, pw + PUB_SAMPLE, seq_sample, ctx->ev_pub, "sampler's bins"));
             TP("sample on host");
             h0 = now_ms();
-            u64 sample_count = 0;
-            for (unsigned i = 0; i < max_radius; ++i) sample_count += s_hist[i];
+            const size_t hi_r = (size_t)pw[PUB_SAMPLE_HDR], hi_f = (size_t)pw[PUB_SAMPLE_HDR + 1];
+            if (hi_r > max_radius || hi_f > 8192) FAIL(SZHIP_ERR_INTERNAL, "sampler's bins: bounds %zu / %zu", hi_r, hi_f);
+            if (ctx->pub_hi_r > hi_r) memset(s_hist + hi_r, 0, (ctx->pub_hi_r - hi_r) * 4);
+            if (ctx->pub_hi_f > hi_f) memset(s_hist + max_radius + hi_f, 0, (ctx->pub_hi_f - hi_f) * 4);
+            ctx->pub_hi_r = hi_r; ctx->pub_hi_f = hi_f; ctx->pub_radius = max_radius;
+            const u64 sample_count = pw[PUB_SAMPLE_HDR + 2], within = pw[PUB_SAMPLE_HDR + 3];
             szhost_decision dec;
             szhost_decide(is_double, s_hist, max_radius, s_hist + max_radius, sample_count, within, prm->pred_threshold, (double)eb, smean, &dec);
             host_ms += now_ms() - h0;
@@ -209,10 +234,11 @@
                 T *d_sum = (T *)(sm + SM_MEANSUM);
                 hipLaunchKernelGGL((k_mean_seq<T>), dim3(1), dim3(64), 0, st, d_in, n, (T)dec.dense_pos, eb, d_sum, sm + SM_MEANCNT);
                 HIPCHK(hipGetLastError());
-                T hsum = 0; u64 hcnt = 0;
-                HIPCHK(hipMemcpyAsync(&hsum, d_sum, sizeof(T), hipMemcpyDeviceToHost, st));
-                HIPCHK(hipMemcpyAsync(&hcnt, sm + SM_MEANCNT, 8, hipMemcpyDeviceToHost, st));
+                HIPCHK(hipMemcpyAsync(ctx->pin_words + PW_MEANSUM, d_sum, sizeof(T), hipMemcpyDeviceToHost, st));
+                HIPCHK(hipMemcpyAsync(ctx->pin_words + PW_MEANCNT, sm + SM_MEANCNT, 8, hipMemcpyDeviceToHost, st));
                 HIPCHK(hipStreamSynchronize(st));
+                T hsum; memcpy(&hsum, ctx->pin_words + PW_MEANSUM, sizeof(T));
+                const u64 hcnt = ctx->pin_words[PW_MEANCNT];
                 if (hcnt > 0) mean = hsum / (T)hcnt;
             }
         }
@@ -432,30 +458,59 @@
         TP("coefficients shipped");
         return SZHIP_OK;
     }
-    int launch_sweep() {
+    static size_t pub_hist_off() { return (size_t)PUB_AREAS * 8; }
+    static size_t pub_sample_off() { return pub_hist_off() + (size_t)SZH_COL_HBINS * 4; }
+    static size_t pub_mean_off(unsigned max_radius) { return (pub_sample_off() + (size_t)(max_radius + 8192) * 4 + 255) & ~(size_t)255; }
+    static size_t pub_bytes(unsigned max_radius, size_t M) { return pub_mean_off(max_radius) + M * sizeof(T) + 256; }
+    int prepare_sweep() {
+        if (sweep_ready) return SZHIP_OK;
         TRY(ensure(ctx, ctx->codes_nat, (size_t)n * 2 + 64));
         TRY(ensure(ctx, ctx->codes_blk, (size_t)n * 2 + 64));
         d_nat = (uint16_t *)ctx->codes_nat.p; d_blk = (uint16_t *)ctx->codes_blk.p;
-        int nI, nJ, ntiles;
+        int nI, nJ;
         using TS = szh_tile_shape<T>;
-        TRY(prepare_pencil(ctx, G, szh_gran<T>::NW, TS::TPI, TS::TPJ, &nI, &nJ, &ntiles));
+        TRY(prepare_pencil(ctx, G, szh_gran<T>::NW, TS::TPI, TS::TPJ, &nI, &nJ, &q_ntiles));
         const szh_bm::grid_t bgrid = szh_bm::make_grid(G);
         beam_words = (size_t)bgrid.nKB * bgrid.nJG * szh_bm::WPG;
+        if (beam_applies<T>(G, d_in, 0)) {
+            TRY(ensure(ctx, ctx->rb_down, szh_bm::kface_words<T>(G) * sizeof(u64) + 64, true));
+            TRY(ensure(ctx, ctx->rb_right, szh_bm::jface_words<T>(G) * sizeof(u64) + 64, true));
+        }
+        TRY(ensure(ctx, ctx->hist, (size_t)(65536 + 8192) * 4 + 64));
+        TRY(ensure(ctx, ctx->col_zeros, (size_t)ncols * 4));
+        TRY(ensure(ctx, ctx->col_zeros64, (size_t)ncols * 8));
+        TRY(ensure(ctx, ctx->col_off, (size_t)ncols * 8));
+        if (G.ndim == 3) {
+            TRY(ensure(ctx, ctx->seg_bits, (size_t)ncols * 8)); TRY(ensure(ctx, ctx->seg_zeros, (size_t)ncols * 8));
+            TRY(ensure(ctx, ctx->seg_bitoff, (size_t)ncols * 8)); TRY(ensure(ctx, ctx->seg_zoff, (size_t)ncols * 8));
+        }
+        szh_qargs<T> &a = qa; memset(&a, 0, sizeof(a));
+        a.pub_lines = 32;
+        a.G = G; a.data = d_in; a.out = nullptr; a.codes = d_nat; a.blk_lor = d_lor; a.coef = d_coef; a.coef_stride = nb;
+        a.eb = eb; a.recip = 1 / eb;
+        a.faceI = (szh_u64 *)ctx->faceI.p; a.faceJ = (szh_u64 *)ctx->faceJ.p;
+        a.nI = nI; a.nJ = nJ; a.order = (const unsigned *)ctx->order.p;
+        a.ticket = (unsigned *)(sm + SM_TICKET); a.err = (unsigned *)(sm + SM_ERR);
+        a.progress = (szh_u64 *)ctx->progress.p; a.backoff = SZH_FILL_BACKOFF; a.wide = pencil_wide<T>(G, nJ);
+        a.coef_progress = nullptr;
+        sweep_ready = true;
+        return SZHIP_OK;
+    }
+    int launch_sweep() {
+        TRY(prepare_sweep());
+        using TS = szh_tile_shape<T>;
+        const int ntiles = q_ntiles;
         if (P.sliced) {
             TRY(ensure_coherent(ctx, 512 + beam_words * 4));
             tile_done = (unsigned *)((char *)ctx->coh + 512);
             if (!ctx->stream3) HIPCHK(hipStreamCreateWithFlags(&ctx->stream3, hipStreamNonBlocking));
             if (!ctx->ev_perm) HIPCHK(hipEventCreateWithFlags(&ctx->ev_perm, hipEventDisableTiming));
         }
-        szh_qargs<T> a; memset(&a, 0, sizeof(a));
-        a.tile_done = tile_done; a.pub_lines = 32;
-        a.G = G; a.data = d_in; a.out = nullptr; a.codes = d_nat; a.blk_lor = d_lor; a.coef = d_coef; a.coef_stride = nb;
-        a.eb = eb; a.recip = 1 / eb; a.mean = mean; a.cap = (int)intervals; a.radius = (int)intervals / 2; a.use_mean = use_mean;
-        a.faceI = (szh_u64 *)ctx->faceI.p; a.faceJ = (szh_u64 *)ctx->faceJ.p; a.epoch = ++ctx->epoch;
-        a.nI = nI; a.nJ = nJ; a.order = (const unsigned *)ctx->order.p; a.no_reg = reg_count == 0;
-        a.ticket = (unsigned *)(sm + SM_TICKET); a.err = (unsigned *)(sm + SM_ERR); a.ticket_mode = ctx->ticket_atomic ? 0 : tune_int("SZ_HIP_TICKET_MODE", 2);
-        a.progress = (szh_u64 *)ctx->progress.p; a.backoff = SZH_FILL_BACKOFF; a.wide = pencil_wide<T>(G, nJ);
-        a.coef_progress = nullptr;
+        szh_qargs<T> a = qa;
+        a.tile_done = tile_done;
+        a.mean = mean; a.cap = (int)intervals; a.radius = (int)intervals / 2; a.use_mean = use_mean;
+        a.epoch = ++ctx->epoch; a.no_reg = reg_count == 0;
+        a.ticket_mode = ctx->ticket_atomic ? 0 : tune_int("SZ_HIP_TICKET_MODE", 2);
         szh_u64 *coh_prog = nullptr;
         T *dec = nullptr;
         const int64_t nbp = (nb + LINE - 1) / LINE * LINE;
@@ -572,13 +627,19 @@
         h_hist = (unsigned *)ctx->pinned;
         if (P.seghist) {
             TRY(ensure(ctx, ctx->seg_hist, (size_t)ncols * intervals * 4));
-            HIPCHK(hipMemsetAsync(d_hist, 0, (size_t)intervals * 4, st));
+            if (!hist_cleared) HIPCHK(hipMemsetAsync(d_hist, 0, (size_t)intervals * 4, st));
             hipLaunchKernelGGL(k_col_hist, dim3((unsigned)ncols), dim3(256), ((size_t)intervals * 4) << P.sh_rshift, st, G, (const uint16_t *)d_nat, intervals, P.sh_rshift, P.se_vw, (unsigned *)ctx->seg_hist.p);
-            hipLaunchKernelGGL(k_hist_reduce, dim3((unsigned)std::min<int64_t>(64, ncols)), dim3(256), 0, st, (const unsigned *)ctx->seg_hist.p, intervals, (int64_t)ncols, d_hist);
-            HIPCHK(hipGetLastError());
             if (!P.dev_book) {
-                HIPCHK(hipMemcpyAsync(h_hist, d_hist, (size_t)intervals * 4, hipMemcpyDeviceToHost, st));
-                HIPCHK(hipEventRecord(ctx->ev_fit, st));
+                TRY(ensure_pub(ctx, pub_bytes(prm->max_quant_intervals / 2, 0)));
+                h_hist = (unsigned *)((char *)ctx->pub + pub_hist_off());
+                seq_hist = ++ctx->pub_seq;
+                hipLaunchKernelGGL(k_hist_reduce, dim3((unsigned)std::min<int64_t>(64, ncols)), dim3(256), 0, st, (const unsigned *)ctx->seg_hist.p, intervals, (int64_t)ncols, d_hist,
+                                   (unsigned *)(sm + SM_ARRIVE) + 1, h_hist, (u64 *)ctx->pub + PUB_HIST, seq_hist);
+                HIPCHK(hipGetLastError());
+                HIPCHK(hipEventRecord(ctx->ev_pub, st));
+            } else {
+                hipLaunchKernelGGL(k_hist_reduce, dim3((unsigned)std::min<int64_t>(64, ncols)), dim3(256), 0, st, (const unsigned *)ctx->seg_hist.p, intervals, (int64_t)ncols, d_hist);
+                HIPCHK(hipGetLastError());
             }
         } else if (!P.sliced) TRY(launch_hist());
         TRY(ensure(ctx, ctx->col_zeros, (size_t)ncols * 4));
@@ -596,10 +657,14 @@
         return q + sizeof(T);
     }
     int upload_segments() {
+        const szhip_ctx::seg_key_t key = {{G.g0.count, G.g1.count, G.g2.count}, P.se_segb, P.se_vw};
+        if (ctx->seg_key == key) return SZHIP_OK;
+        ctx->seg_key.segb = 0;
         se_segs.resize((size_t)P.se_nseg);
         for (int q = 0; q < P.se_nseg; ++q) se_segs[(size_t)q] = szh_se::make_seg(G, 1, q, P.se_segb, P.se_vw);
         TRY(ensure(ctx, ctx->seg_tab, se_segs.size() * sizeof(szh_se::seg_t)));
         HIPCHK(hipMemcpyAsync(ctx->seg_tab.p, se_segs.data(), se_segs.size() * sizeof(szh_se::seg_t), hipMemcpyHostToDevice, st));
+        ctx->seg_key = key;
         return SZHIP_OK;
     }
     template <class F>
@@ -609,8 +674,8 @@
         TRY(ensure(ctx, ctx->seg_bitoff, (size_t)nent * 8)); TRY(ensure(ctx, ctx->seg_zoff, (size_t)nent * 8));
         u64 *const bits = (u64 *)ctx->seg_bits.p, *const zeros = (u64 *)ctx->seg_zeros.p, *const bitoff = (u64 *)ctx->seg_bitoff.p, *const zoff = (u64 *)ctx->seg_zoff.p;
         const size_t lb = intervals <= 16384 ? (size_t)intervals : 16;
-        if (P.seghist) hipLaunchKernelGGL(k_col_bits_h, dim3((unsigned)((nent + 255) / 256)), dim3(256), 0, st, (const unsigned *)ctx->seg_hist.p, (const uint8_t *)ctx->len_tab.p, intervals, nent, bits, zeros);
-        else hipLaunchKernelGGL(k_col_bits, dim3((unsigned)nent), dim3(256), lb, st, G, (const uint16_t *)d_nat, (const uint8_t *)ctx->len_tab.p, intervals, P.se_vw, bits, zeros);
+        if (P.seghist) hipLaunchKernelGGL(k_col_bits_h, dim3((unsigned)((nent + 255) / 256)), dim3(256), 0, st, (const unsigned *)ctx->seg_hist.p, d_len, intervals, nent, bits, zeros);
+        else hipLaunchKernelGGL(k_col_bits, dim3((unsigned)nent), dim3(256), lb, st, G, (const uint16_t *)d_nat, d_len, intervals, P.se_vw, bits, zeros);
         if (nent <= 1024 * SZH_COL_SCAN_PER && tune_int("SZ_HIP_SEG_SCAN1", 1))
             hipLaunchKernelGGL(k_col_scan, dim3(1), dim3(1024), 0, st, (const u64 *)bits, (const u64 *)zeros, (int)nent, bitoff, zoff, sm + SM_TOTAL_BITS, sm + SM_TOTAL_UNPRED, base_bits, (unsigned *)d_stream, d_plan);
         else {
@@ -670,6 +735,7 @@
         unsigned char *d_stream = in_place ? (unsigned char *)*out : (unsigned char *)ctx->stream_buf.p;
         TRY(ensure(ctx, ctx->book_stage, bk_front + bk_mid)); TRY(ensure(ctx, ctx->book_tree, tree_cap)); TRY(ensure(ctx, ctx->book_rec, 32 + SZH_PLAN_COUNT * 8));
         TRY(ensure(ctx, ctx->code_tab, (size_t)intervals * 8)); TRY(ensure(ctx, ctx->len_tab, (size_t)intervals));
+        d_len = (const uint8_t *)ctx->len_tab.p;
         TRY(ensure(ctx, ctx->unpred, unpred_cap + 64));
         szh_book_rec *const d_rec = (szh_book_rec *)ctx->book_rec.p;
         u64 *const d_plan = (u64 *)((char *)ctx->book_rec.p + 32);
@@ -701,10 +767,11 @@
     }
     int build_host_book() {
         TP("permute launched");
-        HIPCHK(hipEventSynchronize(ctx->ev_fit));
+        if (seq_hist) TRY(wait_published(ctx, (const u64 *)ctx->pub + PUB_HIST, seq_hist, ctx->ev_pub, "code histogram"));
+        else HIPCHK(hipEventSynchronize(ctx->ev_fit));
         TP("hist on host");
         double h0 = now_ms();
-        const huff_ptr hf = host_book(h_hist, intervals, tab_code, tab_len, &enc_maxlen);
+        hf = host_book(h_hist, intervals, tab_code, tab_len, &enc_maxlen);
         host_ms += now_ms() - h0;
         total_unpred = h_hist[0];
         if (!hf) FAIL(SZHIP_ERR_INTERNAL, "Huffman build failed");
@@ -719,18 +786,6 @@
         hdr_len = pre_len + sections_total + 8;
         unpred_bytes = (size_t)total_unpred * sizeof(T);
         total_len = hdr_len + unpred_bytes + (size_t)((hf->total_bits + 7) / 8);
-        TRY(ensure_pinned(ctx, pre_len + 8 + 64));
-        hdr = (unsigned char *)ctx->pinned;
-        memset(hdr, 0, pre_len + 8);
-        unsigned char *q = put_front(hdr);
-        szhost_put_u32be(q, intervals); q += 4;
-        szhost_put_u32be(q, (uint32_t)tree_bytes); q += 4;
-        szhost_put_u32be(q, (uint32_t)hf->n_nodes); q += 4;
-        szhost_huff_tree_write(hf.get(), q); q += tree_bytes;
-        *q++ = (unsigned char)use_mean;
-        memcpy(q, &mean, sizeof(T)); q += sizeof(T);
-        memcpy(q, ind_bits, ind_bytes); q += ind_bytes;
-        const uint64_t tu = total_unpred; memcpy(q, &tu, 8);
         total_bits = hf->total_bits;
         lds_e32 = (size_t)intervals * 8 + ((size_t)SZH_E32_ROUND * enc_maxlen / 32 + 4) * 4 + 16;
         enc32 = enc_maxlen >= 1 && enc_maxlen <= 32 && lds_e32 <= 60 * 1024 && tune_int("SZ_HIP_ENC32", 1);
@@ -738,23 +793,56 @@
             if (P.sliced) HIPCHK(hipStreamWaitEvent(st, ctx->ev_perm, 0));
             TRY(permute_all());
         }
-        if (P.segenc) TRY(upload_segments());
-        if (P.segenc) for (unsigned s = 0; s < intervals; ++s) tab_code[s] = (tab_code[s] << 32) | tab_len[s] | (s == 0 ? 0x10000u : 0u);
-        else if (enc32) for (unsigned s = 0; s < intervals; ++s) tab_code[s] = (tab_code[s] << 8) | tab_len[s];
+        if (!P.segenc) {
+            if (enc32) for (unsigned s = 0; s < intervals; ++s) tab_code[s] = (tab_code[s] << 8) | tab_len[s];
+            host_ms += now_ms() - h0;
+            TRY(upload_code_tables(ctx, tab_code, tab_len));
+            d_len = (const uint8_t *)ctx->len_tab.p;
+            return SZHIP_OK;
+        }
+        TRY(upload_segments());
+        const size_t len_off = (size_t)intervals * 8, tab_bytes = len_off + intervals;
+        TRY(ensure_host(ctx, ctx->tab_pin, ctx->tab_pin_cap, tab_bytes, st));
+        u64 *const pc = (u64 *)ctx->tab_pin; uint8_t *const pl = (uint8_t *)ctx->tab_pin + len_off;
+        for (unsigned s = 0; s < intervals; ++s) { pc[s] = (tab_code[s] << 32) | tab_len[s] | (s == 0 ? 0x10000u : 0u); pl[s] = tab_len[s]; }
         host_ms += now_ms() - h0;
-        return upload_code_tables(ctx, tab_code, tab_len);
+        TRY(ensure(ctx, ctx->code_tab, tab_bytes));
+        HIPCHK(hipMemcpyAsync(ctx->code_tab.p, ctx->tab_pin, tab_bytes, hipMemcpyHostToDevice, st));
+        d_len = (const uint8_t *)ctx->code_tab.p + len_off;
+        return SZHIP_OK;
+    }
+    int assemble_header() {
+        const double h0 = now_ms();
+        const size_t tree_bytes = szhost_huff_tree_size(hf.get());
+        TRY(ensure_pinned(ctx, pre_len + 8 + 64));
+        hdr = (unsigned char *)ctx->pinned;
+        unsigned char *q = put_front(hdr);
+        szhost_put_u32be(q, intervals); q += 4;
+        szhost_put_u32be(q, (uint32_t)tree_bytes); q += 4;
+        szhost_put_u32be(q, (uint32_t)hf->n_nodes); q += 4;
+        memset(q, 0, tree_bytes);
+        szhost_huff_tree_write(hf.get(), q); q += tree_bytes;
+        *q++ = (unsigned char)use_mean;
+        memcpy(q, &mean, sizeof(T)); q += sizeof(T);
+        memcpy(q, ind_bits, ind_bytes); q += ind_bytes;
+        const uint64_t tu = total_unpred; memcpy(q, &tu, 8);
+        host_ms += now_ms() - h0;
+        return SZHIP_OK;
     }
     int copy_header(unsigned char *d_stream) {
+        if (sections_total == 0) { HIPCHK(hipMemcpyAsync(d_stream, hdr, pre_len + 8, hipMemcpyHostToDevice, st)); return SZHIP_OK; }
         HIPCHK(hipMemcpyAsync(d_stream, hdr, pre_len, hipMemcpyHostToDevice, st));
         HIPCHK(hipMemcpyAsync(d_stream + pre_len + sections_total, hdr + pre_len, 8, hipMemcpyHostToDevice, st));
-        if (sections_total) {
-            const hipStream_t ssec = ctx->stream3 ? ctx->stream3 : ctx->stream2;
-            HIPCHK(hipEventRecord(ctx->ev_feed, st));
-            HIPCHK(hipStreamWaitEvent(ssec, ctx->ev_feed, 0));
-            size_t off = pre_len;
-            for (int e = 0; e < ncoef; ++e) { HIPCHK(hipMemcpyAsync(d_stream + off, ctx->sec_pin[e], sec_len[e], hipMemcpyHostToDevice, ssec)); off += sec_len[e]; }
-            HIPCHK(hipEventRecord(ctx->ev_sec, ssec));
-        }
+        return SZHIP_OK;
+    }
+    int copy_sections(unsigned char *d_stream) {
+        if (!sections_total) return SZHIP_OK;
+        const hipStream_t ssec = ctx->stream3 ? ctx->stream3 : ctx->stream2;
+        HIPCHK(hipEventRecord(ctx->ev_feed, st));
+        HIPCHK(hipStreamWaitEvent(ssec, ctx->ev_feed, 0));
+        size_t off = pre_len;
+        for (int e = 0; e < ncoef; ++e) { HIPCHK(hipMemcpyAsync(d_stream + off, ctx->sec_pin[e], sec_len[e], hipMemcpyHostToDevice, ssec)); off += sec_len[e]; }
+        HIPCHK(hipEventRecord(ctx->ev_sec, ssec));
         return SZHIP_OK;
     }
     int pack_block_ordered(unsigned char *d_stream) {
@@ -788,13 +876,15 @@
         if (!in_place) TRY(ensure(ctx, ctx->stream_buf, total_len + 64));
         unsigned char *d_stream = in_place ? (unsigned char *)*out : (unsigned char *)ctx->stream_buf.p;
         if (P.segenc) {
-            TRY(pack_columns(d_stream, (u64)(hdr_len + unpred_bytes) * 8, (const u64 *)nullptr, enc_maxlen, [&]() -> int {
-                TRY(copy_header(d_stream));
-                return ensure(ctx, ctx->unpred, unpred_bytes + 64);
-            }));
+            TRY(ensure(ctx, ctx->unpred, unpred_bytes + 64));
+            TRY(pack_columns(d_stream, (u64)(hdr_len + unpred_bytes) * 8, (const u64 *)nullptr, enc_maxlen, [&]() -> int { return copy_sections(d_stream); }));
+            TRY(assemble_header());
+            TRY(copy_header(d_stream));
         } else {
             HIPCHK(hipMemsetAsync(d_stream, 0, total_len + 64, st));
+            TRY(assemble_header());
             TRY(copy_header(d_stream));
+            TRY(copy_sections(d_stream));
             TRY(pack_block_ordered(d_stream));
         }
         if (total_unpred > 0) HIPCHK(hipMemcpyAsync(d_stream + hdr_len, ctx->unpred.p, unpred_bytes, hipMemcpyDeviceToDevice, st));
@@ -1141,6 +1231,7 @@
         HIPCHK(hipGetLastError());
         up_segs.resize((size_t)up_nseg);
         for (int q = 0; q < up_nseg; ++q) up_segs[(size_t)q] = szh_se::make_seg(G, 1, q, up_segb, up_vw);
+        ctx->seg_key.segb = 0;
         TRY(ensure(ctx, ctx->seg_tab, up_segs.size() * sizeof(szh_se::seg_t)));
         HIPCHK(hipMemcpyAsync(ctx->seg_tab.p, up_segs.data(), up_segs.size() * sizeof(szh_se::seg_t), hipMemcpyHostToDevice, st));
     } else
```

Result: no change. 393.0, median of 6 (+2.4%).
